# Sthiber/COSC_4397_Pathtracing_Raytracing_Project

Hardware: AMD Instinct MI355X
Metric: Msamples/s, cornell.txt 1920x1080 depth 8 (+PSNR vs 5000spp ref) (higher is better)
Workload: dtype f32

## Files before the change

### cosc_4397_pathtracing_raytracing_project_amd/capi.py

```python
from __future__ import annotations

import ctypes as C
import os
from typing import Optional, Sequence, Tuple

import numpy as np

_PKG = os.path.dirname(os.path.abspath(__file__))
LIB_PATH = os.environ.get("PT_AMD_LIB") or os.path.join(_PKG, "libpt_amd.so")
PT_MAX_DEPTH = 64
ARITH = {"exact": 0, "fma": 1, "fast": 2}
ARITH_NAMES = {v: k for k, v in ARITH.items()}
FEATURE_PLANES = 3
NOISE_PLANES = 2
NOISE_PIXELS_PER_PARTIAL = 1024
CONVERGENCE_WAVES = 16
CONVERGENCE_CAPACITY = 65536
FLT_MAX = float(np.finfo(np.float32).max)


class PtGeom(C.Structure):
    _fields_ = [("type", C.c_int32), ("materialid", C.c_int32), ("transform", C.c_float * 16),
                ("inverseTransform", C.c_float * 16), ("invTranspose", C.c_float * 16)]


class PtMaterial(C.Structure):
    _fields_ = [("color", C.c_float * 3), ("specular_exponent", C.c_float), ("specular_color", C.c_float * 3),
                ("hasReflective", C.c_float), ("hasRefractive", C.c_float), ("indexOfRefraction", C.c_float),
                ("emittance", C.c_float)]


class PtCamera(C.Structure):
    _fields_ = [("resolution", C.c_int32 * 2), ("position", C.c_float * 3), ("lookAt", C.c_float * 3),
                ("view", C.c_float * 3), ("up", C.c_float * 3), ("right", C.c_float * 3), ("fov", C.c_float * 2),
                ("pixelLength", C.c_float * 2)]


class PtBVHNode(C.Structure):
    _fields_ = [("bmin", C.c_float * 3), ("bmax", C.c_float * 3), ("left", C.c_int32), ("right", C.c_int32),
                ("geomIndex", C.c_int32)]


class PtGridInfo(C.Structure):
    _fields_ = [("res", C.c_int32 * 3), ("origin", C.c_float * 3), ("cell_size", C.c_float * 3), ("pad", C.c_float),
                ("num_cells", C.c_int32), ("num_records", C.c_int32), ("num_leaves", C.c_int32)]


class PtGridRecord(C.Structure):
    _fields_ = [("bmin", C.c_float * 3), ("bmax", C.c_float * 3), ("leaf", C.c_int32), ("neighbours", C.c_int32)]


class PtSceneDesc(C.Structure):
    _fields_ = [("geoms", C.POINTER(PtGeom)), ("num_geoms", C.c_int32), ("materials", C.POINTER(PtMaterial)),
                ("num_materials", C.c_int32), ("camera", PtCamera), ("trace_depth", C.c_int32)]


class PtOptions(C.Structure):
    _fields_ = [("device", C.c_int32), ("pixel_begin", C.c_int32), ("pixel_count", C.c_int32),
                ("iters_per_batch", C.c_int32), ("num_queues", C.c_int32), ("blocks_per_cu", C.c_int32),
                ("time_kernels", C.c_int32), ("legacy_traversal", C.c_int32), ("debug_flags", C.c_int32), ("unfused_primary", C.c_int32), ("unfused_bounces", C.c_int32), ("stripe_pixels", C.c_int32), ("stripe_stride", C.c_int32),
                ("arith", C.c_int32), ("aa_jitter", C.c_int32), ("convergence", C.c_int32),
                ("lds_table_kb", C.c_int32), ("primary_pieces", C.c_int32), ("paths_pieces", C.c_int32), ("paths_min_piece", C.c_int32)]


class PtStats(C.Structure):
    _fields_ = [("samples", C.c_int64), ("live_rays", C.c_int64 * PT_MAX_DEPTH), ("intersect_launches", C.c_int64),
                ("intersect_ms", C.c_double), ("render_ms", C.c_double), ("num_cus", C.c_int32),
                ("grid_blocks", C.c_int32), ("num_queues", C.c_int32), ("iters_per_batch", C.c_int32),
                ("device_bytes", C.c_int64), ("primary_fused", C.c_int32), ("bounces_fused", C.c_int32),
                ("arith", C.c_int32), ("grid_cells", C.c_int32), ("tight_leaves", C.c_int32), ("paths_waves", C.c_int32), ("record_form", C.c_int32)]


class PtDenoiseOptions(C.Structure):
    _fields_ = [("levels", C.c_int32), ("sigma_color", C.c_float), ("sigma_normal", C.c_float), ("sigma_position", C.c_float),
                ("keep_albedo", C.c_int32)]


class PtError(RuntimeError):
    pass


_lib: Optional[C.CDLL] = None
_fp = C.POINTER(C.c_float)
_ip = C.POINTER(C.c_int32)


def lib() -> C.CDLL:
    global _lib
    if _lib is not None:
        return _lib
    if not os.path.exists(LIB_PATH):
        raise PtError(f"{LIB_PATH} not found: run `python -c 'import __graft_entry__ as g; g.build()'` "
                      "(hipcc --offload-arch=gfx950).  There is no CPU fallback.")
    L = C.CDLL(LIB_PATH)
    L.pt_last_error.restype = C.c_char_p
    L.pt_scene_load.argtypes = [C.c_char_p, C.c_int, C.c_int, C.POINTER(C.c_void_p)]
    L.pt_scene_free.argtypes = [C.c_void_p]
    L.pt_scene_free.restype = None
    L.pt_scene_desc.argtypes = [C.c_void_p, C.POINTER(PtSceneDesc)]
    L.pt_scene_iterations.argtypes = [C.c_void_p]
    L.pt_scene_image_name.argtypes = [C.c_void_p]
    L.pt_scene_image_name.restype = C.c_char_p
    L.pt_build_bvh.argtypes = [C.POINTER(PtGeom), C.c_int, C.POINTER(PtBVHNode), C.c_int]
    L.pt_build_grid.argtypes = [C.POINTER(PtGeom), C.c_int, C.c_int, C.POINTER(PtGridInfo), C.POINTER(C.c_uint32), C.POINTER(PtGridRecord)]
    if hasattr(L, "pt_selfcheck_ieee"):
        L.pt_selfcheck_ieee.argtypes = [C.c_int, C.c_int, C.c_uint64, C.c_uint64, C.c_uint32, C.POINTER(C.c_uint64)]
    if hasattr(L, "pt_traversal_boxes"):
        L.pt_traversal_boxes.argtypes = [C.POINTER(PtGeom), C.c_int, _fp, _fp]
    if hasattr(L, "pt_center_half_box"):
        L.pt_center_half_box.argtypes = [_fp, _fp, C.c_int, C.c_float, _fp, _fp]
        L.pt_center_half_box.restype = None
    L.pt_build_transform.argtypes = [_fp, _fp, _fp, _fp]
    L.pt_init.argtypes = [C.POINTER(PtSceneDesc), C.POINTER(PtOptions)]
    L.pt_render.argtypes = [C.c_int, C.c_int]
    L.pt_readback.argtypes = [_fp]
    L.pt_readback_device.argtypes = [C.c_void_p]
    L.pt_preview_rgba8.argtypes = [C.c_int, C.POINTER(C.c_uint8)]
    L.pt_preview_rgba8_device.argtypes = [C.c_int, C.c_void_p]
    L.pt_get_stats.argtypes = [C.POINTER(PtStats)]
    L.pt_stage_generate.argtypes = [C.c_int, C.c_int, _fp, _fp]
    L.pt_stage_intersect.argtypes = [C.c_int, _fp, _fp, _fp, _fp, _ip, _fp]
    if hasattr(L, "pt_stage_intersect_grid"):
        L.pt_stage_intersect_grid.argtypes = [C.c_int, _fp, _fp, C.c_int, _fp, _fp, _ip, _fp]
        L.pt_stage_grid_info.argtypes = [C.POINTER(PtGridInfo), C.POINTER(C.c_int32)]
    L.pt_stage_shade.argtypes = [C.c_int, C.c_int, _ip, _ip, _fp, _fp, _ip, _fp, _fp, _fp, _fp, _ip]
    _u8p = C.POINTER(C.c_uint8)
    L.pt_save_u8.argtypes = [C.c_float, _u8p]
    L.pt_stage_save_u8.argtypes = [C.c_int, C.c_int, C.c_float, _fp, _u8p]
    L.pt_ctx_create.argtypes = [C.POINTER(PtSceneDesc), C.POINTER(PtOptions), C.POINTER(C.c_void_p)]
    L.pt_ctx_destroy.argtypes = [C.c_void_p]
    L.pt_ctx_render.argtypes = [C.c_void_p, C.c_int, C.c_int]
    L.pt_ctx_sync.argtypes = [C.c_void_p]
    L.pt_ctx_readback.argtypes = [C.c_void_p, _fp]
    L.pt_ctx_readback_device.argtypes = [C.c_void_p, C.c_void_p]
    L.pt_ctx_save_u8.argtypes = [C.c_void_p, C.c_float, _u8p]
    L.pt_ctx_get_stats.argtypes = [C.c_void_p, C.POINTER(PtStats)]
    L.pt_ctx_reset_stats.argtypes = [C.c_void_p]
    L.pt_ctx_clear.argtypes = [C.c_void_p]
    L.pt_ctx_pixel_count.argtypes = [C.c_void_p]
    L.pt_group_create.argtypes = [C.POINTER(PtSceneDesc), C.POINTER(PtOptions), _ip, C.c_int, C.POINTER(C.c_void_p)]
    if hasattr(L, "pt_group_create_ex"):
        L.pt_group_create_ex.argtypes = [C.POINTER(PtSceneDesc), C.POINTER(PtOptions), _ip, C.c_int, C.c_int, C.POINTER(C.c_void_p)]
        L.pt_group_transport.argtypes = [C.c_void_p]
    L.pt_group_destroy.argtypes = [C.c_void_p]
    L.pt_group_size.argtypes = [C.c_void_p]
    L.pt_group_context.argtypes = [C.c_void_p, C.c_int]
    L.pt_group_context.restype = C.c_void_p
    L.pt_group_render.argtypes = [C.c_void_p, C.c_int, C.c_int]
    L.pt_group_sync.argtypes = [C.c_void_p]
    L.pt_group_gather.argtypes = [C.c_void_p, _fp]
    L.pt_group_gather_u8.argtypes = [C.c_void_p, C.c_float, _u8p]
    L.pt_group_preview_rgba8.argtypes = [C.c_void_p, C.c_int, _u8p]
    L.pt_write_png_rgb8.argtypes = [C.c_char_p, _u8p, C.c_int, C.c_int]
    L.pt_output_basename.argtypes = [C.c_char_p, C.c_int, C.c_char_p, C.c_int]
    L.pt_save_png.argtypes = [C.c_char_p, _fp, C.c_int, C.c_int, C.c_float]
    L.pt_save_hdr.argtypes = [C.c_char_p, _fp, C.c_int, C.c_int, C.c_float]
    L.pt_save_pfm.argtypes = [C.c_char_p, _fp, C.c_int, C.c_int, C.c_float]
    L.pt_load_pfm.argtypes = [C.c_char_p, _fp, C.c_int, _ip, _ip, C.c_float]
    _dp = C.POINTER(C.c_double)
    L.pt_psnr_from_sse.argtypes = [C.c_double, C.c_int64]
    L.pt_psnr_from_sse.restype = C.c_float
    L.pt_set_reference.argtypes = [_fp]
    L.pt_get_convergence.argtypes = [C.c_int, C.c_int, _dp]
    L.pt_iterations_to_clean.argtypes = [C.c_float, _ip]
    L.pt_ctx_set_reference.argtypes = [C.c_void_p, _fp]
    L.pt_ctx_get_convergence.argtypes = [C.c_void_p, C.c_int, C.c_int, _dp]
    L.pt_ctx_iterations_to_clean.argtypes = [C.c_void_p, C.c_float, _ip]
    L.pt_group_set_reference.argtypes = [C.c_void_p, _fp]
    L.pt_group_get_convergence.argtypes = [C.c_void_p, C.c_int, C.c_int, _dp]
    L.pt_group_iterations_to_clean.argtypes = [C.c_void_p, C.c_float, _ip]
    if hasattr(L, "pt_render_features"):
        L.pt_render_features.argtypes = [C.c_int, C.c_int]
        L.pt_readback_features.argtypes = [_fp]
        L.pt_ctx_render_features.argtypes = [C.c_void_p, C.c_int, C.c_int]
        L.pt_ctx_readback_features.argtypes = [C.c_void_p, _fp]
        L.pt_ctx_device_features.argtypes = [C.c_void_p]
        L.pt_ctx_device_features.restype = C.c_void_p
        L.pt_group_render_features.argtypes = [C.c_void_p, C.c_int, C.c_int]
        L.pt_group_gather_features.argtypes = [C.c_void_p, _fp]
    if hasattr(L, "pt_denoise"):
        _dno = C.POINTER(PtDenoiseOptions)
        L.pt_denoise.argtypes = [C.c_float, _dno, _fp]
        L.pt_ctx_denoise.argtypes = [C.c_void_p, C.c_float, _dno, _fp]
        L.pt_ctx_denoise_device.argtypes = [C.c_void_p, C.c_float, _dno, C.POINTER(C.c_void_p)]
        L.pt_group_denoise.argtypes = [C.c_void_p, C.c_float, _dno, _fp]
        L.pt_stage_denoise.argtypes = [C.c_int, C.c_int, _fp, _fp, C.c_float, _dno, _fp]
        L.pt_denoise_host.argtypes = [C.c_int, C.c_int, _fp, _fp, C.c_float, _dno, _fp]
    if hasattr(L, "pt_denoise_guided"):
        _dno = C.POINTER(PtDenoiseOptions)
        _guided = [C.c_int, C.c_int, _fp, _fp, _fp, C.c_int, C.c_int64, _dno]
        L.pt_denoise_guided.argtypes = [_dno, _fp]
        L.pt_ctx_denoise_guided.argtypes = [C.c_void_p, _dno, _fp]
        L.pt_ctx_denoise_guided_device.argtypes = [C.c_void_p, _dno, C.POINTER(C.c_void_p)]
        L.pt_group_denoise_guided.argtypes = [C.c_void_p, _dno, _fp]
        L.pt_stage_denoise_guided.argtypes = _guided + [_fp]
        L.pt_denoise_guided_host.argtypes = _guided + [_fp]
        L.pt_denoise_guided_variance_host.argtypes = _guided + [_fp, _fp]
    if hasattr(L, "pt_noise_fold"):
        _until = [C.c_int, C.c_int, C.c_int, C.c_float, _ip, _fp]
        L.pt_noise_fold.argtypes = []
        L.pt_get_noise.argtypes = [_dp, _ip, _ip]
        L.pt_readback_noise.argtypes = [_fp]
        L.pt_render_until.argtypes = _until
        L.pt_ctx_noise_fold.argtypes = [C.c_void_p]
        L.pt_ctx_get_noise.argtypes = [C.c_void_p, _dp, _ip, _ip]
        L.pt_ctx_readback_noise.argtypes = [C.c_void_p, _fp]
        L.pt_ctx_render_until.argtypes = [C.c_void_p] + _until
        L.pt_ctx_device_noise.argtypes = [C.c_void_p]
        L.pt_ctx_device_noise.restype = C.c_void_p
        L.pt_group_noise_fold.argtypes = [C.c_void_p]
        L.pt_group_get_noise.argtypes = [C.c_void_p, _dp, _ip, _ip]
        L.pt_group_render_until.argtypes = [C.c_void_p] + _until
        L.pt_noise_fold_host.argtypes = [C.c_int, _fp, _fp, C.c_int, C.c_int, C.c_int64, _dp]
    if hasattr(L, "pt_adaptive_round"):
        _i64p = C.POINTER(C.c_int64)
        _adaptive = [C.c_int, C.c_int, C.c_int, C.c_float, C.c_float, _ip, _i64p, _fp]
        L.pt_adaptive_round.argtypes = [C.c_int, C.c_int, C.c_float]
        L.pt_render_adaptive.argtypes = _adaptive
        L.pt_readback_adaptive.argtypes = [_ip]
        L.pt_resolve.argtypes = [_fp]
        L.pt_ctx_adaptive_round.argtypes = [C.c_void_p, C.c_int, C.c_int, C.c_float]
        L.pt_ctx_render_adaptive.argtypes = [C.c_void_p] + _adaptive
        L.pt_ctx_readback_adaptive.argtypes = [C.c_void_p, _ip]
        L.pt_ctx_resolve.argtypes = [C.c_void_p, _fp]
        L.pt_ctx_resolve_device.argtypes = [C.c_void_p, C.POINTER(C.c_void_p)]
        L.pt_adaptive_select_host.argtypes = [C.c_int, C.c_int, _fp, _ip, C.c_int, _ip]
        L.pt_stage_adaptive_select.argtypes = [C.c_int, C.c_int, _fp, _ip, C.c_int, _ip]
        L.pt_adaptive_merge_host.argtypes = [C.c_int, _fp, _fp, _ip, _ip, C.c_int, _fp, C.c_int, _dp]
        L.pt_stage_render_list.argtypes = [_ip, C.c_int, C.c_int, C.c_int, _fp]
    if hasattr(L, "pt_denoise_adaptive"):
        _dno = C.POINTER(PtDenoiseOptions)
        _dn_adaptive = [C.c_int, C.c_int, _fp, _fp, _fp, _ip, _dno]
        L.pt_denoise_adaptive.argtypes = [_dno, _fp]
        L.pt_ctx_denoise_adaptive.argtypes = [C.c_void_p, _dno, _fp]
        L.pt_ctx_denoise_adaptive_device.argtypes = [C.c_void_p, _dno, C.POINTER(C.c_void_p)]
        L.pt_stage_denoise_adaptive.argtypes = _dn_adaptive + [_fp]
        L.pt_denoise_adaptive_host.argtypes = _dn_adaptive + [_fp]
        L.pt_denoise_adaptive_variance_host.argtypes = _dn_adaptive + [_fp, _fp]
    _lib = L
    return L


def _check(rc: int) -> None:
    if rc != 0:
        raise PtError(lib().pt_last_error().decode(errors="replace"))


def _f(a: np.ndarray):
    assert a.dtype == np.float32 and a.flags.c_contiguous
    return a.ctypes.data_as(_fp)


def _i(a: np.ndarray):
    assert a.dtype == np.int32 and a.flags.c_contiguous
    return a.ctypes.data_as(_ip)


class Scene:

    def __init__(self, path: str, res: Optional[Tuple[int, int]] = None):
        self._h = C.c_void_p()
        w, h = res if res else (0, 0)
        _check(lib().pt_scene_load(os.fsencode(path), int(w), int(h), C.byref(self._h)))
        self.desc = PtSceneDesc()
        _check(lib().pt_scene_desc(self._h, C.byref(self.desc)))

    def __del__(self):
        h = getattr(self, "_h", None)
        if h is not None and h.value and _lib is not None:
            _lib.pt_scene_free(h)
            self._h = C.c_void_p()

    @property
    def resolution(self) -> Tuple[int, int]:
        return self.desc.camera.resolution[0], self.desc.camera.resolution[1]

    @property
    def trace_depth(self) -> int:
        return self.desc.trace_depth

    @trace_depth.setter
    def trace_depth(self, d: int) -> None:
        self.desc.trace_depth = int(d)

    @property
    def iterations(self) -> int:
        return lib().pt_scene_iterations(self._h)

    @property
    def image_name(self) -> str:
        return lib().pt_scene_image_name(self._h).decode()

    def geoms(self):
        return [self.desc.geoms[i] for i in range(self.desc.num_geoms)]

    def materials(self):
        return [self.desc.materials[i] for i in range(self.desc.num_materials)]

    def grid(self, forced: bool = False):
        info = PtGridInfo()
        rc = lib().pt_build_grid(self.desc.geoms, self.desc.num_geoms, int(forced), C.byref(info), None, None)
        if rc < 0:
            raise PtError(lib().pt_last_error().decode(errors="replace"))
        if rc == 0:
            return None
        start = (C.c_uint32 * (info.num_cells + 1))()
        recs = (PtGridRecord * info.num_records)()
        lib().pt_build_grid(self.desc.geoms, self.desc.num_geoms, int(forced), C.byref(info), start, recs)
        return info, np.frombuffer(start, np.uint32).copy(), recs

    def traversal_boxes(self):
        boxes = np.zeros((self.desc.num_geoms, 6), np.float32)
        cam = np.asarray(list(self.desc.camera.position), np.float32)
        rc = lib().pt_traversal_boxes(self.desc.geoms, self.desc.num_geoms, _f(cam), _f(boxes))
        if rc < 0:
            raise PtError(lib().pt_last_error().decode(errors="replace"))
        return boxes, rc

    def bvh(self):
        n = lib().pt_build_bvh(self.desc.geoms, self.desc.num_geoms, None, 0)
        arr = (PtBVHNode * n)()
        lib().pt_build_bvh(self.desc.geoms, self.desc.num_geoms, arr, n)
        return arr


def selfcheck_ieee(kind: int, first: int, count: int, seed: int = 0, arith: str = "exact") -> int:
    n = C.c_uint64(0)
    _check(lib().pt_selfcheck_ieee(ARITH[arith], kind, first, count, seed, C.byref(n)))
    return int(n.value)


def build_transform(trs: Sequence[float]):
    t = np.asarray(trs, np.float32).copy()
    m, i, it = (np.zeros(16, np.float32) for _ in range(3))
    lib().pt_build_transform(_f(t), _f(m), _f(i), _f(it))
    return m, i, it


def make_options(device: int = 0, pixel_begin: int = 0, pixel_count: int = 0, iters_per_batch: int = 0,
                 num_queues: int = 0, blocks_per_cu: int = 0, time_kernels: bool = False, legacy_traversal: bool = False,
                 debug_flags: int = 0, unfused_primary: bool = False, unfused_bounces: bool = False,
                 stripe_pixels: int = 0, stripe_stride: int = 0, arith="exact", aa_jitter: bool = False,
                 lds_table_kb: int = 0, primary_pieces: int = 0, paths_pieces: int = 0, paths_min_piece: int = 0, primary_share: int = 0,
                 convergence: int = 0) -> PtOptions:
    opt = PtOptions()
    opt.device = device
    opt.pixel_begin = pixel_begin
    opt.pixel_count = pixel_count
    opt.iters_per_batch = iters_per_batch
    opt.num_queues = num_queues
    opt.blocks_per_cu = blocks_per_cu
    opt.time_kernels = 1 if time_kernels else 0
    opt.legacy_traversal = 1 if legacy_traversal else 0
    opt.debug_flags = int(debug_flags)
    opt.unfused_primary = 1 if unfused_primary else 0
    opt.unfused_bounces = 1 if unfused_bounces else 0
    opt.stripe_pixels = int(stripe_pixels)
    opt.stripe_stride = int(stripe_stride)
    opt.arith = ARITH[arith] if isinstance(arith, str) else int(arith)
    opt.aa_jitter = 1 if aa_jitter else 0
    opt.convergence = int(convergence)
    opt.lds_table_kb = int(lds_table_kb)
    pp = int(primary_pieces)
    opt.primary_pieces = pp if pp < 0 else min(pp, 0x7fff) | max(0, min(int(primary_share), 64)) << 16
    opt.paths_pieces = int(paths_pieces)
    opt.paths_min_piece = int(paths_min_piece)
    return opt


def split_features(planes: np.ndarray) -> dict:
    p = planes.reshape(FEATURE_PLANES, -1, 4)
    return dict(normal=np.ascontiguousarray(p[0, :, :3]), depth=np.ascontiguousarray(p[0, :, 3]),
                albedo=np.ascontiguousarray(p[1, :, :3]), hits=np.ascontiguousarray(p[1, :, 3]),
# ... 504 lines not shown
```

### cosc_4397_pathtracing_raytracing_project_amd/csrc/pt_api.cpp

```cpp
#include <cmath>
#include <cstdarg>
#include <cstdio>
#include <cstring>
#include <string>

#include "pt_adaptive.h"
#include "pt_context.h"
#include "pt_lds.h"
#include "pt_scene.h"
#include "pt_sched.h"

namespace {

std::string g_err;
constexpr int kDebugFlags = 16 | 32 | 64 | 128 | 256 | 512 | ptk::kRetireEveryIteration | 2048 | ptk::kWholeRecords | ptk::kNoFirstBounce;
static_assert(sizeof(PtOptions) == 80, "capi.PtOptions mirrors this layout");
static_assert(PT_CONVERGENCE_WAVES == ptk::kConvWaves, "pt_amd.h documents the size of the convergence metric's partial sums");
}
int pt_fail(const char* fmt, ...) {
  char buf[1024];
  va_list ap;
  va_start(ap, fmt);
  vsnprintf(buf, sizeof(buf), fmt, ap);
  va_end(ap);
  g_err = buf;
  return -1;
}

namespace ptc {
static PtContext* g_default = nullptr;
PtContext* default_context() { return g_default; }

int get_events(Ctx& g, EventPair* ev) {
  if (!g.free_events.empty()) {
    *ev = g.free_events.back();
    g.free_events.pop_back();
    return 0;
  }
  HIP_OK(hipEventCreate(&ev->a));
  HIP_OK(hipEventCreate(&ev->b));
  return 0;
}
static int resolve_events(Ctx& g) {
  auto drain = [&](std::vector<EventPair>& pending, double& total_ms) -> int {
    for (auto& e : pending) {
      float ms = 0;
      HIP_OK(hipEventElapsedTime(&ms, e.a, e.b));
      total_ms += ms;
      g.free_events.push_back(e);
    }
    pending.clear();
    return 0;
  };
  g.isect_launches += (int64_t)g.pending_isect.size();
  return drain(g.pending_isect, g.isect_ms) || drain(g.pending_render, g.render_ms) ? -1 : 0;
}

ptk::SceneTables tables(const Ctx& g) {
  ptk::SceneTables t = g.scene;
  if (g.debug_flags & 16) t.cull_margin = INFINITY;
  if (g.debug_flags & 32) t.top_xor = 0;
  t.lds_table_bytes = g.lds_table_bytes;
  t.max_batch_iters = g.K;
  t.trace_depth = g.depth;
  t.scan_nodes_lds = -1;
  t.use_grid = !g.grids.empty() && g.grid_enabled && !(g.debug_flags & 512) ? 1 : 0;
  if (t.use_grid) {
    const Ctx::DeviceGrid& gr = g.grids[g.grid_pick];
    t.lds_table_bytes = -1;
    t.grid_start = gr.d_start + gr.guard;
    t.grid_items = gr.d_items;
    t.grid_items_b = gr.d_items_b;
    for (int a = 0; a < 3; ++a)
      t.grid_res[a] = gr.shape.res[a], t.grid_min[a] = gr.shape.gmin[a], t.grid_cs[a] = gr.shape.cs[a], t.grid_inv_cs[a] = gr.shape.inv_cs[a];
    t.grid_pad = gr.shape.pad;
  }
  return t;
}

static size_t pathbuf_words(int64_t stride) { return (size_t)(2 * stride + (stride * ptd::kPathPlane2Bytes + 15) / 16); }
static int alloc_pathbuf(Ctx& g, ptd::PathBuf* b, int64_t stride) {
  b->stride = stride;
  return dalloc(g, &b->r, pathbuf_words(stride));
}
static int alloc_hitbuf(Ctx& g, ptd::HitBuf* h, int64_t stride) {
  h->stride = stride;
  return dalloc(g, &h->t, stride) || dalloc(g, &h->n, 3 * stride) || dalloc(g, &h->mat, stride) || dalloc(g, &h->p, 3 * stride) ? -1 : 0;
}

static ptd::Queues queues_for(const Ctx& g, int grid) {
  ptd::Queues q = g.qs;
  q.W = grid * ptk::kWavesPerBlock;
  return q;
}

static int primary_share_of(const Ctx& g) { return (g.debug_flags & 128) ? 1 : g.primary_share ? g.primary_share : ptk::kShareMax; }
static bool shares_first_hit(const Ctx& g) { return ptk::primary_shares(primary_share_of(g), g.aa_jitter, !g.fuse_bounces); }

ptk::BatchInfo tile_batch(const Ctx& g, int iter_first, int K) {
  ptk::BatchInfo b{};
  b.iter_first = iter_first;
  b.K = K;
  b.N = g.N;
  b.pixel_begin = g.pixel_begin;
  b.trace_depth = g.depth;
  b.aa_jitter = g.aa_jitter ? 1 : 0;
  b.stripe = g.stripe;
  b.gap = g.stripe ? g.stripe_stride - g.stripe : 0;
  b.inv_stripe = g.stripe ? 1.0f / (float)g.stripe : 0.0f;
  return b;
}

int run_batch(Ctx& g, int iter_first, int kb) {
  ptk::BatchInfo b = tile_batch(g, iter_first, kb);
  b.slot_shift = g.slot_shift;
  b.flat = g.fuse_bounces ? 0 : 1;
  b.primary_share = primary_share_of(g);
  b.primary_pieces = g.primary_pieces ? g.primary_pieces
                     : ptk::primary_shares(b) ? ptk::auto_shared_pieces(kb, g.qs.nq, g.ret.wq0) : ptk::auto_primary_pieces(kb, g.qs.nq, g.ret.wq0);
  b.paths_pieces = g.paths_pieces;
  const ptk::SceneTables sc = tables(g);
  b.retire_once = ptk::retires_once(b, g.debug_flags) ? 1 : 0;
  b.split_records = ptk::record_form(b, g.debug_flags, ptk::search_form(sc), sc.num_mats);
  if (b.split_records == ptk::kFirstBounce) b.primary_pieces = 1;
  g.record_form = b.split_records;
  b.list = g.list;
  if (b.list) b.stripe = 1, b.gap = 0, b.inv_stripe = 1.0f;
  const ptk::KernelApi& k = *g.k;
  auto cnt_row = [&](int d) { return g.d_cnt + ptk::cnt_index(g.qs, d, 0); };
  int d0 = 0;
  if (g.fuse_primary) {
    k.primary(g.stream, g.grid_primary, sc, g.dcam, b, queues_for(g, g.grid_primary), cnt_row(0), cnt_row(1), g.buf[1],
              g.ret);
    d0 = 1;
  } else {
    k.generate(g.stream, g.grid_gen, g.dcam, b, queues_for(g, g.grid_gen), g.buf[0], cnt_row(0));
  }
  int src = d0 & 1;
  const bool all_depths = g.grid_paths > 0;
  EventPair ev{};
  auto timed_from = [&]() -> int {
    if (!g.time_kernels) return 0;
    if (get_events(g, &ev)) return -1;
    HIP_OK(hipEventRecord(ev.a, g.stream));
    return 0;
  };
  auto timed_to = [&]() -> int {
    if (!g.time_kernels) return 0;
    HIP_OK(hipEventRecord(ev.b, g.stream));
    g.pending_isect.push_back(ev);
    return 0;
  };
  if (all_depths) {
    if (timed_from()) return -1;
    k.paths(g.stream, g.grid_paths, sc, b, queues_for(g, g.grid_paths), g.d_cnt, g.buf[1], g.ret);
    if (timed_to()) return -1;
  }
  for (int d = d0; d < g.depth && !all_depths; ++d) {
    const int32_t* cin = cnt_row(d);
    int32_t* cout = cnt_row(d + 1);
    if (timed_from()) return -1;
    k.intersect(g.stream, g.grid_isect, sc, queues_for(g, g.grid_isect), cin, g.buf[src], g.hits, g.legacy, d == 0);
    if (timed_to()) return -1;
    k.shade(g.stream, g.grid_shade, sc, b, d, queues_for(g, g.grid_shade), cin, cout, g.buf[src], g.hits, g.buf[src ^ 1], g.ret);
    src ^= 1;
  }
  k.count_stats(g.stream, g.qs, g.d_cnt, g.depth, g.d_stats);
  ptk::ConvInfo cv{g.d_ref, g.d_partial, -1, kb};
  if (g.conv_live) {
    if (g.conv_have_ref) cv.first_k = 0;
    else if (g.conv >= iter_first && g.conv < iter_first + kb) cv.capture_k = g.conv - iter_first, cv.first_k = cv.capture_k + 1, g.conv_have_ref = true;
    g.conv_last = std::max(g.conv_last, iter_first + kb - 1);
  }
  if (cv.capture_k >= 0 || cv.first_k < kb) k.collect_conv(g.stream, b, g.qs, g.ret, g.d_image, cv, g.d_sse);
  else k.collect(g.stream, b, g.qs, g.ret, g.d_image);
  HIP_OK(hipGetLastError());
  g.samples += (int64_t)kb * g.N;
  if (g.pending_isect.size() > 16384) {
    HIP_OK(hipStreamSynchronize(g.stream));
    if (resolve_events(g)) return -1;
  }
  return 0;
}

void plan_launch(Ctx& g) {
  if (!g.borrowed) g.lds_table_bytes = g.k->lds_table_limit(tables(g), g.lds_table_forced);
  const ptk::SceneTables t = tables(g);
  g.grid_gen = g.num_cus * std::min(g.cap_bpc, g.k->resident_blocks_per_cu(ptk::kGenerate, t));
  g.grid_isect = g.num_cus * std::min(g.cap_bpc, g.k->resident_blocks_per_cu(g.legacy ? ptk::kIntersectLegacy : ptk::kIntersect, t));
  g.grid_shade = g.num_cus * std::min(g.cap_bpc, g.k->resident_blocks_per_cu(ptk::kShade, t));
  g.grid_primary = g.num_cus * std::min(g.cap_bpc, g.k->resident_blocks_per_cu(shares_first_hit(g) ? ptk::kPrimaryShared : ptk::kPrimary, t));
  g.ret.wq0 = ptk::wave_slot(0, g.qs.Q, g.grid_primary * ptk::kWavesPerBlock).wq;
  g.grid_paths = (g.fuse_bounces && g.depth > 1) ? g.num_cus * std::min(g.cap_bpc, g.k->resident_blocks_per_cu(ptk::kPaths, t)) : 0;
  g.qs.paths_W = g.grid_paths * ptk::kWavesPerBlock;
}

static int choose_traversal(Ctx& g) {
  auto drop_unused_grids = [&](size_t keep) {
    for (size_t i = 0; i < g.grids.size(); ++i) {
      const Ctx::DeviceGrid& d = g.grids[i];
      if (i == keep) continue;
      for (void* p : {(void*)d.d_start, (void*)d.d_items, d.d_items_b != d.d_items ? (void*)d.d_items_b : nullptr}) {
        if (!p) continue;
        (void)hipFree(p);
        g.allocs.erase(std::remove(g.allocs.begin(), g.allocs.end(), p), g.allocs.end());
      }
      g.device_bytes -= (int64_t)d.bytes;
    }
    g.grids = {g.grids[keep]};
    g.grid_pick = 0;
  };
  if (g.grids.empty()) return 0;
  if (!g.fuse_bounces || (g.debug_flags & (256 | 512))) {
    drop_unused_grids(0);
    return 0;
  }
  auto time_one = [&](float* ms) -> int {
    plan_launch(g);
    for (int rep = 0; rep < 2; ++rep) {
      EventPair ev{};
      if (get_events(g, &ev)) return -1;
      HIP_OK(hipEventRecord(ev.a, g.stream));
      if (run_batch(g, 1, std::min(g.K, 8))) return -1;
      HIP_OK(hipEventRecord(ev.b, g.stream));
      HIP_OK(hipStreamSynchronize(g.stream));
      HIP_OK(hipEventElapsedTime(ms, ev.a, ev.b));
      g.free_events.push_back(ev);
    }
    return 0;
  };
  g.grid_enabled = false;
  if (time_one(&g.probe_ms[0])) return -1;
  g.grid_enabled = true;
  size_t best = 0;
  for (size_t i = 0; i < g.grids.size(); ++i) {
    float ms = 0.f;
    g.grid_pick = i;
    if (time_one(&ms)) return -1;
    if (i == 0 || ms < 0.97f * g.probe_ms[1]) g.probe_ms[1] = ms, best = i;
  }
  drop_unused_grids(best);
  g.grid_enabled = g.probe_ms[1] < 0.95f * g.probe_ms[0];
  plan_launch(g);
  HIP_OK(hipMemsetAsync(g.d_image, 0, 3 * (size_t)g.N * sizeof(float), g.stream));
  HIP_OK(hipMemsetAsync(g.d_stats, 0, PT_MAX_DEPTH * sizeof(unsigned long long), g.stream));
  HIP_OK(hipStreamSynchronize(g.stream));
  g.samples = 0;
  return 0;
}

ptd::Queues single_queue(const Ctx& g, int n) {
  ptd::Queues qs{};
  qs.Q = 1;
  const ptk::QueuePlan p = ptk::queue_plan(n, 1, 1);
  qs.cap = p.cap;
  qs.W = g.grid * ptk::kWavesPerBlock;
  qs.cnt_stride = 16;
  qs.nq = p.nq;
  qs.inv_nq = 1.0f / (float)qs.nq;
  return qs;
}

void destroy(Ctx* c) {
  if (!c) return;
  destroy(c->worker);
  (void)hipSetDevice(c->device);
  if (c->stream) (void)hipStreamSynchronize(c->stream);
  for (void* p : c->allocs) (void)hipFree(p);
  auto kill = [](std::vector<EventPair>& v) {
    for (auto& e : v) {
      (void)hipEventDestroy(e.a);
      (void)hipEventDestroy(e.b);
    }
    v.clear();
  };
  kill(c->free_events);
  kill(c->pending_isect);
  kill(c->pending_render);
  if (c->stream && !c->borrowed) (void)hipStreamDestroy(c->stream);
  delete c;
}

static int open_device(Ctx& g, const PtOptions& opt) {
  g.arith = opt.arith;
  g.k = ptk::api_for(opt.arith);
  if (!g.k) return pt_fail("pt_init: arith %d is not one of PT_ARITH_EXACT / PT_ARITH_FMA / PT_ARITH_FAST", opt.arith);
  if (opt.convergence < -1) return pt_fail("pt_init: convergence %d is not 0 (off), N > 0 (frame captured at iteration N) or -1 (frame supplied)", opt.convergence);
  if (opt.convergence > PT_CONVERGENCE_CAPACITY) return pt_fail("pt_init: convergence %d exceeds PT_CONVERGENCE_CAPACITY (%d iterations)", opt.convergence, PT_CONVERGENCE_CAPACITY);
  if (opt.primary_pieces > 0 && (opt.primary_pieces >> 16) > ptk::kShareMax) return pt_fail("pt_init: primary_pieces 0x%x: primary_share %d exceeds %d (PT_PRIMARY_PIECES)", opt.primary_pieces, opt.primary_pieces >> 16, ptk::kShareMax);
  if (opt.debug_flags & ~kDebugFlags) return pt_fail("pt_init: debug_flags 0x%x: bits 0x%x are not defined", opt.debug_flags, opt.debug_flags & ~kDebugFlags);
  int ndev = 0;
  HIP_OK(hipGetDeviceCount(&ndev));
  if (ndev <= 0) return pt_fail("pt_init: no HIP device (this library has no CPU fallback)");
  if (opt.device < 0 || opt.device >= ndev) return pt_fail("pt_init: device %d of %d", opt.device, ndev);
  g.device = opt.device;
  HIP_OK(hipSetDevice(g.device));
  hipDeviceProp_t prop;
  HIP_OK(hipGetDeviceProperties(&prop, g.device));
  g.num_cus = prop.multiProcessorCount;
  HIP_OK(hipStreamCreateWithFlags(&g.stream, hipStreamNonBlocking));
  return 0;
}

static void take_scene_and_options(Ctx& g, const PtSceneDesc* sc, const PtOptions& opt) {
  g.cam = sc->camera;
  g.depth = sc->trace_depth;
  g.dcam.res_x = g.cam.resolution[0], g.dcam.res_y = g.cam.resolution[1];
  std::memcpy(g.dcam.pos, g.cam.position, 12);
  std::memcpy(g.dcam.view, g.cam.view, 12);
  std::memcpy(g.dcam.up, g.cam.up, 12);
  std::memcpy(g.dcam.right, g.cam.right, 12);
  g.dcam.pl_x = g.cam.pixelLength[0], g.dcam.pl_y = g.cam.pixelLength[1];
  g.legacy = opt.legacy_traversal != 0;
  g.aa_jitter = opt.aa_jitter != 0;
  g.debug_flags = opt.debug_flags;
  g.conv = opt.convergence;
  auto pieces = [](int v, int automatic) { return v ? std::clamp(v, 1, 0x7fff) : automatic; };
  g.lds_table_forced = opt.lds_table_kb ? std::clamp(opt.lds_table_kb, 0, ptk::kLdsTableBytes / 1024) * 1024 : -1;
  g.primary_pieces = pieces(opt.primary_pieces < 0 ? opt.primary_pieces : opt.primary_pieces & 0xffff, 0);
  g.primary_share = opt.primary_pieces < 0 ? 0 : std::min(opt.primary_pieces >> 16 & 0x7f, ptk::kShareMax);
  g.paths_pieces = ptk::pack_paths_pieces(pieces(opt.paths_pieces, 2), pieces(opt.paths_min_piece, 64));
  g.fuse_primary = !g.legacy && !opt.unfused_primary;
  g.fuse_bounces = g.fuse_primary && !opt.unfused_bounces;
  g.cap_bpc = opt.blocks_per_cu > 0 ? std::min(opt.blocks_per_cu, 8) : 8;
}

int batch_iters_for(int iters_per_batch, int N, int* slot_shift) {
  int K = iters_per_batch;
  if (K <= 0) {
    const int64_t target = 48ll << 20;
    K = (int)std::max<int64_t>(1, std::min<int64_t>(256, (target + N - 1) / N));
  }
  int shift = 1;
  while ((1ll << shift) < N) ++shift;
  if (shift > 30) return pt_fail("pt_init: tiles of more than 2^30 pixels are not supported");
  while (K > 1 && K > (1 << (31 - shift))) --K;
  if (slot_shift) *slot_shift = shift;
  return K;
}

int plan_batches(Ctx& g, const PtOptions& opt) {
  const int W = g.cam.resolution[0], H = g.cam.resolution[1];
  g.opt_iters_per_batch = opt.iters_per_batch, g.opt_num_queues = opt.num_queues;
  g.pixel_begin = opt.pixel_begin;
  g.N = opt.pixel_count > 0 ? opt.pixel_count : W * H - opt.pixel_begin;
  g.stripe = opt.stripe_pixels;
  g.stripe_stride = opt.stripe_stride;
  if (g.stripe < 0 || (g.stripe > 0 && g.stripe_stride < g.stripe)) return pt_fail("pt_init: bad stripe %d / stride %d", g.stripe, g.stripe_stride);
  {
    int64_t last = (int64_t)g.pixel_begin + g.N - 1;
    if (g.stripe > 0) last = (int64_t)g.pixel_begin + (g.N - 1) + (int64_t)((g.N - 1) / g.stripe) * (g.stripe_stride - g.stripe);
    if (g.pixel_begin < 0 || g.N <= 0 || last >= (int64_t)W * H)
      return pt_fail("pt_init: tile [%d, +%d, stripe %d/%d) outside %dx%d", opt.pixel_begin, opt.pixel_count, g.stripe, g.stripe_stride, W, H);
    if (g.stripe > 0 && g.N / g.stripe >= 32768) return pt_fail("pt_init: more than 32767 stripes");
    if (H >= 32768) return pt_fail("pt_init: image height %d not supported (>= 32768)", H);
  }
  const int K = batch_iters_for(opt.iters_per_batch, g.N, &g.slot_shift);
  if (K < 0) return -1;

  int Q = opt.num_queues > 0 ? opt.num_queues : 256;
  const int cu_waves = g.num_cus * ptk::kWavesPerBlock;
  if (Q > cu_waves) Q = cu_waves;
  while (cu_waves % Q) --Q;
  if (opt.num_queues <= 0)
    while (ptk::chunks_per_queue(g.N, Q) > 128 && 2 * Q <= cu_waves && cu_waves % (2 * Q) == 0) Q *= 2;
  const ptk::QueuePlan plan = ptk::queue_plan(g.N, Q, K);
  const int grid = g.num_cus * 8;
  g.K = K;
  g.grid = grid;
  g.qs.Q = Q;
  g.qs.W = grid * ptk::kWavesPerBlock;
  g.qs.cnt_stride = 16;
  g.qs.nq = plan.nq;
  g.qs.inv_nq = 1.0f / (float)plan.nq;
  g.qs.cap = plan.cap;
  g.stride = (int64_t)Q * g.qs.cap;
  g.ret.seg_cap = plan.seg_cap;
  g.ret.kmax = K;
  return 0;
}

template <typename T>
static const T* upload(Ctx& g, const std::vector<T>& v) {
  T* p = nullptr;
  if (dalloc(g, &p, v.size())) return nullptr;
  const hipError_t e = hipMemcpy(p, v.data(), v.size() * sizeof(T), hipMemcpyHostToDevice);
  return e == hipSuccess ? p : (pt_fail("hipMemcpy(%zu bytes) failed: %s", v.size() * sizeof(T), hipGetErrorString(e)), nullptr);
}
static int upload_tables(Ctx& g, const pt::HostTables& t) {
  ptk::SceneTables& s = g.scene;
  s.num_nodes = (int)t.nodes.size(), s.num_geoms = (int)t.geoms.size(), s.num_mats = (int)t.mats.size(), s.num_top = (int)t.top.size();
  std::memcpy(s.root_min, t.root_min, 12);
  std::memcpy(s.root_max, t.root_max, 12);
  s.cull_margin = t.cull_margin;
  s.top_xor = t.top_xor;
  s.has_triangles = t.has_triangles ? 1 : 0;
  g.tight_leaves = t.tight_leaves;
  if (!(s.nodes = upload(g, t.nodes)) || !(s.geoms = upload(g, t.geoms)) || !(s.mats = upload(g, t.mats)) || !(s.top = upload(g, t.top))) return -1;
  s.nodes_b = s.nodes, s.top_b = s.top;
  if (!t.nodes_b.empty() && (!(s.nodes_b = upload(g, t.nodes_b)) || !(s.top_b = upload(g, t.top_b)))) return -1;
  for (const pt::Grid& gr : t.grids) {
    Ctx::DeviceGrid d{gr.shape, gr.guard, nullptr, nullptr, nullptr, 0, gr.start};
    const int64_t before = g.device_bytes;
    if (!(d.d_start = upload(g, gr.start)) || !(d.d_items = upload(g, gr.items))) return -1;
    if (!(d.d_items_b = gr.items_b.empty() ? d.d_items : upload(g, gr.items_b))) return -1;
    d.bytes = (size_t)(g.device_bytes - before);
    g.grids.push_back(d);
  }
  return 0;
}

static __global__ void k_poison_records(ptd::Word4* rec, unsigned long long per_queue, unsigned long long total, int Q) {
  const float nan = __builtin_nanf("");
  for (unsigned long long i = (unsigned long long)blockIdx.x * blockDim.x + threadIdx.x; i < total; i += (unsigned long long)gridDim.x * blockDim.x)
    rec[i] = ptd::Word4{nan, nan, nan, __int_as_float(ptk::chunk_pixel((int)(i / per_queue), 0, Q))};
}

int alloc_batch_buffers(Ctx& g) {
  const int Q = g.qs.Q;
  if (alloc_pathbuf(g, &g.buf[0], g.stride) || alloc_pathbuf(g, &g.buf[1], g.stride)) return -1;
  for (const ptd::PathBuf& pb : g.buf) HIP_OK(hipMemset(pb.r, 0xff, pathbuf_words(pb.stride) * sizeof(ptd::Word4)));
  if (!g.fuse_bounces && alloc_hitbuf(g, &g.hits, g.stride)) return -1;
  {
    const size_t regions = (size_t)Q * g.ret.kmax;
    const size_t wq_max = ptk::sub_stride(g.num_cus * 8 * ptk::kWavesPerBlock, Q);
    if (dalloc(g, &g.ret.rec, regions * g.ret.seg_cap)) return -1;
    if (ensure(g, g.ret.cnt, regions * sizeof(*g.ret.cnt), Zero::blocking) || ensure(g, g.ret.sub, regions * wq_max * sizeof(*g.ret.sub), Zero::blocking)) return -1;
    {
      const size_t per_queue = (size_t)g.ret.kmax * g.ret.seg_cap;
      hipLaunchKernelGGL(k_poison_records, dim3((unsigned)std::min<size_t>((regions * g.ret.seg_cap + 255) / 256, 65536)), dim3(256), 0, g.stream, g.ret.rec,
                         (unsigned long long)per_queue, (unsigned long long)(regions * g.ret.seg_cap), Q);
      HIP_OK(hipGetLastError());
    }
  }
  const size_t image_bytes = 3 * (size_t)g.N * sizeof(float);
  const size_t cnt_words = ptk::cnt_index(g.qs, g.depth + 1, 0);
  if (ensure(g, g.d_image, image_bytes, Zero::blocking) || ensure(g, g.d_cnt, cnt_words * sizeof(int32_t), Zero::blocking) ||
      ensure(g, g.d_stats, PT_MAX_DEPTH * sizeof(*g.d_stats), Zero::blocking))
    return -1;
  if (!(g.debug_flags & 64) && ensure(g, g.qs.deal, (size_t)ptk::deal_map(g.qs).words() * sizeof(int32_t), Zero::blocking)) return -1;
  if (g.conv) {
    const size_t partials = (size_t)g.K * Q * ptk::kConvWaves;
    if (ensure(g, g.d_ref, image_bytes, Zero::blocking) || ensure(g, g.d_partial, partials * sizeof(double), Zero::blocking)) return -1;
    if (dalloc(g, &g.d_sse, (size_t)PT_CONVERGENCE_CAPACITY)) return -1;
    HIP_OK(hipMemset(g.d_sse, 0xff, (size_t)PT_CONVERGENCE_CAPACITY * sizeof(double)));
  }
  HIP_OK(hipDeviceSynchronize());
  return 0;
}

static int setup(Ctx& g, const PtSceneDesc* sc, const PtOptions& opt) {
  if (open_device(g, opt)) return -1;
  take_scene_and_options(g, sc, opt);
  if (plan_batches(g, opt)) return -1;
  if ((size_t)sc->num_materials * sizeof(ptd::Mat) > 60 * 1024) return pt_fail("pt_init: %zu materials exceed the LDS table", (size_t)sc->num_materials);
  const pt::HostTables host = pt::build_scene_tables(*sc, g.debug_flags, g.k->boxes_center_half != 0);
  if (upload_tables(g, host)) return -1;
  plan_launch(g);
  if (alloc_batch_buffers(g) || choose_traversal(g)) return -1;
  g.time_kernels = opt.time_kernels != 0;
  g.conv_live = g.conv != 0;
  return 0;
}

int need(const PtContext* c, const char* who) { return c ? 0 : pt_fail("%s: pt_init has not been called", who); }

int admit(const PtContext& g, const char* who, unsigned req) {
  if ((req & kNotFailed) && g.failed) return pt_fail("%s: an earlier batch of this context failed (%s); free it and create a new one", who, g_err.c_str());
  if ((req & kUniform) && g.adaptive)
    return pt_fail("%s: the renderer is in the adaptive state (pt_adaptive_round): one sample count no longer describes the image; read it with pt_resolve, or "
                   "return to the uniform state with pt_clear", who);
  const int W = g.cam.resolution[0];
  if ((req & kWholeRows) && (g.stripe || g.pixel_begin % W || g.N % W))
    return pt_fail("%s: the tile must consist of whole contiguous image rows (begin %d, count %d, stripe %d, width %d)", who, g.pixel_begin, g.N, g.stripe, W);
  if ((req & kFoldedAll) && g.rendered != g.noise_iters)
    return pt_fail("%s: %lld iteration(s) rendered since the last fold; fold first (pt_noise_fold)", who, (long long)(g.rendered - g.noise_iters));
  if (req & kOnDevice) HIP_OK(hipSetDevice(g.device));
  return 0;
}

}
using namespace ptc;

extern "C" {

const char* pt_last_error(void) { return g_err.c_str(); }

int pt_selfcheck_ieee(int arith, int kind, uint64_t first, uint64_t count, uint32_t seed, uint64_t* mismatches) {
  const ptk::KernelApi* k = ptk::api_for(arith);
  if (!k || kind < 0 || kind > 4 || !mismatches) return pt_fail("pt_selfcheck_ieee: bad argument");
  unsigned long long* d = nullptr;
  HIP_OK(hipMalloc(&d, sizeof(*d)));
  hipError_t e = hipMemset(d, 0, sizeof(*d));
  if (e == hipSuccess) {
    k->ieee_check(nullptr, kind, first, count, seed, d);
    e = hipGetLastError();
  }
  unsigned long long h = 0;
  if (e == hipSuccess) e = hipMemcpy(&h, d, sizeof(h), hipMemcpyDeviceToHost);
  (void)hipFree(d);
  if (e != hipSuccess) return pt_fail("pt_selfcheck_ieee: %s", hipGetErrorString(e));
  *mismatches = h;
  return 0;
}

struct PtScene {
  pt::Scene scene;
  explicit PtScene(const std::string& f) : scene(f) {}
};

int pt_scene_load(const char* path, int res_w, int res_h, PtScene** out) {
  if (!path || !out) return pt_fail("pt_scene_load: null argument");
  try {
    PtScene* s = new PtScene(path);
    if (res_w > 0 && res_h > 0) s->scene.overrideResolution(res_w, res_h);
    s->scene.applyInitialCameraState();
    *out = s;
    return 0;
  } catch (const std::exception& e) {
    return pt_fail("pt_scene_load: %s", e.what());
  }
}
void pt_scene_free(PtScene* s) { delete s; }
int pt_scene_desc(const PtScene* s, PtSceneDesc* out) {
  if (!s || !out) return pt_fail("pt_scene_desc: null argument");
  *out = s->scene.desc();
  return 0;
}
int pt_scene_iterations(const PtScene* s) { return s ? (int)s->scene.state.iterations : 0; }
const char* pt_scene_image_name(const PtScene* s) { return s ? s->scene.state.imageName.c_str() : ""; }

int pt_build_bvh(const PtGeom* geoms, int num_geoms, PtBVHNode* out, int cap) {
  std::vector<PtBVHNode> nodes;
  pt::buildBVH(geoms, num_geoms, nodes);
  if (out) std::memcpy(out, nodes.data(), sizeof(PtBVHNode) * std::min<size_t>(nodes.size(), (size_t)std::max(cap, 0)));
  return (int)nodes.size();
}

int pt_traversal_boxes(const PtGeom* geoms, int num_geoms, const float camera_position[3], float* boxes) {
  if (!geoms || num_geoms <= 0 || !camera_position || !boxes) return pt_fail("pt_traversal_boxes: null argument");
  pt::ThreadedBvh bvh = pt::threaded_bvh(geoms, num_geoms);
  double olo[3], ohi[3];
  pt::origin_region(bvh.ref[0].bmin, bvh.ref[0].bmax, camera_position, olo, ohi);
  const int tightened = pt::tighten_sphere_leaves(bvh.nodes, geoms, olo, ohi);
  for (const ptd::Node& n : bvh.nodes)
    if (n.geom >= 0) std::memcpy(boxes + 6 * (size_t)n.geom, n.bmin, 12), std::memcpy(boxes + 6 * (size_t)n.geom + 3, n.bmax, 12);
  return tightened;
}

int pt_build_grid(const PtGeom* geoms, int num_geoms, int forced, PtGridInfo* info, uint32_t* cell_start, PtGridRecord* records) {
  if (!geoms || num_geoms <= 0 || !info) return pt_fail("pt_build_grid: null argument");
  const pt::ThreadedBvh bvh = pt::threaded_bvh(geoms, num_geoms);
  std::memset(info, 0, sizeof(*info));
  info->num_leaves = num_geoms;
  if (!forced && (int)bvh.nodes.size() < pt::kGridNodes) return 0;
  pt::Grid gr;
  if (!pt::build_grid(bvh.nodes, geoms, num_geoms, bvh.ref[0].bmin, bvh.ref[0].bmax, 0.0, 0.0, forced != 0, gr)) return 0;
  for (int a = 0; a < 3; ++a) info->res[a] = gr.shape.res[a], info->origin[a] = gr.shape.gmin[a], info->cell_size[a] = gr.shape.cs[a];
  info->pad = gr.shape.pad;
  info->num_cells = (int32_t)(gr.start.size() - 1);
  info->num_records = (int32_t)gr.items.size();
  if (cell_start) std::memcpy(cell_start, gr.start.data(), gr.start.size() * sizeof(uint32_t));
  static_assert(sizeof(PtGridRecord) == sizeof(ptd::Node), "PtGridRecord mirrors the device record");
  if (records) std::memcpy(records, gr.items.data(), gr.items.size() * sizeof(ptd::Node));
  return 1;
}

void pt_center_half_box(const float lo[3], const float hi[3], int inner, float magnitude, float center[3], float half_extent[3]) {
  float a[3] = {lo[0], lo[1], lo[2]}, b[3] = {hi[0], hi[1], hi[2]};
  pt::center_half_box(a, b, inner != 0, (double)magnitude);
  std::memcpy(center, a, 12);
  std::memcpy(half_extent, b, 12);
}

int pt_build_transform(const float* trs, float* transform, float* inverse, float* invTranspose) {
  if (!trs || !transform || !inverse || !invTranspose) return pt_fail("pt_build_transform: null argument");
  pt::buildTransform(trs, transform, inverse, invTranspose);
  return 0;
}

int pt_ctx_create(const PtSceneDesc* sc, const PtOptions* opt_in, PtContext** out) {
  if (!out) return pt_fail("pt_ctx_create: null output");
  *out = nullptr;
  if (!sc) return pt_fail("pt_init: null scene");
  if (sc->num_geoms <= 0 || !sc->geoms) return pt_fail("pt_init: scene has no geometry");
  if (sc->num_materials <= 0 || !sc->materials) return pt_fail("pt_init: scene has no materials");
  if (sc->trace_depth <= 0 || sc->trace_depth > PT_MAX_DEPTH) return pt_fail("pt_init: trace_depth %d out of range", sc->trace_depth);
  const int W = sc->camera.resolution[0], H = sc->camera.resolution[1];
  if (W <= 0 || H <= 0 || (int64_t)W * H > (1ll << 30)) return pt_fail("pt_init: bad resolution %dx%d", W, H);
  for (int i = 0; i < sc->num_geoms; ++i) {
    if (sc->geoms[i].materialid < 0 || sc->geoms[i].materialid >= sc->num_materials)
      return pt_fail("pt_init: geom %d references material %d of %d", i, sc->geoms[i].materialid, sc->num_materials);
    if (sc->geoms[i].type < PT_GEOM_SPHERE || sc->geoms[i].type > PT_GEOM_TRIANGLE)
      return pt_fail("pt_init: geom %d has unknown type %d", i, sc->geoms[i].type);
  }
  PtOptions opt{};
  if (opt_in) opt = *opt_in;
  PtContext* c = new PtContext();
  if (setup(*c, sc, opt)) {
    destroy(c);
    return -1;
  }
  *out = c;
  return 0;
}

int pt_ctx_destroy(PtContext* c) {
  if (c == g_default) g_default = nullptr;
  destroy(c);
  return 0;
}

int pt_ctx_render(PtContext* c, int iter_first, int iter_count) {
  if (need(c, "pt_render")) return -1;
  if (iter_count <= 0) return 0;
  Ctx& g = *c;
  if (admit(g, "pt_render", kNotFailed | kUniform)) return -1;
  if (g.conv_live) {
    if (iter_first < 1 || (int64_t)iter_first + iter_count - 1 > PT_CONVERGENCE_CAPACITY)
      return pt_fail("pt_render: iterations %d .. %lld outside 1 .. %d (PT_CONVERGENCE_CAPACITY) with the convergence metric on", iter_first,
                  (long long)iter_first + iter_count - 1, PT_CONVERGENCE_CAPACITY);
    if (g.conv < 0 && !g.conv_have_ref) return pt_fail("pt_render: PtOptions.convergence is -1 but no reference frame has been supplied (pt_set_reference)");
  }
  HIP_OK(hipSetDevice(g.device));
  EventPair ev{};
  if (get_events(g, &ev)) return -1;
  HIP_OK(hipEventRecord(ev.a, g.stream));
  const int end = iter_first + iter_count;
  for (int it = iter_first; it < end; it += g.K)
    if (run_batch(g, it, std::min(g.K, end - it))) {
      g.failed = true;
      g.free_events.push_back(ev);
      return -1;
    }
  HIP_OK(hipEventRecord(ev.b, g.stream));
  g.pending_render.push_back(ev);
  g.rendered += iter_count;
  return 0;
}

int pt_ctx_sync(PtContext* c) {
  if (need(c, "pt_sync")) return -1;
  HIP_OK(hipSetDevice(c->device));
  HIP_OK(hipStreamSynchronize(c->stream));
  return resolve_events(*c);
}

int pt_ctx_readback(PtContext* c, float* out) {
  if (need(c, "pt_readback")) return -1;
  return copy_out(c, "pt_readback", out, 3, [&](const float** d) { return *d = c->d_image, 0; });
}

int pt_ctx_readback_device(PtContext* c, void* out) {
  if (need(c, "pt_readback_device")) return -1;
  return copy_out(c, "pt_readback_device", static_cast<float*>(out), 3, [&](const float** d) { return *d = c->d_image, 0; }, hipMemcpyDeviceToDevice);
}

const float* pt_ctx_device_image(PtContext* c) { return c ? c->d_image : nullptr; }
void* pt_ctx_stream(PtContext* c) { return c ? (void*)c->stream : nullptr; }
int pt_ctx_pixel_count(const PtContext* c) { return c ? c->N : 0; }
int pt_ctx_device(const PtContext* c) { return c ? c->device : -1; }

int pt_ctx_save_u8_device(PtContext* c, float samples, const uint8_t** rgb8_dev) {
  if (need(c, "pt_save_u8")) return -1;
  Ctx& g = *c;
  const int W = g.cam.resolution[0];
  if (!(samples > 0.0f)) return pt_fail("pt_save_u8: samples must be positive");
  if (admit(g, "pt_save_u8", kUniform)) return -1;
  if (g.pixel_begin % W || g.N % W || (g.stripe && g.stripe != W))
    return pt_fail("pt_save_u8: the tile must consist of whole image rows (begin %d, count %d, stripe %d, width %d)", g.pixel_begin, g.N, g.stripe, W);
  HIP_OK(hipSetDevice(g.device));
  if (ensure(g, g.d_rgb8, 3 * (size_t)g.N)) return -1;
  g.k->save_u8(g.stream, g.N, W, samples, g.d_image, g.d_rgb8);
  HIP_OK(hipGetLastError());
  if (rgb8_dev) *rgb8_dev = g.d_rgb8;
  return 0;
}
int pt_ctx_save_u8(PtContext* c, float samples, uint8_t* rgb8_host) {
  return copy_out(c, "pt_save_u8", rgb8_host, 3, [&](const uint8_t** d) { return pt_ctx_save_u8_device(c, samples, d); });
}

int pt_ctx_preview_rgba8_device(PtContext* c, int iterations, void* rgba_dev) {
  if (need(c, "pt_preview_rgba8_device")) return -1;
  if (!rgba_dev || iterations <= 0) return pt_fail("pt_preview_rgba8_device: bad argument");
  if (admit(*c, "pt_preview_rgba8_device", kUniform | kOnDevice)) return -1;
  c->k->preview(c->stream, c->N, iterations, c->d_image, reinterpret_cast<uchar4*>(rgba_dev));
  HIP_OK(hipStreamSynchronize(c->stream));
  return 0;
}

int pt_ctx_preview_rgba8(PtContext* c, int iterations, uint8_t* rgba_host) {
  if (need(c, "pt_preview_rgba8")) return -1;
  if (!rgba_host || iterations <= 0) return pt_fail("pt_preview_rgba8: bad argument");
  if (admit(*c, "pt_preview_rgba8", kUniform | kOnDevice)) return -1;
  uchar4* d = nullptr;
  HIP_OK(hipMalloc((void**)&d, (size_t)c->N * 4));
  c->k->preview(c->stream, c->N, iterations, c->d_image, d);
  hipError_t e = hipMemcpyAsync(rgba_host, d, (size_t)c->N * 4, hipMemcpyDeviceToHost, c->stream);
  if (e == hipSuccess) e = hipStreamSynchronize(c->stream);
  (void)hipFree(d);
  if (e != hipSuccess) return pt_fail("pt_preview_rgba8: %s", hipGetErrorString(e));
  return 0;
}

int pt_ctx_get_stats(PtContext* c, PtStats* out) {
  if (need(c, "pt_get_stats")) return -1;
  if (!out) return pt_fail("pt_get_stats: null");
  if (pt_ctx_sync(c)) return -1;
  Ctx& g = *c;
  std::memset(out, 0, sizeof(*out));
  unsigned long long st[PT_MAX_DEPTH];
  HIP_OK(hipMemcpy(st, g.d_stats, sizeof(st), hipMemcpyDeviceToHost));
  for (int d = 0; d < PT_MAX_DEPTH; ++d) out->live_rays[d] = (int64_t)st[d];
  out->samples = g.samples;
  out->intersect_launches = g.isect_launches;
  out->intersect_ms = g.isect_ms;
  out->render_ms = g.render_ms;
  out->num_cus = g.num_cus;
  out->grid_blocks = g.grid_paths > 0 ? g.grid_paths : g.grid_isect;
  out->num_queues = g.qs.Q;
  out->iters_per_batch = g.K;
  out->device_bytes = g.device_bytes;
  out->primary_fused = g.fuse_primary ? 1 : 0;
  out->bounces_fused = g.fuse_bounces ? 1 : 0;
  out->arith = g.arith;
  if (tables(g).use_grid && g.fuse_bounces) {
    const int* res = g.grids[g.grid_pick].shape.res;
    out->grid_cells = res[0] * res[1] * res[2];
  }
  out->tight_leaves = g.tight_leaves;
  out->record_form = g.record_form;
  out->paths_waves = 0;
  if (g.qs.deal && g.grid_paths > 0) {
    const ptk::DealMap dm = ptk::deal_map(g.qs);
    std::vector<int32_t> first((size_t)dm.made_for() + 1);
    HIP_OK(hipMemcpy(first.data(), g.qs.deal + dm.first(0), first.size() * sizeof(int32_t), hipMemcpyDeviceToHost));
    if (first[dm.made_for()] == g.qs.paths_W) {
      int lo = first[1] - first[0], hi = lo;
      for (int q = 1; q < g.qs.Q; ++q) lo = std::min(lo, first[q + 1] - first[q]), hi = std::max(hi, first[q + 1] - first[q]);
      out->paths_waves = std::min(lo, 0xffff) << 16 | std::min(hi, 0xffff);
    }
  }
  return 0;
}

int pt_ctx_reset_stats(PtContext* c) {
  if (need(c, "pt_reset_stats")) return -1;
  if (pt_ctx_sync(c)) return -1;
  Ctx& g = *c;
  HIP_OK(hipMemsetAsync(g.d_stats, 0, PT_MAX_DEPTH * sizeof(unsigned long long), g.stream));
  HIP_OK(hipStreamSynchronize(g.stream));
  g.samples = 0;
  g.isect_ms = g.render_ms = 0;
  g.isect_launches = 0;
  return 0;
}

int pt_ctx_clear(PtContext* c) {
  if (need(c, "pt_clear")) return -1;
  if (pt_ctx_sync(c)) return -1;
  HIP_OK(hipMemsetAsync(c->d_image, 0, 3 * (size_t)c->N * sizeof(float), c->stream));
  if (c->d_feat) HIP_OK(hipMemsetAsync(c->d_feat, 0, (size_t)PT_FEATURE_PLANES * c->N * sizeof(float4), c->stream));
  if (c->d_noise) HIP_OK(hipMemsetAsync(c->d_noise, 0, pt_noise_state_bytes((size_t)c->N), c->stream));
  c->noise_groups = 0;
  c->noise_iters = c->rendered = 0;
  if (c->d_acnt) HIP_OK(hipMemsetAsync(c->d_acnt, 0, (size_t)c->N * sizeof(ptad::Cnt), c->stream));
  c->adaptive = false;
  c->adaptive_rounds = 0;
  c->adaptive_last = 0;
  if (c->conv) {
    HIP_OK(hipMemsetAsync(c->d_sse, 0xff, (size_t)PT_CONVERGENCE_CAPACITY * sizeof(double), c->stream));
    c->conv_last = 0;
    if (c->conv > 0) c->conv_have_ref = false;
  }
  return pt_ctx_reset_stats(c);
}

int pt_ctx_set_reference(PtContext* c, const float* rgb_avg_host) {
  if (need(c, "pt_set_reference")) return -1;
  if (!rgb_avg_host) return pt_fail("pt_set_reference: null image");
  if (c->conv != -1) return pt_fail("pt_set_reference: the renderer was created with PtOptions.convergence = %d, not -1", c->conv);
  if (pt_ctx_sync(c)) return -1;
  HIP_OK(hipMemcpyAsync(c->d_ref, rgb_avg_host, 3 * (size_t)c->N * sizeof(float), hipMemcpyHostToDevice, c->stream));
  HIP_OK(hipStreamSynchronize(c->stream));
  c->conv_have_ref = true;
  return 0;
}

int pt_ctx_get_convergence(PtContext* c, int iter_first, int iter_count, double* sse) {
  if (need(c, "pt_get_convergence")) return -1;
  if (!c->conv) return pt_fail("pt_get_convergence: the renderer was created with PtOptions.convergence = 0 (metric off)");
  if (iter_count < 0 || (iter_count > 0 && !sse)) return pt_fail("pt_get_convergence: bad argument");
  if (pt_ctx_sync(c)) return -1;
  for (int j = 0; j < iter_count; ++j) sse[j] = -1.0;
  const int64_t lo = std::max<int64_t>(iter_first, 1), hi = std::min<int64_t>((int64_t)iter_first + iter_count, (int64_t)PT_CONVERGENCE_CAPACITY + 1);
  if (lo >= hi) return 0;
  double* dst = sse + (lo - iter_first);
  HIP_OK(hipMemcpy(dst, c->d_sse + (lo - 1), (size_t)(hi - lo) * sizeof(double), hipMemcpyDeviceToHost));
  for (int64_t j = 0; j < hi - lo; ++j)
    if (!(dst[j] >= 0.0)) dst[j] = -1.0;
  return 0;
}

int pt_ctx_iterations_to_clean(PtContext* c, float threshold_db, int* iteration) {
  if (need(c, "pt_iterations_to_clean")) return -1;
  if (!iteration) return pt_fail("pt_iterations_to_clean: null output");
  std::vector<double> sse((size_t)std::max(c->conv_last, 0));
  if (pt_ctx_get_convergence(c, 1, (int)sse.size(), sse.data())) return -1;
  *iteration = -1;
  for (size_t i = 0; i < sse.size(); ++i)
    if (sse[i] >= 0.0 && pt_psnr_from_sse(sse[i], c->N) > threshold_db) {
      *iteration = (int)i + 1;
      break;
    }
  return 0;
}

int pt_free(void) {
  PtContext* c = g_default;
  g_default = nullptr;
  destroy(c);
  return 0;
}
int pt_init(const PtSceneDesc* sc, const PtOptions* opt) {
  pt_free();
  return pt_ctx_create(sc, opt, &g_default);
}
int pt_render(int iter_first, int iter_count) { return pt_ctx_render(g_default, iter_first, iter_count); }
int pt_sync(void) { return pt_ctx_sync(g_default); }
int pt_readback(float* out) { return pt_ctx_readback(g_default, out); }
int pt_readback_device(void* out) { return pt_ctx_readback_device(g_default, out); }
int pt_save_u8(float samples, uint8_t* rgb8_host) { return pt_ctx_save_u8(g_default, samples, rgb8_host); }
int pt_preview_rgba8(int iterations, uint8_t* rgba_host) { return pt_ctx_preview_rgba8(g_default, iterations, rgba_host); }
int pt_preview_rgba8_device(int iterations, void* rgba_dev) { return pt_ctx_preview_rgba8_device(g_default, iterations, rgba_dev); }
int pt_get_stats(PtStats* out) { return pt_ctx_get_stats(g_default, out); }
int pt_reset_stats(void) { return pt_ctx_reset_stats(g_default); }
int pt_clear(void) { return pt_ctx_clear(g_default); }
int pt_render_features(int iter_first, int iter_count) { return pt_ctx_render_features(g_default, iter_first, iter_count); }
int pt_readback_features(float* planes_host) { return pt_ctx_readback_features(g_default, planes_host); }
int pt_denoise(float samples, const PtDenoiseOptions* opt, float* rgb_avg_host) { return pt_ctx_denoise(g_default, samples, opt, rgb_avg_host); }
int pt_denoise_guided(const PtDenoiseOptions* opt, float* rgb_avg_host) { return pt_ctx_denoise_guided(g_default, opt, rgb_avg_host); }
int pt_denoise_adaptive(const PtDenoiseOptions* opt, float* rgb_avg_host) { return pt_ctx_denoise_adaptive(g_default, opt, rgb_avg_host); }
int pt_noise_fold(void) { return pt_ctx_noise_fold(g_default); }
int pt_get_noise(double* sse, int* groups, int* iterations) { return pt_ctx_get_noise(g_default, sse, groups, iterations); }
int pt_readback_noise(float* planes_host) { return pt_ctx_readback_noise(g_default, planes_host); }
int pt_render_until(int iter_first, int max_iters, int group_iters, float target_db, int* iters_done, float* psnr_db) {
  return pt_ctx_render_until(g_default, iter_first, max_iters, group_iters, target_db, iters_done, psnr_db);
}
int pt_adaptive_round(int iter_first, int group_iters, float fraction) { return pt_ctx_adaptive_round(g_default, iter_first, group_iters, fraction); }
int pt_render_adaptive(int iter_first, int max_iters, int group_iters, float fraction, float target_db, int* iters_done, int64_t* samples_done,
                       float* psnr_db) {
  return pt_ctx_render_adaptive(g_default, iter_first, max_iters, group_iters, fraction, target_db, iters_done, samples_done, psnr_db);
}
int pt_readback_adaptive(int32_t* counts) { return pt_ctx_readback_adaptive(g_default, counts); }
int pt_resolve(float* rgb_avg_host) { return pt_ctx_resolve(g_default, rgb_avg_host); }
int pt_set_reference(const float* rgb_avg_host) { return pt_ctx_set_reference(g_default, rgb_avg_host); }
int pt_get_convergence(int iter_first, int iter_count, double* sse) { return pt_ctx_get_convergence(g_default, iter_first, iter_count, sse); }
int pt_iterations_to_clean(float threshold_db, int* iteration) { return pt_ctx_iterations_to_clean(g_default, threshold_db, iteration); }

}
```

### cosc_4397_pathtracing_raytracing_project_amd/csrc/pt_context.h

```cpp
#pragma once
#include <hip/hip_runtime.h>

#include <algorithm>
#include <cstdint>
#include <vector>

#include "../../include/pt_amd.h"
#include "pt_device.h"
#include "pt_internal.h"
#include "pt_kernels.h"
#include "pt_tables.h"

#define HIP_OK(expr)                                                                                      \
  do {                                                                                                    \
    hipError_t e_ = (expr);                                                                               \
    if (e_ != hipSuccess) return pt_fail("%s failed: %s (%s:%d)", #expr, hipGetErrorString(e_), __FILE__, __LINE__); \
  } while (0)

struct EventPair {
  hipEvent_t a, b;
};

struct PtShared {
  int device = 0;
  hipStream_t stream = nullptr;
  const ptk::KernelApi* k = nullptr;
  int arith = 0;
  int num_cus = 0;
  PtCamera cam{};
  ptd::Camera dcam{};
  int depth = 0;
  ptk::SceneTables scene{};
  int lds_table_bytes = -1;
  int lds_table_forced = -1;
  int primary_pieces = 0;
  int primary_share = 0;
  int paths_pieces = 0;
  struct DeviceGrid {
    pt::GridShape shape;
    size_t guard;
    const uint32_t* d_start;
    const ptd::Node* d_items;
    const ptd::Node* d_items_b;
    size_t bytes;
    std::vector<uint32_t> start;
  };
  std::vector<DeviceGrid> grids;
  size_t grid_pick = 0;
  int tight_leaves = 0;
  bool grid_enabled = true;
  int cap_bpc = 8;
  bool legacy = false;
  int debug_flags = 0;
  int record_form = 0;
  bool fuse_primary = true, fuse_bounces = true;
  bool aa_jitter = false;
};

struct PtContext : PtShared {
  int N = 0, pixel_begin = 0, K = 1;
  int slot_shift = 0;
  int stripe = 0, stripe_stride = 0;
  int grid = 0;
  int grid_gen = 0, grid_isect = 0, grid_shade = 0;
  ptd::Queues qs{};
  int64_t stride = 0;
  std::vector<void*> allocs;
  int64_t device_bytes = 0;
  float probe_ms[2] = {0.f, 0.f};
  int grid_primary = 0, grid_paths = 0;
  ptd::PathBuf buf[2]{};
  ptd::HitBuf hits{};
  ptd::RetireBuf ret{};
  float* d_image = nullptr;
  float4* d_feat = nullptr;
  int grid_features = 0;
  void* d_denoise = nullptr;
  void* d_noise = nullptr;
  int noise_groups = 0;
  int64_t noise_iters = 0;
  int64_t rendered = 0;
  int conv = 0;
  bool conv_live = false;
  bool conv_have_ref = false;
  int conv_last = 0;
  float* d_ref = nullptr;
  double* d_partial = nullptr;
  double* d_sse = nullptr;
  uint8_t* d_rgb8 = nullptr;
  int32_t* d_cnt = nullptr;
  unsigned long long* d_stats = nullptr;
  bool time_kernels = false;
  std::vector<EventPair> free_events, pending_isect, pending_render;
  double isect_ms = 0, render_ms = 0;
  int64_t isect_launches = 0;
  int64_t samples = 0;
  bool failed = false;
  int opt_iters_per_batch = 0, opt_num_queues = 0;
  bool borrowed = false;
  const int32_t* list = nullptr;
  PtContext* worker = nullptr;
  int32_t* d_list = nullptr;
  void* d_acnt = nullptr;
  void* d_select = nullptr;
  float* d_resolved = nullptr;
  bool adaptive = false;
  int adaptive_rounds = 0;
  int64_t adaptive_last = 0;
};

namespace ptc {
using Ctx = PtContext;

PtContext* default_context();

template <typename T>
int dalloc(Ctx& g, T** out, size_t count) {
  void* p = nullptr;
  size_t bytes = std::max<size_t>(count * sizeof(T), 16);
  hipError_t e = hipMalloc(&p, bytes);
  if (e != hipSuccess) return pt_fail("hipMalloc(%zu bytes) failed: %s", bytes, hipGetErrorString(e));
  g.allocs.push_back(p);
  g.device_bytes += (int64_t)bytes;
  *out = reinterpret_cast<T*>(p);
  return 0;
}
enum class Zero { none, blocking, on_stream };
template <typename T>
int ensure(Ctx& g, T*& p, size_t bytes, Zero zero = Zero::none) {
  if (p) return 0;
  char* q = nullptr;
  if (dalloc(g, &q, bytes)) return -1;
  p = reinterpret_cast<T*>(q);
  if (zero == Zero::blocking) HIP_OK(hipMemset(q, 0, bytes));
  if (zero == Zero::on_stream) HIP_OK(hipMemsetAsync(q, 0, bytes, g.stream));
  return 0;
}
struct Scratch {
  std::vector<void*> p;
  ~Scratch() { for (void* q : p) (void)hipFree(q); }
  template <typename T>
  T* get(size_t n) {
    void* q = nullptr;
    if (hipMalloc(&q, std::max<size_t>(n * sizeof(T), 16)) != hipSuccess) return nullptr;
    p.push_back(q);
    return reinterpret_cast<T*>(q);
  }
};

int need(const PtContext* c, const char* who);
enum Require : unsigned {
  kNotFailed = 1,
  kUniform = 2,
  kWholeRows = 4,
  kFoldedAll = 8,
  kOnDevice = 16,
};
int admit(const PtContext& g, const char* who, unsigned req);

template <typename T, typename Source>
int copy_out(PtContext* c, const char* who, T* host, size_t per_pixel, Source source, hipMemcpyKind kind = hipMemcpyDeviceToHost) {
  if (!host) return pt_fail("%s: null buffer", who);
  const T* d = nullptr;
  if (source(&d)) return -1;
  HIP_OK(hipSetDevice(c->device));
  HIP_OK(hipMemcpyAsync(host, d, per_pixel * (size_t)c->N * sizeof(T), kind, c->stream));
  return pt_ctx_sync(c);
}

ptk::SceneTables tables(const Ctx& g);
ptk::BatchInfo tile_batch(const Ctx& g, int iter_first, int K);
int run_batch(Ctx& g, int iter_first, int kb);
int batch_iters_for(int iters_per_batch, int N, int* slot_shift);
int plan_batches(Ctx& g, const PtOptions& opt);
void plan_launch(Ctx& g);
int alloc_batch_buffers(Ctx& g);
int get_events(Ctx& g, EventPair* ev);
ptd::Queues single_queue(const Ctx& g, int n);
void destroy(Ctx* c);
int ensure_worker(Ctx& g, int m);
int render_list(Ctx& g, int iter_first, int iter_count);
}
```

### cosc_4397_pathtracing_raytracing_project_amd/csrc/pt_kernels.h

```cpp
#pragma once
#include <hip/hip_runtime.h>

#include "pt_device.h"

namespace ptk {

constexpr int kBlock = 256;
constexpr int kWavesPerBlock = 4;
constexpr int kLdsTableBytes = 64 * 1024;
constexpr int kMaxTop = ptd::kMaxTop;

struct SceneTables {
  const ptd::Node* nodes;
  int32_t num_nodes;
  const ptd::Geom* geoms;
  int32_t num_geoms;
  const ptd::Mat* mats;
  int32_t num_mats;
  const ptd::TopEntry* top;
  int32_t num_top;
  float root_min[3], root_max[3];
  float cull_margin;
  unsigned long long top_xor;
  int32_t lds_table_bytes;
  int32_t max_batch_iters;
  const uint32_t* grid_start;
  const ptd::Node* grid_items;
  int32_t grid_res[3];
  float grid_min[3], grid_cs[3], grid_inv_cs[3];
  float grid_pad;
  int32_t use_grid;
  int32_t trace_depth;
  int32_t has_triangles;
  const ptd::Node* nodes_b;
  const ptd::TopEntry* top_b;
  const ptd::Node* grid_items_b;
  int32_t scan_nodes_lds;
};

struct BatchInfo {
  int32_t iter_first;
  int32_t K;
  int32_t N;
  int32_t pixel_begin;
  int32_t stripe, gap;
  float inv_stripe;
  int32_t trace_depth;
  int32_t slot_shift;
  int32_t aa_jitter;
  int32_t flat;
  int32_t primary_pieces;
  int32_t primary_share;
  int32_t paths_pieces;
  int32_t retire_once;
  const int32_t* list;
  int32_t split_records;
};

constexpr int kConvWaves = 16;
struct ConvInfo {
  float* ref;
  double* partial;
  int32_t capture_k;
  int32_t first_k;
};

enum KernelId { kGenerate = 0, kIntersect = 1, kShade = 2, kIntersectLegacy = 3, kPrimary = 4, kPaths = 5, kFeatures = 6, kPrimaryShared = 7 };

struct KernelApi {
  const char* name;
  void (*generate)(hipStream_t s, int grid, const ptd::Camera& cam, const BatchInfo& b, const ptd::Queues& qs,
                   ptd::PathBuf out, int32_t* cnt0);
  void (*primary)(hipStream_t s, int grid, const SceneTables& sc, const ptd::Camera& cam, const BatchInfo& b,
                  const ptd::Queues& qs, int32_t* cnt0, int32_t* cnt_out, ptd::PathBuf out, ptd::RetireBuf ret);
  void (*intersect)(hipStream_t s, int grid, const SceneTables& sc, const ptd::Queues& qs, const int32_t* cnt_in,
                    ptd::PathBuf paths, ptd::HitBuf hits, bool legacy, bool exact_arith);
  void (*shade)(hipStream_t s, int grid, const SceneTables& sc, const BatchInfo& b, int depth, const ptd::Queues& qs,
                const int32_t* cnt_in, int32_t* cnt_out, ptd::PathBuf in, ptd::HitBuf hits, ptd::PathBuf out,
                ptd::RetireBuf ret);
  void (*collect)(hipStream_t s, const BatchInfo& b, const ptd::Queues& qs, ptd::RetireBuf ret, float* image_rgb );
  void (*count_stats)(hipStream_t s, const ptd::Queues& qs, int32_t* cnt, int depth_count, unsigned long long* stats);
  void (*preview)(hipStream_t s, int n, int iterations, const float* image_rgb, uchar4* rgba);
  void (*save_u8)(hipStream_t s, int n, int width, float samples, const float* image_rgb, uint8_t* rgb8);
  void (*shade_stage)(hipStream_t s, const SceneTables& sc, int trace_depth, int depth, int n, const int32_t* iter,
                      const int32_t* pixel, ptd::HitBuf hits, ptd::PathBuf paths, int32_t* alive);
  int (*lds_table_limit)(const SceneTables& sc, int forced_bytes);
  int (*resident_blocks_per_cu)(KernelId id, const SceneTables& sc);
  void (*ieee_check)(hipStream_t s, int kind, unsigned long long first, unsigned long long count, uint32_t seed, unsigned long long* bad);
  void (*paths)(hipStream_t s, int grid, const SceneTables& sc, const BatchInfo& b, const ptd::Queues& qs, int32_t* cnt, ptd::PathBuf in, ptd::RetireBuf ret);
  void (*collect_conv)(hipStream_t s, const BatchInfo& b, const ptd::Queues& qs, ptd::RetireBuf ret, float* image_rgb, const ConvInfo& cv, double* sse);
  void (*features)(hipStream_t s, int grid, const SceneTables& sc, const ptd::Camera& cam, const BatchInfo& b, float4* feat);
  int boxes_center_half;
  void (*intersect_grid)(hipStream_t s, int grid, const SceneTables& sc, const ptd::Queues& qs, const int32_t* cnt_in,
                         ptd::PathBuf paths, ptd::HitBuf hits, bool primary);
};
const KernelApi* api_exact();
const KernelApi* api_fma();
const KernelApi* api_fast();
inline const KernelApi* api_for(int arith) { return arith == 0 ? api_exact() : arith == 1 ? api_fma() : arith == 2 ? api_fast() : nullptr; }

}
```

### cosc_4397_pathtracing_raytracing_project_amd/csrc/pt_kernels.hip

```cpp
#include "pt_kernels.h"

#include <float.h>

#include <type_traits>

#include "pt_lds.h"
#include "pt_sched.h"
#include "pt_portable_math.h"

#ifndef PT_ARITH
#define PT_ARITH 0
#endif
#if PT_ARITH == 0
#define PT_NS arith_exact
#define PT_API_FN api_exact
#elif PT_ARITH == 1
#define PT_NS arith_fma
#define PT_API_FN api_fma
#elif PT_ARITH == 2
#define PT_NS arith_fast
#define PT_API_FN api_fast
#else
#error "PT_ARITH must be 0, 1 or 2"
#endif
// ... 1021 lines not shown
        retire_append(rt, dead, k, pl, s.c);
        return;
      }
      while (ck < k) next_iteration();
      const int sub0 = k * rt.seg_cap + sub_offset(quo, rem, crho) * 64;
      const unsigned long long deadm = ballot(dead);
      if (alive) path_store(out, qbase + sub0 + nl + rank_in(live), s.o, s.d, s.c, tag);
      if (dead) rt.rec[sub0 + nd + rank_in(deadm)] = ptd::Word4{s.c.x, s.c.y, s.c.z, __int_as_float(pl)};
      nl += (int)__popcll(live), nd += (int)__popcll(deadm);
    };
    if constexpr (RING) ws = carry_init<true, 2>(wbase), ws.qo_tab = cam_qo, ws.cam_o = o;
    if constexpr (SHARE && SPLIT == kFirstBounce) {
      const int sub_off = sub_offset(quo, rem, shared_rho(r, 0, wq)) * 64;
      int fnl = 0, fnd = 0;
      auto record_group = [&](unsigned long long best, const float* rec, const Group& g) {
        const bool valid = g.valid;
        const Hit h = resolve_hit(best, rec, valid, leaf_geom);
        const bool cdead = valid && (h.t < 0.0f || mats[h.mat].emittance > 0.0f), lives = valid && !cdead;
        const unsigned long long livem = ballot(lives), cdeadm = ballot(cdead);
        if (lives) path_store(out, qbase + sub_off + fnl + rank_in(livem), bounce_origin(h.n, h.p), h.n, g.d, PathTag{pack_first(g.pl, h.mat, b.slot_shift), g.phash, 0});
        if (cdead) {
          ShadeIO s;
          s.o = o;
          s.d = g.d;
          s.c = mk(1.0f, 1.0f, 1.0f);
          s.alive = false;
          shade_decide(mats, b.trace_depth, 0, iter_hash_of(ihash, sc, b, 0, 0) ^ g.phash, h.t, h.mat, s);
          rt.rec[sub_off + fnd + rank_in(cdeadm)] = ptd::Word4{s.c.x, s.c.y, s.c.z, __int_as_float(g.pl)};
        }
        fnl += (int)__popcll(livem), fnd += (int)__popcll(cdeadm);
      };
      pp.any = false;
      int it = 0;
      for (int jj = shared_rho(r, 0, wq); jj < sh.my_nq; jj += wq, ++it) trace(it, group_of(jj, 0), record_group);
      if constexpr (RING) {
        if (pp.any) {
          carry_drain_to<true, 2, kD0, true>(ws, pp.mark, lane, nodes, geoms);
          record_group(ws.best[pp.par * 64 + lane], ws.rec + pp.par * 6 * 64 + lane, pp.g);
        }
      }
      for (int k = lane; k < b.K; k += 64) rt.sub[k * rt.wq0 + shared_rho(r, k, wq)] = ((unsigned long long)(uint32_t)fnd << 32) | (uint32_t)fnl;
    } else if constexpr (SHARE) {
      const int cap = shared_run_cap(b.primary_share), sub_off = sub_offset(quo, rem, shared_rho(r, k0, wq)) * 64;
      const bool once = b.retire_once != 0;
      for (int run = 0, runs = shared_runs(k0, k1, cap); run < runs; ++run) {
        const Run sr = shared_run(k0, k1, cap, run);
        const int s0 = sr.k0, s1 = sr.k1;
        int vnl = 0, vnd = 0;
        auto shade_run = [&](unsigned long long best, const float* rec, const Group& g) {
          const bool valid = g.valid;
          const int pl = g.pl;
          const uint32_t phash = g.phash;
          const f3 d = g.d;
          const Hit h = resolve_hit(best, rec, valid, leaf_geom);
          const float ht = h.t;
          const int hmat = h.mat;
          const f3 hn = h.n, hp = h.p;
          if constexpr (SPLIT == kSplitRecords) {
            if (s0 == 0) {
              const bool lives = valid && !(ht < 0.0f || mats[hmat].emittance > 0.0f);
              const unsigned long long livem = ballot(lives);
              const f3 o1 = bounce_origin(hn, hp);
              if (lives) out.r[out.stride + qbase + sub_off + __builtin_amdgcn_readlane(vnl, 0) + rank_in(livem)] = ptd::Word4{o1.x, o1.y, o1.z, __int_as_float(hmat)};
            }
          }
          const bool cdead = once && valid && (ht < 0.0f || mats[hmat].emittance > 0.0f);
          const unsigned long long cdeadm = once ? ballot(cdead) : 0ull;
          if (once) {
            if (s0 == 0 && cdeadm) {
              ShadeIO s;
              s.o = o;
              s.d = d;
              s.c = mk(1.0f, 1.0f, 1.0f);
              s.alive = false;
              if (cdead) {
                shade_decide(mats, b.trace_depth, 0, iter_hash_of(ihash, sc, b, 0, 0) ^ phash, ht, hmat, s);
                rt.rec[sub_off + __builtin_amdgcn_readlane(vnd, 0) + rank_in(cdeadm)] = ptd::Word4{s.c.x, s.c.y, s.c.z, __int_as_float(pl)};
              }
            }
            if (ballot(valid && !cdead) == 0) {
              if (lane < s1 - s0) vnd += (int)__popcll(cdeadm);
              return;
            }
          }
          for (int k = s0; k < s1; ++k) {
            ShadeIO s;
            s.o = o;
            s.d = d;
            s.c = mk(1.0f, 1.0f, 1.0f);
            s.alive = false;
            Bounce bo;
            bo.kind = 0;
            if (valid) bo = shade_decide(mats, b.trace_depth, 0, iter_hash_of(ihash, sc, b, 0, k) ^ phash, ht, hmat, s);
            const bool alive = valid && s.alive, dead = valid && !s.alive;
            if (alive) shade_bounce(bo, hn, hp, s);
            const unsigned long long live = ballot(alive), deadm = once ? cdeadm : ballot(dead);
            const int nl = __builtin_amdgcn_readlane(vnl, k - s0), nd = __builtin_amdgcn_readlane(vnd, k - s0);
            const int sub0 = k * rt.seg_cap + sub_off;
            const PathTag tag{make_slot(b, k, pl), phash, k};
            if constexpr (SPLIT == kSplitRecords) {
              if (alive) out.r[qbase + sub0 + nl + rank_in(live)] = ptd::Word4{s.d.x, s.d.y, s.d.z, __uint_as_float(pack_kind(tag.slot, bo.kind == 1))};
            } else if (alive) path_store(out, qbase + sub0 + nl + rank_in(live), s.o, s.d, s.c, tag);
            if (dead && !once) rt.rec[sub0 + nd + rank_in(deadm)] = ptd::Word4{s.c.x, s.c.y, s.c.z, __int_as_float(pl)};
            if (lane == k - s0) vnl += (int)__popcll(live), vnd += (int)__popcll(deadm);
          }
        };
        if constexpr (RING) ws = carry_init<true, 2>(wbase), ws.qo_tab = cam_qo, ws.cam_o = o;
        pp.any = false;
        int it = 0;
        for (int jj = shared_rho(r, s0, wq); jj < sh.my_nq; jj += wq, ++it) trace(it, group_of(jj, 0), shade_run);
        if constexpr (RING) {
          if (pp.any) {
            carry_drain_to<true, 2, kD0, true>(ws, pp.mark, lane, nodes, geoms);
            shade_run(ws.best[pp.par * 64 + lane], ws.rec + pp.par * 6 * 64 + lane, pp.g);
          }
        }
        if (lane < s1 - s0) rt.sub[(s0 + lane) * rt.wq0 + shared_rho(r, s0 + lane, wq)] = ((unsigned long long)(uint32_t)vnd << 32) | (uint32_t)vnl;
      }
    } else {
      int it = 0;
      for (int k = k0, rho = strand_rho(r, k0, wq); k < k1; ++k, rho = rho + 1 == wq ? 0 : rho + 1) {
        for (int jj = rho; jj < sh.my_nq; jj += wq, ++it) trace(it, group_of(jj, k), shade_group);
      }
      if constexpr (RING) {
        if (pp.any) {
          carry_drain_to<true, 2, kD0, true>(ws, pp.mark, lane, nodes, geoms);
          shade_group(ws.best[pp.par * 64 + lane], ws.rec + pp.par * 6 * 64 + lane, pp.g);
        }
      }
      if (!b.flat)
        while (ck < k1) next_iteration();
    }
    if (plan.pieces == 1) break;
    int nx = 0;
    if (lane == 0) nx = atomicAdd(&qs.deal[deal_map(qs).strand_counter()], 1);
    strand = qs.W + __builtin_amdgcn_readfirstlane(nx);
  }
}

constexpr int kPathsWaves = 6;
constexpr int kPathsMinReady = 32;
PT_DEV uint32_t lds_offset(const void* p) { return (uint32_t)(uintptr_t)(__attribute__((address_space(3))) const char*)p; }
template <typename T>
PT_DEV const T* uniform_ptr(const T* p) {
  const uint64_t v = (uint64_t)(uintptr_t)p;
  const uint32_t lo = (uint32_t)__builtin_amdgcn_readfirstlane((int)(uint32_t)v), hi = (uint32_t)__builtin_amdgcn_readfirstlane((int)(uint32_t)(v >> 32));
  return reinterpret_cast<const T*>((uintptr_t)(((uint64_t)hi << 32) | lo));
}
PT_DEV void fetch_record_to_lds(const void* b0, const void* b1, const void* b2, int i, uint32_t lds_base) {
  uint32_t keep;
  const uint32_t off16 = (uint32_t)i << 4, off8 = (uint32_t)i << 3;
  asm volatile(
      "s_mov_b32 %[keep], m0\n\t"
      "s_mov_b32 m0, %[base]\n\t"
      "s_nop 0\n\t"
      "global_load_lds_dwordx4 %[o16], %[b0]\n\t"
      "s_add_u32 m0, m0, 0x400\n\t"
      "s_nop 0\n\t"
      "global_load_lds_dwordx4 %[o16], %[b1]\n\t"
      "s_add_u32 m0, m0, 0x400\n\t"
      "s_nop 0\n\t"
      "global_load_lds_dword %[o8], %[b2]\n\t"
      "s_add_u32 m0, m0, 0xfc\n\t"
      "s_nop 0\n\t"
      "global_load_lds_dword %[o8], %[b2] offset:4\n\t"
      "s_mov_b32 m0, %[keep]"
      : [keep] "=&s"(keep)
      : [base] "s"(lds_base), [b0] "s"(b0), [b1] "s"(b1), [b2] "s"(b2), [o16] "v"(off16), [o8] "v"(off8)
      : "memory", "scc");
}
PT_DEV void fetch_split_to_lds(const void* b0, const void* b1, int i, int i0, uint32_t lds_base) {
  uint32_t keep;
  const uint32_t off = (uint32_t)i << 4, off0 = (uint32_t)i0 << 4;
  asm volatile(
      "s_mov_b32 %[keep], m0\n\t"
      "s_mov_b32 m0, %[base]\n\t"
      "s_nop 0\n\t"
      "global_load_lds_dwordx4 %[o], %[b0]\n\t"
      "s_add_u32 m0, m0, 0x400\n\t"
      "s_nop 0\n\t"
      "global_load_lds_dwordx4 %[o0], %[b1]\n\t"
      "s_mov_b32 m0, %[keep]"
      : [keep] "=&s"(keep)
      : [base] "s"(lds_base), [b0] "s"(b0), [b1] "s"(b1), [o] "v"(off), [o0] "v"(off0)
      : "memory", "scc");
}
PT_DEV void read_record_slot(uint32_t s16, uint32_t s4, v4f& w0, v4f& w1, float& cz, int& nslot, int& nrs) {
  asm volatile(
      "s_waitcnt vmcnt(0)\n\t"
      "ds_read_b128 %0, %5\n\t"
      "ds_read_b128 %1, %5 offset:1024\n\t"
      "ds_read_b32 %2, %6\n\t"
      "ds_read_b32 %3, %6 offset:256\n\t"
      "ds_read_b32 %4, %6 offset:512\n\t"
      "s_waitcnt lgkmcnt(0)"
      : "=&v"(w0), "=&v"(w1), "=&v"(cz), "=&v"(nslot), "=&v"(nrs)
      : "v"(s16), "v"(s4)
      : "memory");
}
struct Lanes {
  unsigned long long* best;
  float* rec;
  uint16_t* ent;
  int head, count;
  int appended, processed;
};
PT_DEV Lanes lanes_init(char* base) {
  Lanes c;
  c.best = reinterpret_cast<unsigned long long*>(base + LanesMap::best);
  c.rec = reinterpret_cast<float*>(base + LanesMap::rec);
  c.ent = reinterpret_cast<uint16_t*>(base + LanesMap::ent);
  c.head = c.count = c.appended = c.processed = 0;
  return c;
}
PT_DEV void paths_chunk(Lanes& c, int n, int lane, f3 o, f3 d, const uint32_t* tword, const ptd::Geom* __restrict__ geoms) {
  const bool valid = lane < n;
  const uint32_t entry = c.ent[(c.head + lane) & (kRing - 1)];
  const int src = (int)(entry & 63u);
  const uint32_t tw = tword[valid ? entry >> 6 : 0u];
  const uint32_t leaf = tw & 255u;
  const f3 ro = mk(bperm(src, o.x), bperm(src, o.y), bperm(src, o.z));
  const f3 rd = mk(bperm(src, d.x), bperm(src, d.y), bperm(src, d.z));
  const ptd::Geom* G = geoms + (valid ? (int)(tw >> 8) : 0);
  f3 pt = mk(0.f, 0.f, 0.f), nrm = mk(0.f, 0.f, 0.f);
  const float t = geom_test<-1, false>(G, ro, rd, pt, nrm, mk(0.f, 0.f, 0.f));
  const uint32_t tb = __float_as_uint(t);
  if (valid && t > 0.f && tb < 0x7f7fffffu) {
    const unsigned long long key = ((unsigned long long)tb << 32) | leaf;
    unsigned long long* slot = &c.best[src];
    atomicMin(slot, key);
    if (*slot == key) {
      float* r = c.rec + src;
      r[0 * 64] = nrm.x, r[1 * 64] = nrm.y, r[2 * 64] = nrm.z;
      r[3 * 64] = pt.x, r[4 * 64] = pt.y, r[5 * 64] = pt.z;
    }
  }
  c.head = (c.head + n) & (kRing - 1);
  c.count -= n;
  c.processed += n;
}
typedef __attribute__((address_space(4))) const v4f cfloat4;
template <typename TOP>
PT_DEV void paths_search(Lanes& c, TOP* top, const uint32_t* tword, int ntop, const ptd::Geom* __restrict__ geoms, f3 o, f3 d,
                         bool fresh, int lane, int& mark) {
  const RayInv ri = ray_inv(d, o);
  if (fresh) {
    c.best[lane] = kNoHit;
    mark = c.processed;
  }
  uint32_t mask = 0;
  for (int e0 = 0; e0 < ntop; e0 += 8) {
#pragma unroll
    for (int u = 0; u < 8; ++u) {
      const int e = e0 + u;
      if (e < ntop) {
        const auto A = top[2 * e], B = top[2 * e + 1];
        mask = push_bit(mask, slab(o, ri, A.x, A.y, A.z, A.w, B.x, B.y));
      }
    }
  }
  mask = fresh ? mask : 0u;
  while (true) {
    const unsigned long long m = ballot(mask != 0u);
    if (!m) break;
    const int rank = rank_in(m);
    if (mask != 0u) {
      const int te = ntop - 1 - __builtin_ctz(mask);
      mask &= mask - 1u;
      c.ent[(c.head + c.count + rank) & (kRing - 1)] = (uint16_t)((te << 6) | lane);
      if (mask == 0u) mark = c.appended + rank + 1;
    }
    const int cnt = __popcll(m);
    c.count += cnt;
    c.appended += cnt;
    if (c.count >= 64) paths_chunk(c, 64, lane, o, d, tword, geoms);
  }
}
constexpr int kPathsScanWaves = 5, kPathsGridWaves = 5;
constexpr int kVisitLap = 32, kVisitsPerRefill = 31;
static_assert(kVisitLap + kVisitsPerRefill + 1 <= kVisitRing, "the visit ring laps a path in flight");
static_assert((kVisitRing & (kVisitRing - 1)) == 0, "visit numbers wrap with a mask");
template <Search MODE, int SPLIT = 0>
__global__ __launch_bounds__(kBlock, MODE == 0 ? kPathsWaves : MODE == 1 ? kPathsScanWaves : kPathsGridWaves) void k_paths(SceneTables sc, BatchInfo b, ptd::Queues qs, int32_t* __restrict__ cnt ,
                                                               ptd::PathBuf in, ptd::RetireBuf ret) {
  extern __shared__ float4 lds_raw[];
  char* lds = reinterpret_cast<char*>(lds_raw);
  const PathsLds L = paths_lds<MODE, kFast>(sc);
  stage16(lds + L.top, sc.top_b, MODE == 2 ? 0 : top_bytes(sc));
  stage16(lds + L.mats, sc.mats, mat_bytes(sc));
  const float4* top = reinterpret_cast<const float4*>(lds + L.top);
  const ptd::Mat* mats = reinterpret_cast<const ptd::Mat*>(lds + L.mats);
  const ptd::Node* nodes = sc.nodes_b;
  const ptd::Geom* geoms = sc.geoms;
  if (MODE == 0) {
    stage16(lds + L.geoms, sc.geoms, geom_bytes(sc));
    geoms = reinterpret_cast<const ptd::Geom*>(lds + L.geoms);
  }
  const char* lnodes = nullptr;
  if (MODE == 1 && sc.scan_nodes_lds > 0) {
    stage16(lds + L.nodes, sc.nodes_b, node_bytes(sc));
    lnodes = lds + L.nodes;
  }
  using WM = PathsWaveMap<MODE, kFast>;
  const int he = iter_hash_entries(sc);
  uint32_t* tword = reinterpret_cast<uint32_t*>(lds + L.tword);
  int* lmat = reinterpret_cast<int*>(lds + L.lmat);
  uint32_t* ihash = reinterpret_cast<uint32_t*>(lds + L.ihash);
  for (int d = 1; d < b.trace_depth; ++d) iter_hash_fill(ihash + (d - 1) * he, sc, b, d);
  for (int e = threadIdx.x; MODE == 0 && e < sc.num_top; e += blockDim.x) {
    const int leaf = sc.top[e].idx, gi = sc.nodes[leaf].geom;
    tword[e] = (uint32_t)leaf | ((uint32_t)gi << 8);
    lmat[leaf & 63] = sc.geoms[gi].material;
  }
  __syncthreads();
  const int wib = threadIdx.x >> 6;
  char* wbase = lds + L.waves + wib * L.wave_bytes;
  Lanes cy = lanes_init(wbase);
  GridRings gr = grid_rings_init<false>(wbase);
  Carry<false, 1>& cb = gr.cy;
  CellRing& cr = gr.cr;
  cb.lnodes = (const __attribute__((address_space(3))) v4f*)(lnodes ? lnodes : lds), cb.lds_nodes = lnodes != nullptr;
  constexpr bool SLOTS = MODE == 0;
  char* slots = wbase + WM::slots;
  int* died = reinterpret_cast<int*>(wbase + WM::died);
  int* fillc = reinterpret_cast<int*>(wbase + WM::fillc);
  const int ntop = sc.num_top;
  const int wave = __builtin_amdgcn_readfirstlane(blockIdx.x * kWavesPerBlock + wib);
  const int lane = lane_id();
  died[lane] = 0;
  const uint64_t t_begin = __builtin_amdgcn_s_memrealtime();
  const DealMap dm = deal_map(qs);
  const WaveSlot even = wave_slot(wave, qs.Q, qs.W);
  int q = even.q, r = even.r, wq = even.wq;
  if (qs.deal != nullptr && qs.deal[dm.made_for()] == qs.W) {
    int at_or_before = 0;
    for (int e0 = 0; e0 < qs.Q; e0 += 64) at_or_before += (int)__popcll(ballot(e0 + lane < qs.Q && qs.deal[dm.first(e0 + lane)] <= wave));
    q = at_or_before - 1;
    const int first = qs.deal[dm.first(q)];
    r = wave - first, wq = qs.deal[dm.first(q + 1)] - first;
  }
  const Retire rt = retire_of(ret, q);
  const int64_t qbase = (int64_t)q * qs.cap;
  const int wq0 = rt.wq0, ne = b.K * wq0;
  const int my_nq = queue_share(b, qs, q).my_nq, quo = my_nq / wq0, rem = my_nq % wq0;
  auto count_of = [&](int e) { return e < ne ? (int)(uint32_t)rt.sub[e] : 0; };
  int total = 0, csum = 0;
  const bool chunk_sums = ne <= 64 * 64;
  for (int e0 = 0; e0 < ne; e0 += 256) {
    int n4[4];
#pragma unroll
    for (int j = 0; j < 4; ++j) n4[j] = count_of(e0 + 64 * j + lane);
#pragma unroll
    for (int j = 0; j < 4; ++j) {
      int sum;
      (void)wave_prefix6(n4[j], sum);
      total += sum;
      if (lane == (e0 >> 6) + j) csum = sum;
    }
  }
  if (r == 0 && lane == 0) cnt[cnt_index(qs, 1, q)] = total;
  const PiecePlan pieces = piece_plan(total, wq, b.paths_pieces, qs.deal != nullptr, chunk_sums);
  [[maybe_unused]] int clist0 = 0;
  int ce = ne, cstart = total, ccnt = 0, clist = 0;
  int cord = 0;
  [[maybe_unused]] int cur_k = 0;
  [[maybe_unused]] uint32_t cur_h = 0u, next_h = 0u;
  int win0 = -64;
  unsigned long long wsub = 0ull;
  auto window_to = [&](int e) {
    if (e < win0 || e >= win0 + 64) {
      win0 = e;
      wsub = (e + lane < ne) ? rt.sub[e + lane] : 0ull;
    }
  };
  auto sub_word = [&](int e) -> unsigned long long {
    const uint32_t lo32 = (uint32_t)__builtin_amdgcn_readlane((int)(uint32_t)wsub, e - win0);
    const uint32_t hi32 = (uint32_t)__builtin_amdgcn_readlane((int)(uint32_t)(wsub >> 32), e - win0);
    return ((unsigned long long)hi32 << 32) | lo32;
  };
  window_to(0);
  auto cursor_bases = [&](int first_rank) {
    const int ec = min(ce, ne - 1), ck = ec / wq0, crho = ec - ck * wq0;
    clist = ck * rt.seg_cap + sub_offset(quo, rem, crho) * 64;
    if constexpr (SPLIT != 0) clist0 = invariant_slot(clist, ck, rt.seg_cap);
    if constexpr (SPLIT == kFirstBounce) cur_k = ck, cur_h = iter_hash(b.iter_first + ck, 0);
    window_to(ec);
    const int crec = clist + (int)(uint32_t)(sub_word(ec) >> 32);
    if (lane == 0) fillc[cord & (kVisitRing - 1)] = crec + (first_rank - cstart);
  };
  auto seek = [&](int at_rank) {
    int cum = 0, e_begin = 0;
    if (chunk_sums) {
      int all;
      const int cbefore = wave_prefix6(csum, all);
      const unsigned long long here = ballot(csum > 0 && cbefore <= at_rank && at_rank < cbefore + csum);
      if (here) {
        const int l = __builtin_ctzll(here);
        e_begin = l * 64, cum = __builtin_amdgcn_readlane(cbefore, l);
      }
    }
    for (int e0 = e_begin; e0 < ne; e0 += 64) {
      const int n = count_of(e0 + lane);
      int sum;
      const int before = wave_prefix6(n, sum);
      const unsigned long long here = ballot(n > 0 && cum + before <= at_rank && at_rank < cum + before + n);
      if (here) {
        const int l = __builtin_ctzll(here);
        ce = e0 + l, cstart = cum + __builtin_amdgcn_readlane(before, l), ccnt = __builtin_amdgcn_readlane(n, l);
        break;
      }
      cum += sum;
    }
    ++cord;
    cursor_bases(at_rank);
  };
  auto assign = [&](bool want, int rank, int& at, [[maybe_unused]] int& at0, int& rs) -> bool {
    bool pending = want;
    const int cord0 = cord;
    while (true) {
      const bool in = pending && rank < cstart + ccnt;
      if (in) at = clist + (rank - cstart), rs = cord;
      if constexpr (SPLIT != 0)
        if (in) at0 = clist0 + (rank - cstart);
      if constexpr (SPLIT == kFirstBounce)
        if (in) rs = (int)pack_visit(cur_k, cord), next_h = cur_h;
      pending = pending && !in;
      if (!ballot(pending) || ce >= ne || cord - cord0 >= kVisitsPerRefill) break;
      cstart += ccnt;
      ccnt = 0;
      int nxt = ce + 1;
      while (nxt < ne) {
        window_to(nxt);
        const unsigned long long holds = ballot((uint32_t)wsub != 0u) & (~0ull << (nxt - win0));
        if (holds) {
          nxt = win0 + (int)__builtin_ctzll(holds);
          ccnt = (int)(uint32_t)sub_word(nxt);
          break;
        }
        nxt = win0 + 64;
      }
      ce = min(nxt, ne);
      ++cord;
      cursor_bases(cstart);
    }
    return want && !pending;
  };
  const uint32_t s_base = (uint32_t)__builtin_amdgcn_readfirstlane((int)lds_offset(slots));
  const uint32_t s16 = s_base + (uint32_t)lane * 16u, s4 = s_base + (uint32_t)kSlotTail + (uint32_t)lane * 4u;
  const ptd::Word4 *in0 = uniform_ptr(in.r + qbase), *in1 = uniform_ptr(in.r + in.stride + qbase);
  const float* in2 = uniform_ptr(reinterpret_cast<const float*>(in.r + 2 * in.stride) + 2 * qbase);
  PathRec nx;
  nx.o = nx.d = nx.c = mk(0.f, 0.f, 0.f), nx.tag = PathTag{0, 0u, 0};
  int nx_rs = 0;
  int* slot_rs = reinterpret_cast<int*>(slots + kSlotVisit) + lane;
  auto fetch = [&](int at, [[maybe_unused]] int at0, int rs) {
    if constexpr (SLOTS && SPLIT == kSplitRecords) fetch_split_to_lds(in0, in1, at, at0, s_base), *slot_rs = rs;
    else if constexpr (SLOTS) fetch_record_to_lds(in0, in1, in2, SPLIT == kFirstBounce ? at0 : at, s_base), *slot_rs = rs;
    else if constexpr (SPLIT == kSplitRecords) {
      const ptd::Word4 w0 = in.r[qbase + at], w1 = in.r[in.stride + qbase + at0];
      nx.o = mk(w0.x, w0.y, w0.z), nx.d = mk(w0.w, w1.x, w1.y), nx.c = mk(w1.z, w1.w, 0.f), nx_rs = rs;
    } else nx = path_load(in, qbase + at), nx_rs = rs;
  };
  f3 o = mk(0.f, 0.f, 0.f), d = o, c = o;
  int slot = 0, depth = 1, mark = 0, rslot = 0;
  uint32_t phash = 0u;
  bool valid = false, fresh = false, owes = false;
  bool has_next = false;
  int streamed = 0, p_hi = 0;
  while (SPLIT != kFirstBounce) {
    if (streamed >= p_hi && p_hi >= 0) {
      int nextp = -1;
      if (cord == 0) nextp = r;
      else if (pieces.needs_counter()) {
        int v = 0;
        if (lane == 0) v = atomicAdd(&qs.deal[dm.piece_counter(q)], 1);
        nextp = wq + __builtin_amdgcn_readfirstlane(v);
      }
      const PieceRange pr = pieces.piece_range(nextp);
      if (pr.some) {
        streamed = pr.start, p_hi = pr.end;
        seek(streamed);
      } else {
        p_hi = -1;
      }
    }
    const bool take = !valid && has_next;
    if (ballot(take || owes || (!valid && !has_next && streamed < p_hi))) {
      v4f w0, w1;
      float cz;
      int nslot, nrs;
      if constexpr (SLOTS && SPLIT == kSplitRecords) {
        asm volatile(
            "s_waitcnt vmcnt(0)\n\t"
            "ds_read_b128 %0, %3\n\t"
            "ds_read_b128 %1, %3 offset:1024\n\t"
            "ds_read_b32 %2, %4 offset:512\n\t"
            "s_waitcnt lgkmcnt(0)"
            : "=&v"(w0), "=&v"(w1), "=&v"(nrs)
            : "v"(s16), "v"(s4)
            : "memory");
        cz = 0.f, nslot = 0;
      } else if constexpr (SLOTS) {
        read_record_slot(s16, s4, w0, w1, cz, nslot, nrs);
      } else {
        w0 = v4f{nx.o.x, nx.o.y, nx.o.z, nx.d.x}, w1 = v4f{nx.d.y, nx.d.z, nx.c.x, nx.c.y}, cz = nx.c.z, nslot = nx.tag.slot, nrs = nx_rs;
      }
      if (owes) {
        rt.rec[rslot] = ptd::Word4{c.x, c.y, c.z, __int_as_float(slot & ((1 << b.slot_shift) - 1))};
        owes = false;
      }
      if constexpr (SPLIT == kSplitRecords) {
        if (take) {
          const uint32_t word = __float_as_uint(w0.w);
          const ptd::Mat* m = mats + __float_as_int(w1.w);
          nslot = kind_sample_id(word);
          o = mk(w1.x, w1.y, w1.z), d = mk(w0.x, w0.y, w0.z);
          c = mul(mk(1.0f, 1.0f, 1.0f), kind_specular(word) ? mk(m->spec[0], m->spec[1], m->spec[2]) : mk(m->color[0], m->color[1], m->color[2]));
        }
      } else if (take) o = mk(w0.x, w0.y, w0.z), d = mk(w0.w, w1.x, w1.y), c = mk(w1.z, w1.w, cz);
      if (take) {
        slot = nslot, rslot = nrs;
        phash = utilhash((uint32_t)global_pixel(b, nslot & ((1 << b.slot_shift) - 1)));
        depth = 1;
        valid = fresh = true;
        has_next = false;
      }
      const bool lapping = ballot(valid && cord - rslot >= kVisitLap) != 0ull;
      const bool empty = !has_next && !lapping;
      const unsigned long long em = ballot(empty);
      const int rank = rank_in(em);
      const bool more = empty && streamed + rank < p_hi;
      int at = 0, at0 = 0, rs = 0;
      const bool served = assign(more, streamed + rank, at, at0, rs);
      if (served) {
        has_next = true;
        fetch(at, at0, rs);
      }
      streamed += (int)__popcll(ballot(served));
    }
    if (!ballot(valid || has_next) && p_hi < 0) break;
    bool ready;
    if constexpr (MODE == 0) {
      if (ballot(fresh)) {
        if constexpr (kFast) paths_search(cy, (cfloat4*)(uintptr_t)sc.top_b, tword, ntop, geoms, o, d, fresh, lane, mark);
        else paths_search(cy, top, tword, ntop, geoms, o, d, fresh, lane, mark);
      }
      ready = valid && (cy.processed - mark) >= 0;
      if (cy.count > 0 && __popcll(ballot(ready)) < kPathsMinReady) {
        paths_chunk(cy, cy.count, lane, o, d, tword, geoms);
        ready = valid;
      }
    } else {
      cb.best[lane] = kNoHit;
      if constexpr (MODE == 2) grid_search<1>(cb, cr, sc, nodes, geoms, o, d, valid, lane, 0);
      else {
        PT_STAT(14, 1);
        PT_STAT(15, __popcll(ballot(valid)));
        carry_search<true, 1>(cb, top, ntop, nodes, geoms, o, d, valid, lane, 0, sc.cull_margin, sc.top_xor);
      }
      while (cb.count > 0) carry_chunk<false, 1, false, MODE == 2>(cb, min(64, cb.count), lane, nodes, geoms);
      ready = valid;
    }
    fresh = false;
    {
      ShadeIO s;
      s.o = mk(0.f, 0.f, 0.f);
      s.d = d;
      s.c = c;
      s.alive = false;
      Bounce bo;
      bo.kind = 0;
      const int k = (int)((uint32_t)slot >> b.slot_shift);
      const unsigned long long best = cy.best[lane];
      Hit h{false, -1.0f, -1, 0, mk(0.f, 0.f, 0.f), mk(0.f, 0.f, 0.f)};
      if (ready) {
        if ((uint32_t)(best >> 32) != 0x7f7fffffu) {
          h.t = __uint_as_float((uint32_t)(best >> 32));
          const float* rr = cy.rec + lane;
          h.n = mk(rr[0 * 64], rr[1 * 64], rr[2 * 64]);
          h.p = mk(rr[3 * 64], rr[4 * 64], rr[5 * 64]);
          if constexpr (MODE == 0) {
            h.mat = lmat[(uint32_t)best & 63u];
          } else {
            const ptd::Geom* G = geoms + nodes[(uint32_t)best].geom;
            h.mat = G->material;
            if (MODE == 2) h.n = finish_normal(G, h.n);
          }
        }
        const uint32_t ih = he > 0 ? ihash[(depth - 1) * he + k] : iter_hash(b.iter_first + k, depth);
        bo = shade_decide(mats, b.trace_depth, depth, ih ^ phash, h.t, h.mat, s);
      }
      const bool alive = ready && s.alive, dead = ready && !s.alive;
      if (dead) atomicAdd(&died[depth & 63], 1);
      if (dead) rslot = atomicAdd(&fillc[rslot & (kVisitRing - 1)], 1);
      if (alive) shade_bounce(bo, h.n, h.p, s);
      if (ready) {
        c = s.c;
        if (alive) o = s.o, d = s.d, depth += 1, fresh = true;
        else valid = false, owes = true;
      }
    }
  }
  if constexpr (SPLIT == kFirstBounce) {
    static_assert(MODE == kLdsTables, "the first-bounce form takes its records from the refill slots of the LDS-table form");
    while (true) {
      if (ballot(fresh)) {
        if constexpr (kFast) paths_search(cy, (cfloat4*)(uintptr_t)sc.top_b, tword, ntop, geoms, o, d, fresh, lane, mark);
        else paths_search(cy, top, tword, ntop, geoms, o, d, fresh, lane, mark);
      }
      bool ready = valid && (cy.processed - mark) >= 0;
      if (cy.count > 0 && __popcll(ballot(ready)) < kPathsMinReady) {
        paths_chunk(cy, cy.count, lane, o, d, tword, geoms);
        ready = valid;
      }
      fresh = false;
      Bounce bo;
      bo.kind = 0, bo.rng_x = 1u, bo.roughness = 0.f;
      f3 axis = mk(0.f, 0.f, 0.f);
      bool go = false;
      {
        ShadeIO s;
        s.o = mk(0.f, 0.f, 0.f);
        s.d = d;
        s.c = c;
        s.alive = false;
        const int k = (int)((uint32_t)slot >> b.slot_shift);
        const unsigned long long best = cy.best[lane];
        Hit h{false, -1.0f, -1, 0, mk(0.f, 0.f, 0.f), mk(0.f, 0.f, 0.f)};
        if (ready) {
          if ((uint32_t)(best >> 32) != 0x7f7fffffu) {
            h.t = __uint_as_float((uint32_t)(best >> 32));
            const float* rr = cy.rec + lane;
            h.n = mk(rr[0 * 64], rr[1 * 64], rr[2 * 64]);
            h.p = mk(rr[3 * 64], rr[4 * 64], rr[5 * 64]);
            h.mat = lmat[(uint32_t)best & 63u];
          }
          const uint32_t ih = he > 0 ? ihash[(depth - 1) * he + k] : iter_hash(b.iter_first + k, depth);
          bo = shade_decide(mats, b.trace_depth, depth, ih ^ phash, h.t, h.mat, s);
        }
        const bool alive = ready && s.alive, dead = ready && !s.alive;
        if (dead) atomicAdd(&died[depth & 63], 1);
        if (dead) rslot = atomicAdd(&fillc[rslot & (kVisitRing - 1)], 1);
        if (ready) {
          c = s.c;
          if (alive) {
            const BounceAxis a = bounce_axis(bo, h.n, h.p, d);
            o = a.o, axis = a.f, go = true;
          } else valid = false, owes = true;
        }
      }
      if (streamed >= p_hi && p_hi >= 0) {
        int nextp = -1;
        if (cord == 0) nextp = r;
        else if (pieces.needs_counter()) {
          int v = 0;
          if (lane == 0) v = atomicAdd(&qs.deal[dm.piece_counter(q)], 1);
          nextp = wq + __builtin_amdgcn_readfirstlane(v);
        }
        const PieceRange pr = pieces.piece_range(nextp);
        if (pr.some) {
          streamed = pr.start, p_hi = pr.end;
          seek(streamed);
        } else {
          p_hi = -1;
        }
      }
      const bool take = !valid && has_next;
      if (ballot(take || owes || (!valid && !has_next && streamed < p_hi))) {
        v4f w0, w1;
        float cz;
        int word, vword;
        read_record_slot(s16, s4, w0, w1, cz, word, vword);
        if (owes) {
          rt.rec[rslot] = ptd::Word4{c.x, c.y, c.z, __int_as_float(slot & ((1 << b.slot_shift) - 1))};
          owes = false;
        }
        if (take) {
          const int pl = first_pixel(word, b.slot_shift), k = visit_k((uint32_t)vword);
          const f3 hn = mk(w0.w, w1.x, w1.y), cam_d = mk(w1.z, w1.w, cz);
          slot = make_slot(b, k, pl), rslot = visit_number((uint32_t)vword);
          phash = utilhash((uint32_t)global_pixel(b, pl));
          ShadeIO s;
          s.o = mk(0.f, 0.f, 0.f);
          s.d = cam_d;
          s.c = mk(1.0f, 1.0f, 1.0f);
          s.alive = false;
          bo = shade_decide(mats, b.trace_depth, 0, next_h ^ phash, 0.0f, first_material(word, b.slot_shift), s);
          o = mk(w0.x, w0.y, w0.z), c = s.c;
          axis = bo.kind == 1 ? bounce_reflect(cam_d, hn) : hn;
          depth = 0;
          valid = go = true;
          has_next = false;
        }
        const bool lapping = ballot(valid && visit_gap(cord, rslot) >= kVisitLap) != 0ull;
        const bool empty = !has_next && !lapping;
        const unsigned long long em = ballot(empty);
        const int rank = rank_in(em);
        const bool more = empty && streamed + rank < p_hi;
        int at = 0, at0 = 0, rs = 0;
        const bool served = assign(more, streamed + rank, at, at0, rs);
        if (served) {
          has_next = true;
          fetch(at, at0, rs);
        }
        streamed += (int)__popcll(ballot(served));
      }
      if (!ballot(valid || has_next) && p_hi < 0) break;
      if (go) d = bounce_sample(bo, axis), depth += 1, fresh = true;
    }
  }
  if (lane == 0) {
    int reached = 0, rays = 0;
    for (int dd = min(b.trace_depth - 1, 63); dd >= 2; --dd) {
      reached += died[dd];
      rays += reached;
      if (reached) atomicAdd(&cnt[cnt_index(qs, dd, q)], reached);
    }
    rays += reached + died[1];
    const int ticks = (int)min((uint64_t)(__builtin_amdgcn_s_memrealtime() - t_begin) >> 6, (uint64_t)0x3ffff);
    if (qs.deal != nullptr && rays) atomicAdd(&qs.deal[dm.time(q)], ticks), atomicAdd(&qs.deal[dm.rays(q)], rays);
  }
}

__global__ __launch_bounds__(kBlock) void k_shade_stage(SceneTables sc, int trace_depth, int depth, int n,
                                                        const int32_t* __restrict__ iter,
                                                        const int32_t* __restrict__ pixel, ptd::HitBuf hits,
                                                        ptd::PathBuf paths, int32_t* __restrict__ alive) {
  extern __shared__ float4 lds_raw[];
  char* lds = reinterpret_cast<char*>(lds_raw);
  const ShadeLds L = shade_lds<false>(sc);
  stage16(lds + L.mats, sc.mats, mat_bytes(sc));
  __syncthreads();
  const ptd::Mat* mats = reinterpret_cast<const ptd::Mat*>(lds + L.mats);
  const int64_t HS = hits.stride;
  for (int at = blockIdx.x * blockDim.x + threadIdx.x; at < n; at += gridDim.x * blockDim.x) {
    const PathRec pr = path_load(paths, at);
    ShadeIO s;
    s.o = pr.o;
    s.d = pr.d;
    s.c = pr.c;
    s.alive = false;
    const Bounce bo = shade_decide(mats, trace_depth, depth, iter_hash(iter[at], depth) ^ utilhash((uint32_t)pixel[at]), hits.t[at], hits.mat[at], s);
    if (bo.kind) shade_bounce(bo, mk(hits.n[at], hits.n[HS + at], hits.n[2 * HS + at]),
                              mk(hits.p[at], hits.p[HS + at], hits.p[2 * HS + at]), s);
    path_store(paths, at, s.o, s.d, s.c, pr.tag);
    alive[at] = s.alive ? 1 : 0;
  }
}

#include "pt_features.inc"
#include "pt_output.inc"
#include "pt_launch.inc"
const KernelApi kApi = {
#if PT_ARITH == 0
    "exact",
#elif PT_ARITH == 1
    "fma",
#else
    "fast",
#endif
    launch_generate, launch_primary, launch_intersect, launch_shade, launch_collect, launch_count_stats,
    launch_preview, launch_save_u8, launch_shade_stage, lds_table_limit, resident_blocks_per_cu, launch_ieee_check, launch_paths,
    launch_collect_conv, launch_features, kFast ? 1 : 0, launch_intersect_grid};

}
}

const KernelApi* PT_API_FN() { return &PT_NS::kApi; }

#if defined(PT_WALK_STATS) && PT_ARITH == 2
}
extern "C" int pt_debug_walk_stats(unsigned long long* out) {
  unsigned long long zero[16] = {0};
  if (hipDeviceSynchronize() != hipSuccess) return -1;
  if (hipMemcpyFromSymbol(out, HIP_SYMBOL(ptk::arith_fast::g_walk_stats), sizeof(zero)) != hipSuccess) return -1;
  if (hipMemcpyToSymbol(HIP_SYMBOL(ptk::arith_fast::g_walk_stats), zero, sizeof(zero)) != hipSuccess) return -1;
  return 16;
}
namespace ptk {
#endif

}
```

### cosc_4397_pathtracing_raytracing_project_amd/csrc/pt_launch.inc

```
template <bool EX, typename F>
void with_intersect_of(const SceneTables& sc, bool legacy, F&& f) {
  const bool in_lds = tables_in_lds(sc);
  if (legacy) in_lds ? f(k_intersect_legacy<true, EX>, legacy_lds<true>(sc).total) : f(k_intersect_legacy<false, EX>, legacy_lds<false>(sc).total);
  else in_lds ? f(k_intersect<true, EX>, intersect_lds<true>(sc).total) : f(k_intersect<false, EX>, intersect_lds<false>(sc).total);
}
template <typename F>
void with_intersect(const SceneTables& sc, bool legacy, bool exact, F&& f) {
  exact ? with_intersect_of<kD0>(sc, legacy, f) : with_intersect_of<false>(sc, legacy, f);
}
template <typename F>
void with_intersect_grid(const SceneTables& sc, bool primary, F&& f) {
  primary ? f(k_intersect_grid<kD0>, intersect_grid_lds<kFast, kD0>(sc).total) : f(k_intersect_grid<false>, intersect_grid_lds<kFast, false>(sc).total);
}
bool leaves_fit_top(const SceneTables& sc) { return (sc.num_nodes + 1) / 2 <= kMaxTop; }
template <typename F>
void with_features(const SceneTables& sc, F&& f) {
  if (tables_in_lds(sc)) return f(k_features<true, false>, intersect_lds<true>(sc).total);
  if (leaves_fit_top(sc)) return f(k_features<false, false>, intersect_lds<false>(sc).total);
  return f(k_features<false, true>, intersect_lds<false>(sc).total);
}
template <Search S, typename F>
void with_primary_of(const SceneTables& sc, bool share, int split, F&& f) {
  const int lds = primary_lds<S, kFast, kD0>(sc).total;
  if constexpr (S == kLdsTables)
    if (share && split == kFirstBounce) return f(k_primary<S, true, kFirstBounce>, lds);
  return !share ? f(k_primary<S>, lds) : split ? f(k_primary<S, true, kSplitRecords>, lds) : f(k_primary<S, true>, lds);
}
template <typename F>
void with_primary(const SceneTables& sc, bool share, int split, F&& f) {
  switch (search_form(sc)) {
    case kLdsTables: return with_primary_of<kLdsTables>(sc, share, split, f);
    case kTopScan: return with_primary_of<kTopScan>(sc, share, split, f);
    case kGrid: return with_primary_of<kGrid>(sc, share, split, f);
  }
}

template <typename F>
void with_paths(const SceneTables& sc, Search form, int split, F&& f) {
  switch (form) {
    case kLdsTables:
      if (split == kFirstBounce) return f(k_paths<kLdsTables, kFirstBounce>, paths_lds<kLdsTables, kFast>(sc).total);
      return split ? f(k_paths<kLdsTables, kSplitRecords>, paths_lds<kLdsTables, kFast>(sc).total) : f(k_paths<kLdsTables>, paths_lds<kLdsTables, kFast>(sc).total);
    case kTopScan: return split ? f(k_paths<kTopScan, kSplitRecords>, paths_lds<kTopScan, kFast>(sc).total) : f(k_paths<kTopScan>, paths_lds<kTopScan, kFast>(sc).total);
    case kGrid: return split ? f(k_paths<kGrid, kSplitRecords>, paths_lds<kGrid, kFast>(sc).total) : f(k_paths<kGrid>, paths_lds<kGrid, kFast>(sc).total);
  }
}
int paths_lds_bytes(const SceneTables& sc, Search form) {
  int bytes = 0;
  with_paths(sc, form, 0, [&](auto, int lds) { bytes = lds; });
  return bytes;
}
int lds_share_limit(int bytes);
SceneTables resolve_scan_nodes(const SceneTables& sc_in) {
  SceneTables sc = sc_in;
  if (iter_hash_entries(sc) > 0) {
    SceneTables without = sc;
    without.max_batch_iters = kIterHashMax + 1;
    const Search form = search_form(sc);
    const int reg_waves = form == kLdsTables ? kPathsWaves : form == kTopScan ? kPathsScanWaves : kPathsGridWaves;
    SceneTables a = sc, b = without;
    if (a.scan_nodes_lds < 0) a.scan_nodes_lds = b.scan_nodes_lds = 0;
    const bool costs = min(lds_share_limit(paths_lds_bytes(b, form)), reg_waves) > min(lds_share_limit(paths_lds_bytes(a, form)), reg_waves);
    if (costs) sc = without;
  }
  SceneTables t = sc;
  if (t.scan_nodes_lds >= 0) return t;
  SceneTables with = sc, without = sc;
  with.scan_nodes_lds = 1, without.scan_nodes_lds = 0;
  const int bw = paths_lds_bytes(with, kTopScan), bo = paths_lds_bytes(without, kTopScan);
  t.scan_nodes_lds = (bw <= 64 * 1024 && lds_share_limit(bw) >= min(lds_share_limit(bo), kPathsScanWaves)) ? 1 : 0;
  return t;
}
auto occupancy_into(int& n, int fallback) {
  return [&n, fallback](auto kernel, int lds) {
    if (hipOccupancyMaxActiveBlocksPerMultiprocessor(&n, kernel, kBlock, lds) != hipSuccess) n = fallback;
  };
}
int lds_table_limit(const SceneTables& sc, int forced_bytes) {
  if (forced_bytes >= 0) return leaves_fit_top(sc) ? forced_bytes : -1;
  const int tbl = table_bytes(sc);
  int with = 0, without = 0;
  if (tbl <= kLdsTableBytes && leaves_fit_top(sc)) {
    SceneTables in = sc;
    in.lds_table_bytes = tbl;
    with_paths(in, kLdsTables, 0, occupancy_into(with, 0));
  }
  with_paths(sc, kTopScan, 0, occupancy_into(without, 1));
  (void)hipGetLastError();
  return (with >= without && with > 0) ? tbl : -1;
}

constexpr int kLdsGranule = 1280;
int lds_share_limit(int bytes) { return bytes > 0 ? (160 * 1024) / (((bytes + kLdsGranule - 1) / kLdsGranule) * kLdsGranule) : 8; }
int resident_blocks_per_cu(KernelId id, const SceneTables& sc) {
  int n = 0, m = 0, lds = 0;
  const auto query = occupancy_into(n, 1);
  const auto query_share = [&](auto kernel, int bytes) { query(kernel, bytes), lds = bytes; };
  switch (id) {
    case kGenerate: query(k_generate, 0); break;
    case kIntersect: with_intersect(sc, false, false, query); break;
    case kIntersectLegacy: with_intersect(sc, true, false, query); break;
    case kPrimary: with_primary(sc, false, 0, query_share); break;
    case kPrimaryShared:
      for (int form : {0, kSplitRecords, kFirstBounce}) with_primary(sc, true, form, query_share), m = form ? min(m, n) : n;
      n = m;
      break;
    case kPaths:
      for (int form : {0, kSplitRecords, kFirstBounce}) with_paths(resolve_scan_nodes(sc), search_form(sc), form, query_share), m = form ? min(m, n) : n;
      n = m;
      break;
    case kShade: query(k_shade, shade_lds<true>(sc).total); break;
    case kFeatures: with_features(sc, query); break;
  }
  if (n < 1) n = 1;
  n = min(n, max(1, lds_share_limit(lds)));
  return n > 8 ? 8 : n;
}

void launch_generate(hipStream_t s, int grid, const ptd::Camera& cam, const BatchInfo& b, const ptd::Queues& qs,
                     ptd::PathBuf out, int32_t* cnt0) {
  hipLaunchKernelGGL(k_generate, dim3(grid), dim3(kBlock), 0, s, cam, b, qs, out, cnt0);
}

void launch_intersect(hipStream_t s, int grid, const SceneTables& sc, const ptd::Queues& qs, const int32_t* cnt_in,
                      ptd::PathBuf paths, ptd::HitBuf hits, bool legacy, bool exact_arith) {
  with_intersect(sc, legacy, exact_arith, [&](auto kernel, int lds) { hipLaunchKernelGGL(kernel, dim3(grid), dim3(kBlock), lds, s, sc, qs, cnt_in, paths, hits); });
}

void launch_intersect_grid(hipStream_t s, int grid, const SceneTables& sc, const ptd::Queues& qs, const int32_t* cnt_in,
                           ptd::PathBuf paths, ptd::HitBuf hits, bool primary) {
  with_intersect_grid(sc, primary, [&](auto kernel, int lds) { hipLaunchKernelGGL(kernel, dim3(grid), dim3(kBlock), lds, s, sc, qs, cnt_in, paths, hits); });
}

void launch_primary(hipStream_t s, int grid, const SceneTables& sc, const ptd::Camera& cam, const BatchInfo& b,
                    const ptd::Queues& qs, int32_t* cnt0, int32_t* cnt_out, ptd::PathBuf out, ptd::RetireBuf ret) {
  with_primary(sc, primary_shares(b), primary_shares(b) ? b.split_records : 0, [&](auto kernel, int lds) { hipLaunchKernelGGL(kernel, dim3(grid), dim3(kBlock), lds, s, sc, cam, b, qs, cnt0, cnt_out, out, ret); });
}

void launch_features(hipStream_t s, int grid, const SceneTables& sc, const ptd::Camera& cam, const BatchInfo& b, float4* feat) {
  with_features(sc, [&](auto kernel, int lds) {
    if (lds > 64 * 1024) (void)hipFuncSetAttribute(reinterpret_cast<const void*>(kernel), hipFuncAttributeMaxDynamicSharedMemorySize, lds);
    hipLaunchKernelGGL(kernel, dim3(grid), dim3(kBlock), lds, s, sc, cam, b, feat);
  });
}

void launch_paths(hipStream_t s, int grid, const SceneTables& sc_in, const BatchInfo& b, const ptd::Queues& qs, int32_t* cnt, ptd::PathBuf in, ptd::RetireBuf ret) {
  const SceneTables sc = resolve_scan_nodes(sc_in);
  with_paths(sc, search_form(sc), b.split_records, [&](auto kernel, int lds) { hipLaunchKernelGGL(kernel, dim3(grid), dim3(kBlock), lds, s, sc, b, qs, cnt, in, ret); });
}
void launch_shade(hipStream_t s, int grid, const SceneTables& sc, const BatchInfo& b, int depth, const ptd::Queues& qs,
                  const int32_t* cnt_in, int32_t* cnt_out, ptd::PathBuf in, ptd::HitBuf hits, ptd::PathBuf out,
                  ptd::RetireBuf ret) {
  hipLaunchKernelGGL(k_shade, dim3(grid), dim3(kBlock), shade_lds<true>(sc).total, s, sc, b, depth, qs, cnt_in, cnt_out, in, hits, out,
                     ret);
}

int flat_grid(int n, int cap) {
  int grid = (n + kBlock - 1) / kBlock;
  return grid > cap ? cap : (grid < 1 ? 1 : grid);
}
void launch_collect(hipStream_t s, const BatchInfo& b, const ptd::Queues& qs, ptd::RetireBuf ret, float* image_rgb) {
  (void)hipFuncSetAttribute(reinterpret_cast<const void*>(k_collect), hipFuncAttributeMaxDynamicSharedMemorySize, collect_lds_bytes(ret.wq0));
  hipLaunchKernelGGL(k_collect, dim3(qs.Q), dim3(kCollectThreads), collect_lds_bytes(ret.wq0), s, b, qs, ret, image_rgb);
}
void launch_collect_conv(hipStream_t s, const BatchInfo& b, const ptd::Queues& qs, ptd::RetireBuf ret, float* image_rgb, const ConvInfo& cv, double* sse) {
  (void)hipFuncSetAttribute(reinterpret_cast<const void*>(k_collect_conv), hipFuncAttributeMaxDynamicSharedMemorySize, collect_lds_bytes(ret.wq0));
  hipLaunchKernelGGL(k_collect_conv, dim3(qs.Q), dim3(kCollectThreads), collect_lds_bytes(ret.wq0), s, b, qs, ret, image_rgb, cv);
  if (cv.first_k < b.K) hipLaunchKernelGGL(k_conv_reduce, dim3(b.K - cv.first_k), dim3(kBlock), 0, s, b.iter_first, cv.first_k, qs.Q * kCollectWaves, cv.partial, sse);
}

#include "pt_ieee_check.inc"

void launch_count_stats(hipStream_t s, const ptd::Queues& qs, int32_t* cnt, int depth_count,
                        unsigned long long* stats) {
  hipLaunchKernelGGL(k_count_stats, dim3(depth_count + 2), dim3(kBlock), 0, s, qs, cnt, depth_count, stats);
}

void launch_preview(hipStream_t s, int n, int iterations, const float* image_rgb, uchar4* rgba) {
  hipLaunchKernelGGL(k_preview, dim3(flat_grid(n, 4096)), dim3(kBlock), 0, s, n, iterations, image_rgb, rgba);
}

void launch_save_u8(hipStream_t s, int n, int width, float samples, const float* image_rgb, uint8_t* rgb8) {
  hipLaunchKernelGGL(k_save_u8, dim3(flat_grid(n, 4096)), dim3(kBlock), 0, s, n, width, samples, image_rgb, rgb8);
}

void launch_shade_stage(hipStream_t s, const SceneTables& sc, int trace_depth, int depth, int n, const int32_t* iter,
                        const int32_t* pixel, ptd::HitBuf hits, ptd::PathBuf paths, int32_t* alive) {
  hipLaunchKernelGGL(k_shade_stage, dim3(flat_grid(n, 2048)), dim3(kBlock), shade_lds<false>(sc).total, s, sc, trace_depth, depth, n, iter, pixel, hits,
                     paths, alive);
}
```

### cosc_4397_pathtracing_raytracing_project_amd/csrc/pt_output.inc

```
constexpr int kCollectThreads = 1024;
constexpr int kCollectPPT = 8;
constexpr int kCollectPixels = kCollectPPT * kCollectThreads;
__host__ __device__ inline int collect_lds_bytes(int wq0) { return kCollectPixels * 12 + wq0 * 4; }
struct CollectChunk {
  ptd::Word4 v[kCollectPPT];
};
template <bool FRESH = false>
PT_DEV void collect_load(const ptd::Word4* rec, int n, int i0, uint32_t skip, CollectChunk& c) {
  int t = (int)threadIdx.x;
  if constexpr (FRESH) asm volatile("" : "+v"(t));
#pragma unroll
  for (int u = 0; u < kCollectPPT; ++u) {
    if (u > 0 && i0 + u * kCollectThreads >= n) break;
    const int i = i0 + u * kCollectThreads + t;
    if (!(skip >> u & 1u)) c.v[u] = rec[i < n ? i : (n > 0 ? n - 1 : 0)];
  }
}
PT_DEV uint32_t collect_front_bits(const int* front, int quo, int rem, int n, int i0) {
  uint32_t bits = 0;
#pragma unroll 1
  for (int u = 0; u < kCollectPPT; ++u) {
    if (u > 0 && i0 + u * kCollectThreads >= n) break;
    const int i = i0 + u * kCollectThreads + (int)threadIdx.x;
    if (i < n) {
      const SubSlot s = sub_slot(quo, rem, i);
      bits |= (retiree_slot(s, front[s.rho]) ? 1u : 0u) << u;
    }
  }
  return bits;
}
PT_DEV void collect_scatter(const CollectChunk& c, int n, int i0, uint32_t skip, int g0, int g1, int Q, float inv_q, int first, float* tile) {
#pragma unroll
  for (int u = 0; u < kCollectPPT; ++u) {
    if (u > 0 && i0 + u * kCollectThreads >= n) break;
    const int i = i0 + u * kCollectThreads + (int)threadIdx.x;
    const int pl = __float_as_int(c.v[u].w);
    int jj, qq;
    divmod(pl >> 6, Q, inv_q, jj, qq);
    const int li = jj * 64 + (pl & 63) - first;
    if (i < n && !(skip >> u & 1u) && !(i >= g0 && i < g1) && li >= 0 && li < kCollectPixels) tile[3 * li] = c.v[u].x, tile[3 * li + 1] = c.v[u].y, tile[3 * li + 2] = c.v[u].z;
  }
}
constexpr int kCollectWaves = kCollectThreads / 64;
static_assert(kCollectWaves == kConvWaves, "the host sizes the partial sums with pt_kernels.h kConvWaves");
PT_DEV bool conv_div_ok(float x, float y, float z) {
  const uint32_t a = __float_as_uint(x), b = __float_as_uint(y), c = __float_as_uint(z);
  return max(max(a, b), c) < 0x57000000u && min(min(a - 1u, b - 1u), c - 1u) >= 0x28000000u - 1u;
}
template <int CTRL>
PT_DEV double dpp_f64(double v) {
  const unsigned long long u = (unsigned long long)__double_as_longlong(v);
  const uint32_t lo = (uint32_t)__builtin_amdgcn_update_dpp(0, (int)(uint32_t)u, CTRL, 0xf, 0xf, false);
  const uint32_t hi = (uint32_t)__builtin_amdgcn_update_dpp(0, (int)(uint32_t)(u >> 32), CTRL, 0xf, 0xf, false);
  return __longlong_as_double((long long)((unsigned long long)hi << 32 | lo));
}
PT_DEV double readlane_f64(double v, int lane) {
  const unsigned long long u = (unsigned long long)__double_as_longlong(v);
  const uint32_t lo = (uint32_t)__builtin_amdgcn_readlane((int)(uint32_t)u, lane), hi = (uint32_t)__builtin_amdgcn_readlane((int)(uint32_t)(u >> 32), lane);
  return __longlong_as_double((long long)((unsigned long long)hi << 32 | lo));
}
PT_DEV double wave_sum_f64(double v) {
  v += dpp_f64<0xb1>(v);
  v += dpp_f64<0x4e>(v);
  v += dpp_f64<0x141>(v);
  v += dpp_f64<0x140>(v);
  return ((readlane_f64(v, 0) + readlane_f64(v, 16)) + readlane_f64(v, 32)) + readlane_f64(v, 48);
}
template <bool CONV, bool ONCE>
PT_DEV void collect_body(BatchInfo b, ptd::Queues qs, ptd::RetireBuf ret, float* __restrict__ image, ConvInfo cv) {
  extern __shared__ float4 lds_raw[];
  float* tile = reinterpret_cast<float*>(lds_raw);
  const int q = blockIdx.x;
  const QueueShare sh = queue_share(b, qs, q);
  const float inv_q = 1.0f / (float)qs.Q;
  const ptd::Word4* rec = ret.rec + (int64_t)q * ret.kmax * ret.seg_cap;
  const int n = b.flat ? sh.my_pixels : sh.my_nq * 64;
  const auto [g0, g1] = b.flat ? Gap{0, 0} : region_gap(sh, ret.wq0);
  constexpr bool once = ONCE;
  int* front = reinterpret_cast<int*>(tile + 3 * kCollectPixels);
  const int quo = once ? sh.my_nq / ret.wq0 : 0, rem = once ? sh.my_nq % ret.wq0 : 0;
  if (once) {
    for (int rho = threadIdx.x; rho < ret.wq0; rho += kCollectThreads) front[rho] = (int)(ret.sub[(int64_t)q * ret.kmax * ret.wq0 + rho] >> 32);
    __syncthreads();
  }
  for (int first = 0; first < sh.my_nq * 64; first += kCollectPixels) {
    float acc[kCollectPPT][3];
    float rf[CONV ? kCollectPPT : 1][3];
    uint32_t mine_bits = 0;
    if (once) mine_bits = collect_front_bits(front, quo, rem, n, 0) << 8;
#pragma unroll
    for (int m = 0; m < kCollectPPT; ++m) {
      const int li = first + threadIdx.x + kCollectThreads * m;
      const int pl = slot_pixel(q, li, qs.Q);
      const bool mine = li < sh.my_nq * 64 && pl < b.N;
      acc[m][0] = mine ? image[3 * (int64_t)pl] : 0.f, acc[m][1] = mine ? image[3 * (int64_t)pl + 1] : 0.f, acc[m][2] = mine ? image[3 * (int64_t)pl + 2] : 0.f;
      if constexpr (CONV) {
        const bool have = mine && cv.first_k == 0;
        mine_bits |= (mine ? 1u : 0u) << m;
        rf[m][0] = have ? cv.ref[3 * (int64_t)pl] : 0.f, rf[m][1] = have ? cv.ref[3 * (int64_t)pl + 1] : 0.f, rf[m][2] = have ? cv.ref[3 * (int64_t)pl + 2] : 0.f;
      }
    }
    CollectChunk c;
    collect_load<CONV>(rec, n, 0, 0u, c);
    for (int k = 0; k < b.K; ++k) {
      collect_scatter(c, n, 0, once && k > 0 ? mine_bits >> 8 : 0u, g0, g1, qs.Q, inv_q, first, tile);
      for (int i0 = kCollectPixels; i0 < n; i0 += kCollectPixels) {
        const uint32_t skip = once && k > 0 ? collect_front_bits(front, quo, rem, n, i0) : 0u;
        collect_load<CONV>(rec + (int64_t)k * ret.seg_cap, n, i0, skip, c);
        collect_scatter(c, n, i0, skip, g0, g1, qs.Q, inv_q, first, tile);
      }
      if (k + 1 < b.K) collect_load<CONV>(rec + (int64_t)(k + 1) * ret.seg_cap, n, 0, once ? mine_bits >> 8 : 0u, c);
      __syncthreads();
#pragma unroll
      for (int m = 0; m < kCollectPPT; ++m) {
        if (m > 0 && first + kCollectThreads * m >= sh.my_nq * 64) break;
        const int li = threadIdx.x + kCollectThreads * m;
        acc[m][0] += tile[3 * li], acc[m][1] += tile[3 * li + 1], acc[m][2] += tile[3 * li + 2];
      }
      if constexpr (CONV) {
        if (k == cv.capture_k || k >= cv.first_k) {
          const float n_it = __uint_as_float(__builtin_amdgcn_readfirstlane(__float_as_uint((float)(b.iter_first + k))));
          uint32_t ok = 1u;
#pragma unroll
          for (int m = 0; m < kCollectPPT; ++m) {
            if (m > 0 && first + kCollectThreads * m >= sh.my_nq * 64) break;
            ok &= (~mine_bits >> m & 1u) | (uint32_t)conv_div_ok(acc[m][0], acc[m][1], acc[m][2]);
          }
          const bool short_div = ieee::every_lane(ok != 0u);
          const float r_it = __uint_as_float(__builtin_amdgcn_readfirstlane(__float_as_uint(ieee::rcp_core(n_it))));
          double sum = 0.0;
#pragma unroll
          for (int m = 0; m < kCollectPPT; ++m) {
            if (m > 0 && first + kCollectThreads * m >= sh.my_nq * 64) break;
            const bool mine = mine_bits >> m & 1u;
            f3 cur;
            if (short_div) cur = mk(ieee::quot_core(acc[m][0], n_it, r_it), ieee::quot_core(acc[m][1], n_it, r_it), ieee::quot_core(acc[m][2], n_it, r_it));
            else cur = mk(acc[m][0] / n_it, acc[m][1] / n_it, acc[m][2] / n_it);
            if (k == cv.capture_k) {
              rf[m][0] = cur.x, rf[m][1] = cur.y, rf[m][2] = cur.z;
              int t_cap = (int)threadIdx.x;
              asm volatile("" : "+v"(t_cap));
              const int li = first + t_cap + kCollectThreads * m;
              const int pl = slot_pixel(q, li, qs.Q);
              if (mine) cv.ref[3 * (int64_t)pl] = cur.x, cv.ref[3 * (int64_t)pl + 1] = cur.y, cv.ref[3 * (int64_t)pl + 2] = cur.z;
            } else {
              const f3 d = ex::sub(cur, mk(rf[m][0], rf[m][1], rf[m][2]));
              sum += mine ? (double)ex::dot(d, d) : 0.0;
            }
          }
          if (k >= cv.first_k) {
            sum = wave_sum_f64(sum);
            double* slot = cv.partial + ((int64_t)k * qs.Q + q) * kCollectWaves + (threadIdx.x >> 6);
            if ((threadIdx.x & 63) == 0) *slot = first == 0 ? sum : *slot + sum;
          }
        }
      }
      __syncthreads();
    }
    int t_out = (int)threadIdx.x;
    if constexpr (CONV) asm volatile("" : "+v"(t_out));
#pragma unroll
    for (int m = 0; m < kCollectPPT; ++m) {
      const int li = first + t_out + kCollectThreads * m;
      const int pl = slot_pixel(q, li, qs.Q);
      if (li < sh.my_nq * 64 && pl < b.N) image[3 * (int64_t)pl] = acc[m][0], image[3 * (int64_t)pl + 1] = acc[m][1], image[3 * (int64_t)pl + 2] = acc[m][2];
    }
  }
  for (int i = threadIdx.x; i < ret.kmax; i += kCollectThreads) ret.cnt[(int64_t)q * ret.kmax + i] = 0ull;
}
__global__ __launch_bounds__(kCollectThreads) void k_collect(BatchInfo b, ptd::Queues qs, ptd::RetireBuf ret, float* __restrict__ image) {
  if (b.retire_once && !b.flat) collect_body<false, true>(b, qs, ret, image, ConvInfo{});
  else collect_body<false, false>(b, qs, ret, image, ConvInfo{});
}
__global__ __launch_bounds__(kCollectThreads) void k_collect_conv(BatchInfo b, ptd::Queues qs, ptd::RetireBuf ret, float* __restrict__ image, ConvInfo cv) {
  if (b.retire_once && !b.flat) collect_body<true, true>(b, qs, ret, image, cv);
  else collect_body<true, false>(b, qs, ret, image, cv);
}
__global__ __launch_bounds__(kBlock) void k_conv_reduce(int iter_first, int first_k, int count, const double* __restrict__ partial, double* __restrict__ sse) {
  const int k = first_k + blockIdx.x;
  const double* p = partial + (int64_t)k * count;
  double acc = 0.0;
  for (int i = threadIdx.x; i < count; i += kBlock) acc += p[i];
  for (int off = 32; off > 0; off >>= 1) acc += __shfl_xor(acc, off, 64);
  __shared__ double part[kWavesPerBlock];
  if ((threadIdx.x & 63) == 0) part[threadIdx.x >> 6] = acc;
  __syncthreads();
  if (threadIdx.x == 0) {
    double t = part[0];
    for (int w = 1; w < kWavesPerBlock; ++w) t += part[w];
    sse[iter_first + k - 1] = t;
  }
}

constexpr int kDealMaxQ = 2048;
PT_DEV void deal_waves(const ptd::Queues& qs) {
  __shared__ int work[kDealMaxQ];
  if (qs.deal == nullptr) return;
  const DealMap dm = deal_map(qs);
  if (threadIdx.x == 0) qs.deal[dm.strand_counter()] = 0;
  for (int q = threadIdx.x; q < qs.Q; q += blockDim.x) qs.deal[dm.piece_counter(q)] = 0;
  int32_t* first = qs.deal + dm.first(0);
  int32_t* wk = qs.deal + dm.time(0);
  const int Q = qs.Q, W = qs.paths_W;
  if (Q > kDealMaxQ || W < Q) {
    if (threadIdx.x == 0) qs.deal[dm.made_for()] = 0;
    for (int q = threadIdx.x; q < Q; q += blockDim.x) wk[q] = 0, qs.deal[dm.rays(q)] = 0;
    return;
  }
  __shared__ unsigned long long ray_total_s;
  __shared__ int ray_heaviest_s;
  if (threadIdx.x == 0) ray_total_s = 0ull, ray_heaviest_s = 0;
  __syncthreads();
  {
    int32_t* rays = qs.deal + dm.rays(0);
    unsigned long long sum = 0;
    int hv = 0;
    for (int q = threadIdx.x; q < Q; q += blockDim.x) sum += (unsigned long long)rays[q], hv = max(hv, rays[q]), rays[q] = 0;
    atomicAdd(&ray_total_s, sum);
    atomicMax(&ray_heaviest_s, hv);
  }
  for (int q = threadIdx.x; q < Q; q += blockDim.x) work[q] = wk[q], wk[q] = 0;
  __syncthreads();
  const bool close_together = queues_close_together(ray_heaviest_s, ray_total_s, W, Q);
  if (threadIdx.x < 64) {
    const int lane = threadIdx.x;
    unsigned long long total = 0;
    for (int e0 = 0; e0 < Q; e0 += 64) {
      unsigned long long v = e0 + lane < Q ? (unsigned long long)work[e0 + lane] : 0ull;
      for (int off = 32; off > 0; off >>= 1) v += __shfl_xor(v, off, 64);
      total += v;
    }
    if (close_together) total = 0;
    unsigned long long before = 0;
    for (int e0 = 0; e0 < Q && total > 0; e0 += 64) {
      const unsigned long long mine = e0 + lane < Q ? (unsigned long long)work[e0 + lane] : 0ull;
      unsigned long long incl = mine;
      for (int off = 1; off < 64; off <<= 1) {
        const unsigned long long up = __shfl_up(incl, off, 64);
        if (lane >= off) incl += up;
      }
      if (e0 + lane < Q) first[e0 + lane] = dealt_first(e0 + lane, W, Q, before + incl - mine, total);
      before += __shfl(incl, 63, 64);
    }
    if (lane == 0) qs.deal[dm.made_for()] = total > 0 ? W : 0;
  }
}

__global__ void k_count_stats(ptd::Queues qs, int32_t* __restrict__ cnt, int depth_count,
                              unsigned long long* __restrict__ stats) {
  const int d = blockIdx.x;
  if (d == depth_count + 1) {
    deal_waves(qs);
    return;
  }
  if (d > depth_count) return;
  unsigned long long acc = 0;
  for (int q = threadIdx.x; q < qs.Q; q += blockDim.x) {
    int32_t* c = &cnt[cnt_index(qs, d, q)];
    acc += (unsigned long long)*c;
    *c = 0;
  }
  if (d == depth_count) return;
  for (int off = 32; off > 0; off >>= 1) acc += __shfl_down(acc, off, 64);
  __shared__ unsigned long long part[kWavesPerBlock];
  if ((threadIdx.x & 63) == 0) part[threadIdx.x >> 6] = acc;
  __syncthreads();
  if (threadIdx.x == 0) {
    unsigned long long t = 0;
    for (int w = 0; w < (int)(blockDim.x >> 6); ++w) t += part[w];
    stats[d] += t;
  }
}

__global__ __launch_bounds__(kBlock) void k_preview(int n, int iterations, const float* __restrict__ image,
                                                    uchar4* __restrict__ rgba) {
  for (int p = blockIdx.x * blockDim.x + threadIdx.x; p < n; p += gridDim.x * blockDim.x) {
    const float inv = (float)iterations;
    float v[3];
    for (int c = 0; c < 3; ++c) {
      const float pix = __builtin_powf(image[3 * (int64_t)p + c] / inv, 1.0f / 2.2f);
      int q = (int)(pix * 255.0f);
      v[c] = (float)(q < 0 ? 0 : (q > 255 ? 255 : q));
    }
    rgba[p] = make_uchar4((unsigned char)v[0], (unsigned char)v[1], (unsigned char)v[2], 0);
  }
}

__global__ __launch_bounds__(kBlock) void k_save_u8(int n, int width, float samples, const float* __restrict__ image,
                                                    uint8_t* __restrict__ rgb8) {
  const float inv_w = 1.0f / (float)width;
  for (int p = blockIdx.x * blockDim.x + threadIdx.x; p < n; p += gridDim.x * blockDim.x) {
    int ty, x;
    divmod(p, width, inv_w, ty, x);
    uint8_t* dst = rgb8 + 3 * ((int64_t)ty * width + (width - 1 - x));
#pragma unroll
    for (int c = 0; c < 3; ++c) {
      const float v = image[3 * (int64_t)p + c] / samples;
      float m = v > 0.0f ? v : 0.0f;
      m = m < 1.0f ? m : 1.0f;
      dst[c] = (uint8_t)(m * 255.f);
    }
  }
}
```

### cosc_4397_pathtracing_raytracing_project_amd/csrc/pt_sched.h

```cpp
#pragma once
#include "pt_kernels.h"

#define PT_SCHED __host__ __device__ inline __attribute__((always_inline))

namespace ptk {

PT_SCHED int sched_min(int a, int b) { return a < b ? a : b; }
PT_SCHED int sched_max(int a, int b) { return a > b ? a : b; }

struct DealMap {
  int Q;
  PT_SCHED int first(int q) const { return q; }
  PT_SCHED int made_for() const { return Q; }
  PT_SCHED int time(int q) const { return Q + 1 + q; }
  PT_SCHED int strand_counter() const { return 2 * Q + 1; }
  PT_SCHED int piece_counter(int q) const { return 2 * Q + 2 + q; }
  PT_SCHED int rays(int q) const { return 3 * Q + 2 + q; }
  PT_SCHED int words() const { return 4 * Q + 2; }
};
PT_SCHED DealMap deal_map(const ptd::Queues& qs) { return DealMap{qs.Q}; }

PT_SCHED int dealt_first(int q, int W, int Q, unsigned long long work_before, unsigned long long work_total) {
  return q + (int)((unsigned long long)(W - Q) * work_before / work_total);
}
PT_SCHED bool queues_close_together(int heaviest_rays, unsigned long long total_rays, int W, int Q) {
  return (unsigned long long)heaviest_rays * W * Q <= total_rays * ((unsigned long long)W + Q);
}

struct WaveSlot {
  int q, r, wq;
};
PT_SCHED WaveSlot wave_slot(int wave, int Q, int W) { return WaveSlot{wave % Q, wave / Q, W / Q}; }

struct QueueShare {
  int my_nq;
  int my_pixels;
  float inv_my_nq;
};
PT_SCHED QueueShare queue_share(const BatchInfo& b, const ptd::Queues& qs, int q) {
  const int chunks = (b.N + 63) >> 6;
  QueueShare sh;
  sh.my_nq = q < chunks ? (chunks - q + qs.Q - 1) / qs.Q : 0;
  const int last_q = (chunks - 1) % qs.Q;
  sh.my_pixels = sh.my_nq * 64 - ((q == last_q && (b.N & 63)) ? 64 - (b.N & 63) : 0);
  sh.inv_my_nq = sh.my_nq > 0 ? 1.0f / (float)sh.my_nq : 0.0f;
  return sh;
}
PT_SCHED int chunk_pixel(int q, int jj, int Q) { return (q + jj * Q) * 64; }
PT_SCHED int slot_pixel(int q, int li, int Q) { return chunk_pixel(q, li >> 6, Q) + (li & 63); }

PT_SCHED int sub_chunks(int quo, int rem, int rho) { return quo + (rho < rem ? 1 : 0); }
PT_SCHED int sub_offset(int quo, int rem, int rho) { return rho * quo + sched_min(rho, rem); }
struct Gap {
  int g0, g1;
};
PT_SCHED Gap region_gap(const QueueShare& sh, int wq0) {
  Gap g{0, 0};
  const int missing = sh.my_nq * 64 - sh.my_pixels;
  if (missing > 0) {
    const int quo = sh.my_nq / wq0, rem = sh.my_nq % wq0, rho = (sh.my_nq - 1) % wq0;
    g.g1 = (sub_offset(quo, rem, rho) + sub_chunks(quo, rem, rho)) * 64;
    g.g0 = g.g1 - missing;
  }
  return g;
}

PT_SCHED size_t cnt_index(const ptd::Queues& qs, int d, int q) { return (size_t)qs.Q * qs.cnt_stride * d + (size_t)q * qs.cnt_stride; }

struct QueuePlan {
  int nq, seg_cap, cap;
};
PT_SCHED int chunks_per_queue(int64_t N, int Q) { return (int)(((N + 63) / 64 + Q - 1) / Q); }
PT_SCHED QueuePlan queue_plan(int64_t N, int Q, int K) {
  QueuePlan p;
  p.nq = chunks_per_queue(N, Q);
  p.seg_cap = p.nq * 64;
  p.cap = K * p.seg_cap;
  return p;
}
PT_SCHED size_t sub_stride(int widest_grid_waves, int Q) { return (size_t)widest_grid_waves / Q; }

struct StrandPlan {
  int kp, pieces;
};
PT_SCHED StrandPlan strand_plan(int K, int primary_pieces, bool deal_present, bool flat) {
  StrandPlan p;
  p.kp = primary_pieces > 1 && deal_present && !flat ? (K + primary_pieces - 1) / primary_pieces : K;
  p.pieces = (K + p.kp - 1) / p.kp;
  return p;
}
struct Strand {
  int piece, q, r, wq, k0, k1;
};
PT_SCHED Strand strand_of(int strand, const StrandPlan& p, int K, int Q, int W) {
  Strand s;
  s.piece = strand / W;
  const WaveSlot w = wave_slot(strand - s.piece * W, Q, W);
  s.q = w.q, s.r = w.r, s.wq = w.wq;
  s.k0 = s.piece * p.kp, s.k1 = sched_min(K, s.k0 + p.kp);
  return s;
}
PT_SCHED int strand_rho(int r, int k, int wq) { return (r + k) % wq; }
PT_SCHED int strand_rho_before(int r, int k, int wq) { return (r + k + wq - 1) % wq; }
PT_SCHED int auto_primary_pieces(int K, int nq, int wq0) {
  const int64_t want = (int64_t)K * nq / sched_max(1, wq0) / 48;
  return want < 1 ? 1 : want > 4 ? 4 : (int)want;
}

constexpr int kShareMax = 64;
PT_SCHED bool primary_shares(int primary_share, bool aa_jitter, bool flat) { return primary_share > 1 && !aa_jitter && !flat; }
PT_SCHED bool primary_shares(const BatchInfo& b) { return primary_shares(b.primary_share, b.aa_jitter != 0, b.flat != 0); }
PT_SCHED int shared_rho(int r, int , int ) { return r; }
PT_SCHED int shared_run_cap(int primary_share) { return primary_share < 1 ? 1 : sched_min(primary_share, kShareMax); }
struct Run {
  int k0, k1;
};
PT_SCHED int shared_runs(int k0, int k1, int cap) { return (k1 - k0 + cap - 1) / cap; }
PT_SCHED Run shared_run(int k0, int k1, int cap, int i) { return Run{k0 + i * cap, sched_min(k1, k0 + (i + 1) * cap)}; }
PT_SCHED int auto_shared_pieces(int K, int , int ) {
  const int want = sched_max(2, (K + kShareMax - 1) / kShareMax);
  return sched_max(1, sched_min(want, K));
}

constexpr int kRetireEveryIteration = 1024;
PT_SCHED bool retires_once(int primary_share, bool aa_jitter, bool flat, int trace_depth, int debug_flags) {
  return primary_shares(primary_share, aa_jitter, flat) && trace_depth >= 2 && !(debug_flags & kRetireEveryIteration);
}
PT_SCHED bool retires_once(const BatchInfo& b, int debug_flags) {
  return retires_once(b.primary_share, b.aa_jitter != 0, b.flat != 0, b.trace_depth, debug_flags);
}
struct SubSlot {
  int rho, pos;
};
PT_SCHED SubSlot sub_slot(int quo, int rem, int i) {
  const int c = i >> 6, big = rem * (quo + 1);
  const int rho = c < big ? c / (quo + 1) : rem + (c - big) / sched_max(quo, 1);
  return SubSlot{rho, i - sub_offset(quo, rem, rho) * 64};
}
PT_SCHED bool retiree_slot(const SubSlot& s, int retirees) { return s.pos < retirees; }

constexpr int kWholeRecords = 4096;
PT_SCHED bool splits_records(int primary_share, bool aa_jitter, bool flat, int trace_depth, int debug_flags) {
  return primary_shares(primary_share, aa_jitter, flat) && trace_depth >= 2 && !(debug_flags & kWholeRecords);
}
PT_SCHED bool splits_records(const BatchInfo& b, int debug_flags) {
  return splits_records(b.primary_share, b.aa_jitter != 0, b.flat != 0, b.trace_depth, debug_flags);
}
PT_SCHED int invariant_slot(int at, int k, int seg_cap) { return at - k * seg_cap; }
PT_SCHED uint32_t pack_kind(int sample_id, bool specular) { return (uint32_t)sample_id | (specular ? 0x80000000u : 0u); }
PT_SCHED int kind_sample_id(uint32_t word) { return (int)(word & 0x7fffffffu); }
PT_SCHED bool kind_specular(uint32_t word) { return (word >> 31) != 0u; }

constexpr int kNoFirstBounce = 8192;
constexpr int kSplitRecords = 1, kFirstBounce = 2;
constexpr int kVisitBits = 8;
PT_SCHED uint32_t pack_visit(int k, int visit) { return ((uint32_t)k << kVisitBits) | ((uint32_t)visit & ((1u << kVisitBits) - 1u)); }
PT_SCHED int visit_k(uint32_t word) { return (int)(word >> kVisitBits); }
PT_SCHED int visit_number(uint32_t word) { return (int)(word & ((1u << kVisitBits) - 1u)); }
PT_SCHED int visit_gap(int visits_now, int visit) { return (visits_now - visit) & ((1 << kVisitBits) - 1); }
PT_SCHED bool visit_k_fits(int K) { return K <= (1 << (31 - kVisitBits)); }
PT_SCHED int pack_first(int pl, int mat, int slot_shift) { return (mat << slot_shift) | pl; }
PT_SCHED int first_pixel(int word, int slot_shift) { return word & ((1 << slot_shift) - 1); }
PT_SCHED int first_material(int word, int slot_shift) { return (int)((uint32_t)word >> slot_shift); }
PT_SCHED bool first_material_fits(int num_mats, int slot_shift) { return num_mats <= (1 << (31 - slot_shift)); }
PT_SCHED bool first_bounces(int primary_share, bool aa_jitter, bool flat, int trace_depth, int debug_flags, int search_form, int num_mats,
                            int slot_shift, int K) {
  return splits_records(primary_share, aa_jitter, flat, trace_depth, debug_flags) &&
         retires_once(primary_share, aa_jitter, flat, trace_depth, debug_flags) && !(debug_flags & kNoFirstBounce) && search_form == 0 &&
         first_material_fits(num_mats, slot_shift) && visit_k_fits(K);
}
PT_SCHED bool first_bounces(const BatchInfo& b, int debug_flags, int search_form, int num_mats) {
  return first_bounces(b.primary_share, b.aa_jitter != 0, b.flat != 0, b.trace_depth, debug_flags, search_form, num_mats, b.slot_shift, b.K);
}
PT_SCHED int record_form(const BatchInfo& b, int debug_flags, int search_form, int num_mats) {
  return first_bounces(b, debug_flags, search_form, num_mats) ? kFirstBounce : splits_records(b, debug_flags) ? kSplitRecords : 0;
}

PT_SCHED int pack_paths_pieces(int count, int min_piece) { return count | min_piece << 16; }
PT_SCHED int paths_pieces_count(int word) { return word & 0xffff; }
PT_SCHED int paths_pieces_min(int word) { return word >> 16; }
struct PieceRange {
  int start, end;
  bool some;
};
struct PiecePlan {
  int total, wq, pieces_per_wave, ps_min, ps0;
  PT_SCHED bool needs_counter() const { return ps0 * wq < total; }
  PT_SCHED PieceRange piece_range(int nextp) const {
    int start = total, sz = ps0;
    if (nextp >= 0) {
      start = 0;
      int level = nextp / wq;
      const int idx = nextp - level * wq;
      for (; level > 0 && start < total; --level) start += wq * sz, sz = sched_max(sz - sz / pieces_per_wave, ps_min);
      start += idx * sz;
    }
    return start < total ? PieceRange{start, sched_min(start + sz, total), true} : PieceRange{total, total, false};
  }
};
PT_SCHED PiecePlan piece_plan(int total, int wq, int paths_pieces, bool deal_present, bool chunk_sums) {
  PiecePlan p;
  p.total = total, p.wq = wq;
  p.pieces_per_wave = deal_present && chunk_sums && paths_pieces_count(paths_pieces) > 1 ? paths_pieces_count(paths_pieces) : 1;
  p.ps_min = paths_pieces_min(paths_pieces);
  p.ps0 = sched_max((total + wq * p.pieces_per_wave - 1) / (wq * p.pieces_per_wave), p.ps_min);
  return p;
}

}
```

### include/pt_amd.h

```cpp
#ifndef PT_AMD_H
#define PT_AMD_H

#include <stdint.h>

#ifdef __cplusplus
extern "C" {
#endif

#define PT_GEOM_SPHERE 0
#define PT_GEOM_CUBE 1
#define PT_GEOM_TRIANGLE 2

typedef struct PtGeom {
  int32_t type;
  int32_t materialid;
  float transform[16];
  float inverseTransform[16];
  float invTranspose[16];
} PtGeom;

typedef struct PtMaterial {
  float color[3];
  float specular_exponent;
  float specular_color[3];
  float hasReflective;
  float hasRefractive;
  float indexOfRefraction;
  float emittance;
} PtMaterial;

typedef struct PtCamera {
  int32_t resolution[2];
  float position[3];
  float lookAt[3];
  float view[3];
  float up[3];
  float right[3];
  float fov[2];
  float pixelLength[2];
} PtCamera;

typedef struct PtBVHNode {
  float bmin[3];
  float bmax[3];
  int32_t left, right, geomIndex;
} PtBVHNode;

typedef struct PtSceneDesc {
  const PtGeom* geoms;
  int32_t num_geoms;
  const PtMaterial* materials;
  int32_t num_materials;
  PtCamera camera;
  int32_t trace_depth;
} PtSceneDesc;

typedef struct PtOptions {
  int32_t device;
  int32_t pixel_begin;
  int32_t pixel_count;
  int32_t iters_per_batch;
  int32_t num_queues;
  int32_t blocks_per_cu;
  int32_t time_kernels;
  int32_t legacy_traversal;
  int32_t debug_flags;
  int32_t unfused_primary;
  int32_t unfused_bounces;
  int32_t stripe_pixels;
  int32_t stripe_stride;
  int32_t arith;
  int32_t aa_jitter;
  int32_t convergence;
  int32_t lds_table_kb;
  int32_t primary_pieces;
  int32_t paths_pieces;
  int32_t paths_min_piece;
} PtOptions;
#define PT_PRIMARY_PIECES(pieces, share) ((int32_t)((pieces) | (share) << 16))

#define PT_ARITH_EXACT 0
#define PT_ARITH_FMA 1
#define PT_ARITH_FAST 2

#define PT_MAX_DEPTH 64
typedef struct PtStats {
  int64_t samples;
  int64_t live_rays[PT_MAX_DEPTH];
  int64_t intersect_launches;
  double intersect_ms;
  double render_ms;
  int32_t num_cus, grid_blocks, num_queues, iters_per_batch;
  int64_t device_bytes;
  int32_t primary_fused;
  int32_t bounces_fused;
  int32_t arith;
  int32_t grid_cells;
  int32_t tight_leaves;
  int32_t paths_waves;
  int32_t record_form;
} PtStats;

typedef struct PtScene PtScene;
int pt_scene_load(const char* path, int res_w, int res_h, PtScene** out);
void pt_scene_free(PtScene* s);
int pt_scene_desc(const PtScene* s, PtSceneDesc* out);
int pt_scene_iterations(const PtScene* s);
const char* pt_scene_image_name(const PtScene* s);

int pt_build_bvh(const PtGeom* geoms, int num_geoms, PtBVHNode* out, int cap);

typedef struct PtGridInfo {
  int32_t res[3];
  float origin[3], cell_size[3], pad;
  int32_t num_cells, num_records, num_leaves;
} PtGridInfo;
typedef struct PtGridRecord {
  float bmin[3], bmax[3];
  int32_t leaf;
  int32_t neighbours;
} PtGridRecord;
int pt_build_grid(const PtGeom* geoms, int num_geoms, int forced, PtGridInfo* info, uint32_t* cell_start, PtGridRecord* records);

int pt_traversal_boxes(const PtGeom* geoms, int num_geoms, const float camera_position[3], float* boxes);

void pt_center_half_box(const float lo[3], const float hi[3], int inner, float magnitude, float center[3], float half_extent[3]);

int pt_build_transform(const float* trs, float* transform, float* inverse, float* invTranspose);

int pt_init(const PtSceneDesc* scene, const PtOptions* opt);
int pt_free(void);
int pt_render(int iter_first, int iter_count);
int pt_sync(void);
int pt_readback(float* rgb_sum_host);
int pt_readback_device(void* rgb_sum_dev);
int pt_preview_rgba8(int iterations, uint8_t* rgba_host);
int pt_preview_rgba8_device(int iterations, void* rgba_dev);
int pt_get_stats(PtStats* out);
int pt_reset_stats(void);
int pt_clear(void);
const char* pt_last_error(void);
int pt_selfcheck_ieee(int arith, int kind, uint64_t first, uint64_t count, uint32_t seed, uint64_t* mismatches);
#define PT_CONVERGENCE_WAVES 16
#define PT_CONVERGENCE_CAPACITY 65536
int pt_set_reference(const float* rgb_avg_host);
int pt_get_convergence(int iter_first, int iter_count, double* sse);
int pt_iterations_to_clean(float threshold_db, int* iteration);
float pt_psnr_from_sse(double sse, int64_t pixels);

#define PT_FEATURE_PLANES 3
int pt_render_features(int iter_first, int iter_count);
int pt_readback_features(float* planes_host);

typedef struct PtDenoiseOptions {
  int32_t levels;
  float sigma_color;
  float sigma_normal;
  float sigma_position;
  int32_t keep_albedo;
} PtDenoiseOptions;
int pt_denoise(float samples, const PtDenoiseOptions* opt, float* rgb_avg_host);
int pt_denoise_host(int w, int rows, const float* rgb_sum, const float* planes, float samples, const PtDenoiseOptions* opt, float* rgb_avg);

#define PT_NOISE_PLANES 2
#define PT_NOISE_PIXELS_PER_PARTIAL 1024
int pt_noise_fold(void);
int pt_get_noise(double* sse, int* groups, int* iterations);
int pt_readback_noise(float* planes_host);
int pt_render_until(int iter_first, int max_iters, int group_iters, float target_db, int* iters_done, float* psnr_db);
int pt_noise_fold_host(int pixels, const float* rgb_sum, float* planes, int group_iters, int groups_after, int64_t iters_after, double* sse);

#define PT_DENOISE_VARIANCE_FLOOR 1e-8f
int pt_denoise_guided(const PtDenoiseOptions* opt, float* rgb_avg_host);
int pt_denoise_guided_host(int w, int rows, const float* rgb_sum, const float* planes, const float* noise_planes, int groups, int64_t iters,
                           const PtDenoiseOptions* opt, float* rgb_avg);
int pt_denoise_guided_variance_host(int w, int rows, const float* rgb_sum, const float* planes, const float* noise_planes, int groups, int64_t iters,
                                    const PtDenoiseOptions* opt, float* var_raw, float* var_0);

int pt_adaptive_round(int iter_first, int group_iters, float fraction);
int pt_render_adaptive(int iter_first, int max_iters, int group_iters, float fraction, float target_db, int* iters_done, int64_t* samples_done,
                       float* psnr_db);
int pt_readback_adaptive(int32_t* counts);
int pt_resolve(float* rgb_avg_host);
int pt_adaptive_select_host(int w, int rows, const float* noise_planes, const int32_t* counts, int m, int32_t* list);
int pt_adaptive_merge_host(int pixels, float* rgb_sum, float* planes, int32_t* counts, const int32_t* list, int m, const float* group_sum,
                           int group_iters, double* sse);

int pt_denoise_adaptive(const PtDenoiseOptions* opt, float* rgb_avg_host);
int pt_denoise_adaptive_host(int w, int rows, const float* rgb_sum, const float* planes, const float* noise_planes, const int32_t* counts,
                             const PtDenoiseOptions* opt, float* rgb_avg);
int pt_denoise_adaptive_variance_host(int w, int rows, const float* rgb_sum, const float* planes, const float* noise_planes, const int32_t* counts,
                                      const PtDenoiseOptions* opt, float* var_raw, float* var_0);

int pt_save_u8(float samples, uint8_t* rgb8_host);

typedef struct PtContext PtContext;
int pt_ctx_create(const PtSceneDesc* scene, const PtOptions* opt, PtContext** out);
int pt_ctx_destroy(PtContext* c);
int pt_ctx_render(PtContext* c, int iter_first, int iter_count);
int pt_ctx_sync(PtContext* c);
int pt_ctx_readback(PtContext* c, float* rgb_sum_host);
int pt_ctx_readback_device(PtContext* c, void* rgb_sum_dev);
int pt_ctx_save_u8(PtContext* c, float samples, uint8_t* rgb8_host);
int pt_ctx_save_u8_device(PtContext* c, float samples, const uint8_t** rgb8_dev);
int pt_ctx_preview_rgba8(PtContext* c, int iterations, uint8_t* rgba_host);
int pt_ctx_preview_rgba8_device(PtContext* c, int iterations, void* rgba_dev);
int pt_ctx_get_stats(PtContext* c, PtStats* out);
int pt_ctx_reset_stats(PtContext* c);
int pt_ctx_clear(PtContext* c);
int pt_ctx_set_reference(PtContext* c, const float* rgb_avg_host);
int pt_ctx_get_convergence(PtContext* c, int iter_first, int iter_count, double* sse);
int pt_ctx_iterations_to_clean(PtContext* c, float threshold_db, int* iteration);
int pt_ctx_render_features(PtContext* c, int iter_first, int iter_count);
int pt_ctx_readback_features(PtContext* c, float* planes_host);
int pt_ctx_denoise(PtContext* c, float samples, const PtDenoiseOptions* opt, float* rgb_avg_host);
int pt_ctx_denoise_device(PtContext* c, float samples, const PtDenoiseOptions* opt, const float** rgb_dev);
int pt_ctx_denoise_guided(PtContext* c, const PtDenoiseOptions* opt, float* rgb_avg_host);
int pt_ctx_denoise_guided_device(PtContext* c, const PtDenoiseOptions* opt, const float** rgb_dev);
int pt_ctx_denoise_adaptive(PtContext* c, const PtDenoiseOptions* opt, float* rgb_avg_host);
int pt_ctx_denoise_adaptive_device(PtContext* c, const PtDenoiseOptions* opt, const float** rgb_dev);
int pt_ctx_noise_fold(PtContext* c);
int pt_ctx_get_noise(PtContext* c, double* sse, int* groups, int* iterations);
int pt_ctx_readback_noise(PtContext* c, float* planes_host);
int pt_ctx_render_until(PtContext* c, int iter_first, int max_iters, int group_iters, float target_db, int* iters_done, float* psnr_db);
int pt_ctx_adaptive_round(PtContext* c, int iter_first, int group_iters, float fraction);
int pt_ctx_render_adaptive(PtContext* c, int iter_first, int max_iters, int group_iters, float fraction, float target_db, int* iters_done,
                           int64_t* samples_done, float* psnr_db);
int pt_ctx_readback_adaptive(PtContext* c, int32_t* counts);
int pt_ctx_resolve(PtContext* c, float* rgb_avg_host);
int pt_ctx_resolve_device(PtContext* c, const float** rgb_dev);
const float* pt_ctx_device_noise(PtContext* c);
const float* pt_ctx_device_features(PtContext* c);
const float* pt_ctx_device_image(PtContext* c);
void* pt_ctx_stream(PtContext* c);
int pt_ctx_pixel_count(const PtContext* c);
int pt_ctx_device(const PtContext* c);

typedef struct PtGroup PtGroup;
#define PT_GROUP_TRANSPORT_AUTO 0
#define PT_GROUP_TRANSPORT_RCCL 1
#define PT_GROUP_TRANSPORT_COPY 2
int pt_group_create_ex(const PtSceneDesc* scene, const PtOptions* base, const int* devices, int num_devices, int transport,
                       PtGroup** out);
int pt_group_transport(const PtGroup* g);
int pt_group_create(const PtSceneDesc* scene, const PtOptions* base, const int* devices, int num_devices, PtGroup** out);
int pt_group_destroy(PtGroup* g);
int pt_group_size(const PtGroup* g);
PtContext* pt_group_context(PtGroup* g, int i);
int pt_group_render(PtGroup* g, int iter_first, int iter_count);
int pt_group_sync(PtGroup* g);
int pt_group_gather(PtGroup* g, float* rgb_sum_host);
int pt_group_gather_u8(PtGroup* g, float samples, uint8_t* rgb8_host);
int pt_group_render_features(PtGroup* g, int iter_first, int iter_count);
int pt_group_gather_features(PtGroup* g, float* planes_host);
int pt_group_denoise(PtGroup* g, float samples, const PtDenoiseOptions* opt, float* rgb_avg_host);
int pt_group_denoise_guided(PtGroup* g, const PtDenoiseOptions* opt, float* rgb_avg_host);
int pt_group_noise_fold(PtGroup* g);
int pt_group_get_noise(PtGroup* g, double* sse, int* groups, int* iterations);
int pt_group_render_until(PtGroup* g, int iter_first, int max_iters, int group_iters, float target_db, int* iters_done, float* psnr_db);
int pt_group_preview_rgba8(PtGroup* g, int iterations, uint8_t* rgba_host);

int pt_group_set_reference(PtGroup* g, const float* rgb_avg_host);
int pt_group_get_convergence(PtGroup* g, int iter_first, int iter_count, double* sse);
int pt_group_iterations_to_clean(PtGroup* g, float threshold_db, int* iteration);

int pt_stage_generate(int pix_begin, int n, float* origin, float* dir);
int pt_stage_intersect(int n, const float* origin, const float* dir, float* t, float* normal, int32_t* material,
                       float* point);
int pt_stage_intersect_grid(int n, const float* origin, const float* dir, int primary_form, float* t, float* normal,
                            int32_t* material, float* point);
int pt_stage_grid_info(PtGridInfo* info, int32_t* max_cell_records);
int pt_stage_shade(int n, int depth, const int32_t* iter, const int32_t* pixel, const float* t, const float* normal,
                   const int32_t* material, const float* point, float* origin, float* dir, float* color,
                   int32_t* alive);

int pt_stage_save_u8(int w, int h, float samples, const float* rgb_sum, uint8_t* rgb8);

int pt_stage_denoise(int w, int rows, const float* rgb_sum, const float* planes, float samples, const PtDenoiseOptions* opt, float* rgb_avg);
int pt_stage_denoise_guided(int w, int rows, const float* rgb_sum, const float* planes, const float* noise_planes, int groups, int64_t iters,
                            const PtDenoiseOptions* opt, float* rgb_avg);

int pt_stage_denoise_adaptive(int w, int rows, const float* rgb_sum, const float* planes, const float* noise_planes, const int32_t* counts,
                              const PtDenoiseOptions* opt, float* rgb_avg);
int pt_stage_adaptive_select(int w, int rows, const float* noise_planes, const int32_t* counts, int m, int32_t* list);
int pt_stage_render_list(const int32_t* list, int m, int iter_first, int iter_count, float* rgb_sum_host);

int pt_save_png(const char* path, const float* rgb_sum, int w, int h, float samples);
int pt_write_png_rgb8(const char* path, const uint8_t* rgb8, int w, int h);
int pt_output_basename(const char* name, int samples, char* out, int cap);
int pt_save_pfm(const char* path, const float* rgb_sum, int w, int h, float samples);
int pt_load_pfm(const char* path, float* rgb_sum, int cap_pixels, int* w, int* h, float samples);
int pt_save_hdr(const char* path, const float* rgb_sum, int w, int h, float samples);

#ifdef __cplusplus
}
#endif
#endif
```

Baseline: 39420.

## Write first-bounce retirees to fixed slots and gather image with streaming collect kernel

Adds a fixed-slot variant of the first-bounce paths kernel, where each retired path's record slot is derived from its region offset and iteration instead of being claimed through an atomic fill counter on a visit ring. This also removes the visit-lap ballot and the per-refill visit limit. A new streaming collect kernel then sums each pixel's K records directly from their fixed positions, with coalesced grouped loads, and folds the count_stats rows into the same launch. The aim is to drop LDS atomics and a tile-sort gather pass plus one launch, at the cost of a new slot-packing scheme whose bit width limits K and which depends on retiree slot invariants holding.

```diff
diff --git a/cosc_4397_pathtracing_raytracing_project_amd/capi.py b/cosc_4397_pathtracing_raytracing_project_amd/capi.py
--- a/cosc_4397_pathtracing_raytracing_project_amd/capi.py
+++ b/cosc_4397_pathtracing_raytracing_project_amd/capi.py
@@ -68,7 +68,8 @@
                 ("intersect_ms", C.c_double), ("render_ms", C.c_double), ("num_cus", C.c_int32),
                 ("grid_blocks", C.c_int32), ("num_queues", C.c_int32), ("iters_per_batch", C.c_int32),
                 ("device_bytes", C.c_int64), ("primary_fused", C.c_int32), ("bounces_fused", C.c_int32),
-                ("arith", C.c_int32), ("grid_cells", C.c_int32), ("tight_leaves", C.c_int32), ("paths_waves", C.c_int32), ("record_form", C.c_int32)]
+                ("arith", C.c_int32), ("grid_cells", C.c_int32), ("tight_leaves", C.c_int32), ("paths_waves", C.c_int32), ("record_form", C.c_int32),
+                ("gather_form", C.c_int32)]
 
 
 class PtDenoiseOptions(C.Structure):
diff --git a/cosc_4397_pathtracing_raytracing_project_amd/csrc/pt_api.cpp b/cosc_4397_pathtracing_raytracing_project_amd/csrc/pt_api.cpp
--- a/cosc_4397_pathtracing_raytracing_project_amd/csrc/pt_api.cpp
+++ b/cosc_4397_pathtracing_raytracing_project_amd/csrc/pt_api.cpp
@@ -13,7 +13,7 @@
 namespace {
 
 std::string g_err;
-constexpr int kDebugFlags = 16 | 32 | 64 | 128 | 256 | 512 | ptk::kRetireEveryIteration | 2048 | ptk::kWholeRecords | ptk::kNoFirstBounce;
+constexpr int kDebugFlags = 16 | 32 | 64 | 128 | 256 | 512 | ptk::kRetireEveryIteration | 2048 | ptk::kWholeRecords | ptk::kNoFirstBounce | ptk::kRecordsByVisit | ptk::kTileGather;
 static_assert(sizeof(PtOptions) == 80, "capi.PtOptions mirrors this layout");
 static_assert(PT_CONVERGENCE_WAVES == ptk::kConvWaves, "pt_amd.h documents the size of the convergence metric's partial sums");
 }
@@ -124,6 +124,7 @@
   b.split_records = ptk::record_form(b, g.debug_flags, ptk::search_form(sc), sc.num_mats);
   if (b.split_records == ptk::kFirstBounce) b.primary_pieces = 1;
   g.record_form = b.split_records;
+  b.fixed_slots = ptk::fixed_slots(b, g.debug_flags, ptk::search_form(sc), sc.num_mats, g.ret.seg_cap) ? 1 : 0;
   b.list = g.list;
   if (b.list) b.stripe = 1, b.gap = 0, b.inv_stripe = 1.0f;
   const ptk::KernelApi& k = *g.k;
@@ -165,15 +166,20 @@
     k.shade(g.stream, g.grid_shade, sc, b, d, queues_for(g, g.grid_shade), cin, cout, g.buf[src], g.hits, g.buf[src ^ 1], g.ret);
     src ^= 1;
   }
-  k.count_stats(g.stream, g.qs, g.d_cnt, g.depth, g.d_stats);
   ptk::ConvInfo cv{g.d_ref, g.d_partial, -1, kb};
   if (g.conv_live) {
     if (g.conv_have_ref) cv.first_k = 0;
     else if (g.conv >= iter_first && g.conv < iter_first + kb) cv.capture_k = g.conv - iter_first, cv.first_k = cv.capture_k + 1, g.conv_have_ref = true;
     g.conv_last = std::max(g.conv_last, iter_first + kb - 1);
   }
-  if (cv.capture_k >= 0 || cv.first_k < kb) k.collect_conv(g.stream, b, g.qs, g.ret, g.d_image, cv, g.d_sse);
-  else k.collect(g.stream, b, g.qs, g.ret, g.d_image);
+  const bool conv_batch = cv.capture_k >= 0 || cv.first_k < kb;
+  g.gather_form = ptk::gather_form(b.fixed_slots != 0, g.debug_flags, conv_batch);
+  if (g.gather_form == ptk::kGatherStream) k.collect_stream(g.stream, b, g.qs, g.ret, g.d_image, g.d_cnt, g.depth, g.d_stats);
+  else {
+    k.count_stats(g.stream, g.qs, g.d_cnt, g.depth, g.d_stats);
+    if (conv_batch) k.collect_conv(g.stream, b, g.qs, g.ret, g.d_image, cv, g.d_sse);
+    else k.collect(g.stream, b, g.qs, g.ret, g.d_image);
+  }
   HIP_OK(hipGetLastError());
   g.samples += (int64_t)kb * g.N;
   if (g.pending_isect.size() > 16384) {
@@ -730,6 +736,7 @@
   }
   out->tight_leaves = g.tight_leaves;
   out->record_form = g.record_form;
+  out->gather_form = g.gather_form;
   out->paths_waves = 0;
   if (g.qs.deal && g.grid_paths > 0) {
     const ptk::DealMap dm = ptk::deal_map(g.qs);
diff --git a/cosc_4397_pathtracing_raytracing_project_amd/csrc/pt_context.h b/cosc_4397_pathtracing_raytracing_project_amd/csrc/pt_context.h
--- a/cosc_4397_pathtracing_raytracing_project_amd/csrc/pt_context.h
+++ b/cosc_4397_pathtracing_raytracing_project_amd/csrc/pt_context.h
@@ -53,6 +53,7 @@
   bool legacy = false;
   int debug_flags = 0;
   int record_form = 0;
+  int gather_form = 0;
   bool fuse_primary = true, fuse_bounces = true;
   bool aa_jitter = false;
 };
diff --git a/cosc_4397_pathtracing_raytracing_project_amd/csrc/pt_kernels.h b/cosc_4397_pathtracing_raytracing_project_amd/csrc/pt_kernels.h
--- a/cosc_4397_pathtracing_raytracing_project_amd/csrc/pt_kernels.h
+++ b/cosc_4397_pathtracing_raytracing_project_amd/csrc/pt_kernels.h
@@ -55,6 +55,7 @@
   int32_t retire_once;
   const int32_t* list;
   int32_t split_records;
+  int32_t fixed_slots;
 };
 
 constexpr int kConvWaves = 16;
@@ -93,6 +94,8 @@
   int boxes_center_half;
   void (*intersect_grid)(hipStream_t s, int grid, const SceneTables& sc, const ptd::Queues& qs, const int32_t* cnt_in,
                          ptd::PathBuf paths, ptd::HitBuf hits, bool primary);
+  void (*collect_stream)(hipStream_t s, const BatchInfo& b, const ptd::Queues& qs, ptd::RetireBuf ret, float* image_rgb, int32_t* cnt, int depth_count,
+                         unsigned long long* stats);
 };
 const KernelApi* api_exact();
 const KernelApi* api_fma();
diff --git a/cosc_4397_pathtracing_raytracing_project_amd/csrc/pt_kernels.hip b/cosc_4397_pathtracing_raytracing_project_amd/csrc/pt_kernels.hip
--- a/cosc_4397_pathtracing_raytracing_project_amd/csrc/pt_kernels.hip
+++ b/cosc_4397_pathtracing_raytracing_project_amd/csrc/pt_kernels.hip
@@ -1347,6 +1347,7 @@
     lnodes = lds + L.nodes;
   }
   using WM = PathsWaveMap<MODE, kFast>;
+  constexpr bool FIXED = SPLIT == kFixedSlots, FIRST = SPLIT == kFirstBounce || FIXED;
   const int he = iter_hash_entries(sc);
   uint32_t* tword = reinterpret_cast<uint32_t*>(lds + L.tword);
   int* lmat = reinterpret_cast<int*>(lds + L.lmat);
@@ -1368,7 +1369,7 @@
   constexpr bool SLOTS = MODE == 0;
   char* slots = wbase + WM::slots;
   int* died = reinterpret_cast<int*>(wbase + WM::died);
-  int* fillc = reinterpret_cast<int*>(wbase + WM::fillc);
+  [[maybe_unused]] int* fillc = reinterpret_cast<int*>(wbase + WM::fillc);
   const int ntop = sc.num_top;
   const int wave = __builtin_amdgcn_readfirstlane(blockIdx.x * kWavesPerBlock + wib);
   const int lane = lane_id();
@@ -1410,6 +1411,8 @@
   int cord = 0;
   [[maybe_unused]] int cur_k = 0;
   [[maybe_unused]] uint32_t cur_h = 0u, next_h = 0u;
+  [[maybe_unused]] int crec0 = 0;
+  [[maybe_unused]] const int fbits = fixed_bits(rt.seg_cap);
   int win0 = -64;
   unsigned long long wsub = 0ull;
   auto window_to = [&](int e) {
@@ -1428,10 +1431,11 @@
     const int ec = min(ce, ne - 1), ck = ec / wq0, crho = ec - ck * wq0;
     clist = ck * rt.seg_cap + sub_offset(quo, rem, crho) * 64;
     if constexpr (SPLIT != 0) clist0 = invariant_slot(clist, ck, rt.seg_cap);
-    if constexpr (SPLIT == kFirstBounce) cur_k = ck, cur_h = iter_hash(b.iter_first + ck, 0);
+    if constexpr (FIRST) cur_k = ck, cur_h = iter_hash(b.iter_first + ck, 0);
     window_to(ec);
     const int crec = clist + (int)(uint32_t)(sub_word(ec) >> 32);
-    if (lane == 0) fillc[cord & (kVisitRing - 1)] = crec + (first_rank - cstart);
+    if constexpr (FIXED) crec0 = invariant_slot(crec, ck, rt.seg_cap);
+    else if (lane == 0) fillc[cord & (kVisitRing - 1)] = crec + (first_rank - cstart);
   };
   auto seek = [&](int at_rank) {
     int cum = 0, e_begin = 0;
@@ -1467,10 +1471,10 @@
       if (in) at = clist + (rank - cstart), rs = cord;
       if constexpr (SPLIT != 0)
         if (in) at0 = clist0 + (rank - cstart);
-      if constexpr (SPLIT == kFirstBounce)
-        if (in) rs = (int)pack_visit(cur_k, cord), next_h = cur_h;
+      if constexpr (FIRST)
+        if (in) rs = (int)(FIXED ? pack_fixed(cur_k, crec0 + (rank - cstart), fbits) : pack_visit(cur_k, cord)), next_h = cur_h;
       pending = pending && !in;
-      if (!ballot(pending) || ce >= ne || cord - cord0 >= kVisitsPerRefill) break;
+      if (!ballot(pending) || ce >= ne || (!FIXED && cord - cord0 >= kVisitsPerRefill)) break;
       cstart += ccnt;
       ccnt = 0;
       int nxt = ce + 1;
@@ -1500,7 +1504,7 @@
   int* slot_rs = reinterpret_cast<int*>(slots + kSlotVisit) + lane;
   auto fetch = [&](int at, [[maybe_unused]] int at0, int rs) {
     if constexpr (SLOTS && SPLIT == kSplitRecords) fetch_split_to_lds(in0, in1, at, at0, s_base), *slot_rs = rs;
-    else if constexpr (SLOTS) fetch_record_to_lds(in0, in1, in2, SPLIT == kFirstBounce ? at0 : at, s_base), *slot_rs = rs;
+    else if constexpr (SLOTS) fetch_record_to_lds(in0, in1, in2, FIRST ? at0 : at, s_base), *slot_rs = rs;
     else if constexpr (SPLIT == kSplitRecords) {
       const ptd::Word4 w0 = in.r[qbase + at], w1 = in.r[in.stride + qbase + at0];
       nx.o = mk(w0.x, w0.y, w0.z), nx.d = mk(w0.w, w1.x, w1.y), nx.c = mk(w1.z, w1.w, 0.f), nx_rs = rs;
@@ -1512,7 +1516,7 @@
   bool valid = false, fresh = false, owes = false;
   bool has_next = false;
   int streamed = 0, p_hi = 0;
-  while (SPLIT != kFirstBounce) {
+  while (!FIRST) {
     if (streamed >= p_hi && p_hi >= 0) {
       int nextp = -1;
       if (cord == 0) nextp = r;
@@ -1646,7 +1650,7 @@
       }
     }
   }
-  if constexpr (SPLIT == kFirstBounce) {
+  if constexpr (FIRST) {
     static_assert(MODE == kLdsTables, "the first-bounce form takes its records from the refill slots of the LDS-table form");
     while (true) {
       if (ballot(fresh)) {
@@ -1685,7 +1689,8 @@
         }
         const bool alive = ready && s.alive, dead = ready && !s.alive;
         if (dead) atomicAdd(&died[depth & 63], 1);
-        if (dead) rslot = atomicAdd(&fillc[rslot & (kVisitRing - 1)], 1);
+        if constexpr (!FIXED)
+          if (dead) rslot = atomicAdd(&fillc[rslot & (kVisitRing - 1)], 1);
         if (ready) {
           c = s.c;
           if (alive) {
@@ -1721,9 +1726,9 @@
           owes = false;
         }
         if (take) {
-          const int pl = first_pixel(word, b.slot_shift), k = visit_k((uint32_t)vword);
+          const int pl = first_pixel(word, b.slot_shift), k = FIXED ? fixed_k((uint32_t)vword, fbits) : visit_k((uint32_t)vword);
           const f3 hn = mk(w0.w, w1.x, w1.y), cam_d = mk(w1.z, w1.w, cz);
-          slot = make_slot(b, k, pl), rslot = visit_number((uint32_t)vword);
+          slot = make_slot(b, k, pl), rslot = FIXED ? fixed_slot_of((uint32_t)vword, fbits, rt.seg_cap) : visit_number((uint32_t)vword);
           phash = utilhash((uint32_t)global_pixel(b, pl));
           ShadeIO s;
           s.o = mk(0.f, 0.f, 0.f);
@@ -1737,7 +1742,8 @@
           valid = go = true;
           has_next = false;
         }
-        const bool lapping = ballot(valid && visit_gap(cord, rslot) >= kVisitLap) != 0ull;
+        bool lapping = false;
+        if constexpr (!FIXED) lapping = ballot(valid && visit_gap(cord, rslot) >= kVisitLap) != 0ull;
         const bool empty = !has_next && !lapping;
         const unsigned long long em = ballot(empty);
         const int rank = rank_in(em);
@@ -1806,7 +1812,7 @@
 #endif
     launch_generate, launch_primary, launch_intersect, launch_shade, launch_collect, launch_count_stats,
     launch_preview, launch_save_u8, launch_shade_stage, lds_table_limit, resident_blocks_per_cu, launch_ieee_check, launch_paths,
-    launch_collect_conv, launch_features, kFast ? 1 : 0, launch_intersect_grid};
+    launch_collect_conv, launch_features, kFast ? 1 : 0, launch_intersect_grid, launch_collect_stream};
 
 }
 }
diff --git a/cosc_4397_pathtracing_raytracing_project_amd/csrc/pt_launch.inc b/cosc_4397_pathtracing_raytracing_project_amd/csrc/pt_launch.inc
--- a/cosc_4397_pathtracing_raytracing_project_amd/csrc/pt_launch.inc
+++ b/cosc_4397_pathtracing_raytracing_project_amd/csrc/pt_launch.inc
@@ -40,6 +40,7 @@
   switch (form) {
     case kLdsTables:
       if (split == kFirstBounce) return f(k_paths<kLdsTables, kFirstBounce>, paths_lds<kLdsTables, kFast>(sc).total);
+      if (split == kFixedSlots) return f(k_paths<kLdsTables, kFixedSlots>, paths_lds<kLdsTables, kFast>(sc).total);
       return split ? f(k_paths<kLdsTables, kSplitRecords>, paths_lds<kLdsTables, kFast>(sc).total) : f(k_paths<kLdsTables>, paths_lds<kLdsTables, kFast>(sc).total);
     case kTopScan: return split ? f(k_paths<kTopScan, kSplitRecords>, paths_lds<kTopScan, kFast>(sc).total) : f(k_paths<kTopScan>, paths_lds<kTopScan, kFast>(sc).total);
     case kGrid: return split ? f(k_paths<kGrid, kSplitRecords>, paths_lds<kGrid, kFast>(sc).total) : f(k_paths<kGrid>, paths_lds<kGrid, kFast>(sc).total);
@@ -106,7 +107,7 @@
       n = m;
       break;
     case kPaths:
-      for (int form : {0, kSplitRecords, kFirstBounce}) with_paths(resolve_scan_nodes(sc), search_form(sc), form, query_share), m = form ? min(m, n) : n;
+      for (int form : {0, kSplitRecords, kFirstBounce, kFixedSlots}) with_paths(resolve_scan_nodes(sc), search_form(sc), form, query_share), m = form ? min(m, n) : n;
       n = m;
       break;
     case kShade: query(k_shade, shade_lds<true>(sc).total); break;
@@ -146,7 +147,7 @@
 
 void launch_paths(hipStream_t s, int grid, const SceneTables& sc_in, const BatchInfo& b, const ptd::Queues& qs, int32_t* cnt, ptd::PathBuf in, ptd::RetireBuf ret) {
   const SceneTables sc = resolve_scan_nodes(sc_in);
-  with_paths(sc, search_form(sc), b.split_records, [&](auto kernel, int lds) { hipLaunchKernelGGL(kernel, dim3(grid), dim3(kBlock), lds, s, sc, b, qs, cnt, in, ret); });
+  with_paths(sc, search_form(sc), b.split_records == kFirstBounce && b.fixed_slots ? kFixedSlots : b.split_records, [&](auto kernel, int lds) { hipLaunchKernelGGL(kernel, dim3(grid), dim3(kBlock), lds, s, sc, b, qs, cnt, in, ret); });
 }
 void launch_shade(hipStream_t s, int grid, const SceneTables& sc, const BatchInfo& b, int depth, const ptd::Queues& qs,
                   const int32_t* cnt_in, int32_t* cnt_out, ptd::PathBuf in, ptd::HitBuf hits, ptd::PathBuf out,
@@ -162,6 +163,11 @@
 void launch_collect(hipStream_t s, const BatchInfo& b, const ptd::Queues& qs, ptd::RetireBuf ret, float* image_rgb) {
   (void)hipFuncSetAttribute(reinterpret_cast<const void*>(k_collect), hipFuncAttributeMaxDynamicSharedMemorySize, collect_lds_bytes(ret.wq0));
   hipLaunchKernelGGL(k_collect, dim3(qs.Q), dim3(kCollectThreads), collect_lds_bytes(ret.wq0), s, b, qs, ret, image_rgb);
+}
+void launch_collect_stream(hipStream_t s, const BatchInfo& b, const ptd::Queues& qs, ptd::RetireBuf ret, float* image_rgb, int32_t* cnt, int depth_count,
+                           unsigned long long* stats) {
+  const int per_queue = (ret.seg_cap + kBlock - 1) / kBlock;
+  hipLaunchKernelGGL(k_collect_stream, dim3(qs.Q * per_queue + depth_count + 2), dim3(kBlock), 0, s, b, qs, ret, image_rgb, per_queue, cnt, depth_count, stats);
 }
 void launch_collect_conv(hipStream_t s, const BatchInfo& b, const ptd::Queues& qs, ptd::RetireBuf ret, float* image_rgb, const ConvInfo& cv, double* sse) {
   (void)hipFuncSetAttribute(reinterpret_cast<const void*>(k_collect_conv), hipFuncAttributeMaxDynamicSharedMemorySize, collect_lds_bytes(ret.wq0));
diff --git a/cosc_4397_pathtracing_raytracing_project_amd/csrc/pt_output.inc b/cosc_4397_pathtracing_raytracing_project_amd/csrc/pt_output.inc
--- a/cosc_4397_pathtracing_raytracing_project_amd/csrc/pt_output.inc
+++ b/cosc_4397_pathtracing_raytracing_project_amd/csrc/pt_output.inc
@@ -246,9 +246,7 @@
   }
 }
 
-__global__ void k_count_stats(ptd::Queues qs, int32_t* __restrict__ cnt, int depth_count,
-                              unsigned long long* __restrict__ stats) {
-  const int d = blockIdx.x;
+PT_DEV void count_stats_row(const ptd::Queues& qs, int32_t* __restrict__ cnt, int depth_count, unsigned long long* __restrict__ stats, int d) {
   if (d == depth_count + 1) {
     deal_waves(qs);
     return;
@@ -271,6 +269,51 @@
     stats[d] += t;
   }
 }
+__global__ void k_count_stats(ptd::Queues qs, int32_t* __restrict__ cnt, int depth_count,
+                              unsigned long long* __restrict__ stats) {
+  count_stats_row(qs, cnt, depth_count, stats, blockIdx.x);
+}
+
+constexpr int kStreamGroup = 8;
+__global__ __launch_bounds__(kBlock) void k_collect_stream(BatchInfo b, ptd::Queues qs, ptd::RetireBuf ret, float* __restrict__ image, int per_queue,
+                                                           int32_t* __restrict__ cnt, int depth_count, unsigned long long* __restrict__ stats) {
+  const int gather_blocks = qs.Q * per_queue;
+  if ((int)blockIdx.x >= gather_blocks) {
+    count_stats_row(qs, cnt, depth_count, stats, (int)blockIdx.x - gather_blocks);
+    return;
+  }
+  const int q = (int)blockIdx.x / per_queue, blk = (int)blockIdx.x - q * per_queue;
+  const int s = blk * kBlock + (int)threadIdx.x;
+  if (blk == 0)
+    for (int i = threadIdx.x; i < ret.kmax; i += kBlock) ret.cnt[(int64_t)q * ret.kmax + i] = 0ull;
+  const QueueShare sh = queue_share(b, qs, q);
+  const Gap gap = region_gap(sh, ret.wq0);
+  if (s >= sh.my_nq * 64 || (s >= gap.g0 && s < gap.g1)) return;
+  const SubSlot ss = sub_slot(sh.my_nq / ret.wq0, sh.my_nq % ret.wq0, s);
+  const int retirees = (int)(ret.sub[(int64_t)q * ret.kmax * ret.wq0 + ss.rho] >> 32);
+  const ptd::Word4* rec = ret.rec + (int64_t)q * ret.kmax * ret.seg_cap + s;
+  const ptd::Word4 r0 = rec[0];
+  const int pl = __float_as_int(r0.w);
+  if (pl < 0 || pl >= b.N) return;
+  float* px = image + 3 * (int64_t)pl;
+  float a0 = px[0], a1 = px[1], a2 = px[2];
+  if (retiree_slot(ss, retirees)) {
+    for (int k = 0; k < b.K; ++k) a0 += r0.x, a1 += r0.y, a2 += r0.z;
+  } else {
+    a0 += r0.x, a1 += r0.y, a2 += r0.z;
+    for (int k0 = 1; k0 < b.K; k0 += kStreamGroup) {
+      ptd::Word4 v[kStreamGroup];
+#pragma unroll
+      for (int u = 0; u < kStreamGroup; ++u) v[u] = rec[(int64_t)min(k0 + u, b.K - 1) * ret.seg_cap];
+#pragma unroll
+      for (int u = 0; u < kStreamGroup; ++u) {
+        const bool have = k0 + u < b.K;
+        a0 = have ? a0 + v[u].x : a0, a1 = have ? a1 + v[u].y : a1, a2 = have ? a2 + v[u].z : a2;
+      }
+    }
+  }
+  px[0] = a0, px[1] = a1, px[2] = a2;
+}
 
 __global__ __launch_bounds__(kBlock) void k_preview(int n, int iterations, const float* __restrict__ image,
                                                     uchar4* __restrict__ rgba) {
diff --git a/cosc_4397_pathtracing_raytracing_project_amd/csrc/pt_sched.h b/cosc_4397_pathtracing_raytracing_project_amd/csrc/pt_sched.h
--- a/cosc_4397_pathtracing_raytracing_project_amd/csrc/pt_sched.h
+++ b/cosc_4397_pathtracing_raytracing_project_amd/csrc/pt_sched.h
@@ -176,6 +176,25 @@
   return first_bounces(b, debug_flags, search_form, num_mats) ? kFirstBounce : splits_records(b, debug_flags) ? kSplitRecords : 0;
 }
 
+constexpr int kRecordsByVisit = 16384, kTileGather = 32768;
+constexpr int kFixedSlots = 3;
+PT_SCHED int fixed_slot(int k, int seg_cap, int quo, int rem, int rho, int retirees, int i) { return k * seg_cap + sub_offset(quo, rem, rho) * 64 + retirees + i; }
+PT_SCHED int fixed_bits(int seg_cap) { return 32 - __builtin_clz((unsigned)(seg_cap - 1)); }
+PT_SCHED uint32_t pack_fixed(int k, int in_region, int bits) { return ((uint32_t)k << bits) | (uint32_t)in_region; }
+PT_SCHED int fixed_k(uint32_t word, int bits) { return (int)(word >> bits); }
+PT_SCHED int fixed_slot_of(uint32_t word, int bits, int seg_cap) { return (int)(word >> bits) * seg_cap + (int)(word & ((1u << bits) - 1u)); }
+PT_SCHED bool fixed_word_fits(int K, int seg_cap) { return K <= (1 << (31 - fixed_bits(seg_cap))); }
+PT_SCHED bool fixed_slots(int primary_share, bool aa_jitter, bool flat, int trace_depth, int debug_flags, int search_form, int num_mats, int slot_shift,
+                          int K, int seg_cap) {
+  return first_bounces(primary_share, aa_jitter, flat, trace_depth, debug_flags, search_form, num_mats, slot_shift, K) && fixed_word_fits(K, seg_cap) &&
+         !(debug_flags & kRecordsByVisit);
+}
+PT_SCHED bool fixed_slots(const BatchInfo& b, int debug_flags, int search_form, int num_mats, int seg_cap) {
+  return fixed_slots(b.primary_share, b.aa_jitter != 0, b.flat != 0, b.trace_depth, debug_flags, search_form, num_mats, b.slot_shift, b.K, seg_cap);
+}
+constexpr int kGatherTile = 0, kGatherTileFixed = 1, kGatherStream = 2;
+PT_SCHED int gather_form(bool fixed, int debug_flags, bool convergence) { return !fixed ? kGatherTile : (debug_flags & kTileGather) || convergence ? kGatherTileFixed : kGatherStream; }
+
 PT_SCHED int pack_paths_pieces(int count, int min_piece) { return count | min_piece << 16; }
 PT_SCHED int paths_pieces_count(int word) { return word & 0xffff; }
 PT_SCHED int paths_pieces_min(int word) { return word >> 16; }
diff --git a/include/pt_amd.h b/include/pt_amd.h
--- a/include/pt_amd.h
+++ b/include/pt_amd.h
@@ -99,6 +99,7 @@
   int32_t tight_leaves;
   int32_t paths_waves;
   int32_t record_form;
+  int32_t gather_form;
 } PtStats;
 
 typedef struct PtScene PtScene;
```

New measurement: 40310 (median of 6 runs). 1.02x the previous value.
